# google/dynibar

Hardware: AMD Instinct MI355X
Metric: rays/sec (64 samples x 8 src views) (higher is better)
Workload: dtype f32 in / f32 accumulate; products from two half-float parts per operand (22-bit operands, 3 of the 4 partial products on the f16 matrix pipe, ~2^-20 relative per product); the exact 6-term bf16 build is tested beside it

## Files before the change

dynibar_amd/csrc/dyn_mlp.h:

```cpp
#pragma once
#include <utility>

#include "dyn_device.h"

#ifndef DYN_EXCLUSIVE_CU
#define DYN_EXCLUSIVE_CU 1
#endif
#if DYN_EXCLUSIVE_CU && defined(__AMDGCN__)
#define DYN_CLAIM_REGISTER_FILE() asm volatile("; the whole register file" ::: "v255", "a255")
#else
#define DYN_CLAIM_REGISTER_FILE()
#endif
#define DYN_NET_THREADS 256
#define DYN_VIEW_THREADS 512

__host__ __device__ constexpr int dyn_fi(int r, int h) { return (r & 3) + 8 * (r >> 2) + 4 * h; }

__device__ __forceinline__ f32x16 mfma32(float a, float b, f32x16 c) { return __builtin_amdgcn_mfma_f32_32x32x2f32(a, b, c, 0, 0, 0); }

template <int NT>
__device__ __forceinline__ void acc_zero(f32x16 (&acc)[NT]) {
#pragma unroll
  for (int t = 0; t < NT; ++t)
#pragma unroll
// ... 50 lines not shown
  return __builtin_bit_cast(float, __builtin_amdgcn_mov_dpp(__builtin_bit_cast(int, v), CTRL, 0xF, 0xF, true));
}
template <int VSEG, class Op>
__device__ __forceinline__ float seg_reduce(float v, Op op) {
  static_assert(VSEG == 4 || VSEG == 8 || VSEG == 16 || VSEG == 32, "segments are 4, 8, 16 or 32 lanes");
  v = op(v, dpp_get<DYN_DPP_XOR1>(v));
  v = op(v, dpp_get<DYN_DPP_XOR2>(v));
  if (VSEG >= 8) v = op(v, dpp_get<DYN_DPP_HALF_MIRROR>(v));
  if (VSEG >= 16) v = op(v, dpp_get<DYN_DPP_ROW_MIRROR>(v));
  if (VSEG >= 32) v = op(v, __shfl_xor(v, 16));
  return v;
}
__device__ __forceinline__ float add_half_mirror(float v) {
#if defined(__AMDGCN__)
  float r;
  asm("s_nop 1\n\tv_add_f32_dpp %0, %1, %1 row_half_mirror row_mask:0xf bank_mask:0xf bound_ctrl:1" : "=v"(r) : "v"(v));
  return r;
#else
  return v + dpp_get<DYN_DPP_HALF_MIRROR>(v);
#endif
}
template <int VSEG>
__device__ __forceinline__ float seg_sum(float v, int, int) {
  if (VSEG == 8) {
    v = seg_reduce<4>(v, [](float a, float b) {
#pragma clang fp contract(off)
      return a + b;
    });
    return add_half_mirror(v);
  }
  return seg_reduce<VSEG>(v, [](float a, float b) {
#pragma clang fp contract(off)
    return a + b;
  });
}
template <int VSEG>
__device__ __forceinline__ void seg_sum4(float& a, float& b, float& c, float& d) {
#if defined(__AMDGCN__)
  if (VSEG == 8) {
    auto quad = [](float v) {
      return seg_reduce<4>(v, [](float x, float y) {
#pragma clang fp contract(off)
        return x + y;
      });
    };
    a = quad(a); b = quad(b); c = quad(c); d = quad(d);
    asm("s_nop 1\n\t"
        "v_add_f32_dpp %0, %0, %0 row_half_mirror row_mask:0xf bank_mask:0xf bound_ctrl:1\n\t"
        "v_add_f32_dpp %1, %1, %1 row_half_mirror row_mask:0xf bank_mask:0xf bound_ctrl:1\n\t"
        "v_add_f32_dpp %2, %2, %2 row_half_mirror row_mask:0xf bank_mask:0xf bound_ctrl:1\n\t"
        "v_add_f32_dpp %3, %3, %3 row_half_mirror row_mask:0xf bank_mask:0xf bound_ctrl:1"
        : "+v"(a), "+v"(b), "+v"(c), "+v"(d));
    return;
  }
#endif
  a = seg_sum<VSEG>(a, 0, 0); b = seg_sum<VSEG>(b, 0, 0); c = seg_sum<VSEG>(c, 0, 0); d = seg_sum<VSEG>(d, 0, 0);
}
template <int VSEG>
__device__ __forceinline__ float seg_min(float v, int, int) {
  return seg_reduce<VSEG>(v, [](float a, float b) { return fminf(a, b); });
}
template <int VSEG>
__device__ __forceinline__ float seg_max(float v, int, int) {
  return seg_reduce<VSEG>(v, [](float a, float b) { return fmaxf(a, b); });
}

template <int NTI>
__device__ __forceinline__ float row_dot(const f32x16 (&act)[NTI], const float* tab) {
  const int h = (threadIdx.x & 63) >> 5;
  const float4* t4 = reinterpret_cast<const float4*>(tab + h * 16 * NTI);
  float s = 0.f;
#pragma unroll
  for (int t = 0; t < NTI; ++t)
#pragma unroll
    for (int q = 0; q < 4; ++q) {
      const float4 w = t4[t * 4 + q];
      s = fmaf(act[t][q * 4 + 0], w.x, s);
      s = fmaf(act[t][q * 4 + 1], w.y, s);
      s = fmaf(act[t][q * 4 + 2], w.z, s);
      s = fmaf(act[t][q * 4 + 3], w.w, s);
    }
  return s + __shfl_xor(s, 32);
}

#ifndef DYN_SPLIT_TERMS
#define DYN_SPLIT_TERMS 3
#endif
#ifndef DYN_SPLIT_F16
#define DYN_SPLIT_F16 1
#endif
#if DYN_SPLIT_F16 && DYN_SPLIT_TERMS == 6
#error "the half-float engine has one or two parts per operand (DYN_SPLIT_TERMS == 1 or 3)"
#endif
#if !DYN_SPLIT_F16 && DYN_SPLIT_TERMS == 1
#error "the one-product engine multiplies IEEE halves (DYN_SPLIT_F16 == 1)"
#endif
#if DYN_SPLIT_TERMS == 1
#define DYN_SPLIT_PARTS 1
#define B6_CHUNK_PAIRS 48
#elif DYN_SPLIT_TERMS == 3
#define DYN_SPLIT_PARTS 2
#define B6_CHUNK_PAIRS 24
#elif DYN_SPLIT_TERMS == 6
#define DYN_SPLIT_PARTS 3
#define B6_CHUNK_PAIRS 16
#else
#error "DYN_SPLIT_TERMS must be 1, 3 or 6"
#endif
#define DYN_BIAS_ONE(h) ((DYN_SPLIT_TERMS == 1 || (h) == 0) ? 1.0f : 0.0f)
typedef __bf16 bf16x8 __attribute__((ext_vector_type(8)));
typedef __bf16 bf16x2v __attribute__((ext_vector_type(2)));
typedef _Float16 f16x8 __attribute__((ext_vector_type(8)));
typedef _Float16 f16x2v __attribute__((ext_vector_type(2)));
typedef float f32x2v __attribute__((ext_vector_type(2)));
typedef unsigned u32x4v __attribute__((ext_vector_type(4)));

#define B6_PAIR_FLOATS (DYN_SPLIT_PARTS * 256)
#define B6_CHUNK (B6_CHUNK_PAIRS * B6_PAIR_FLOATS)

#ifdef DYN_PHASE_TIMING
__device__ unsigned long long g_phase[3][2][160];
#define DYN_PHASE_ON (threadIdx.x == 0 && (blockIdx.x == 0 || blockIdx.x == gridDim.x / 2))
#define DYN_PHASE(i)                                                                                  \
  do {                                                                                                \
    if (DYN_PHASE_ON) g_phase[PHASE_KID][blockIdx.x != 0][i] = __builtin_readcyclecounter();          \
  } while (0)
extern "C" int dyn_debug_phases(unsigned long long* out) {
  return hipMemcpyFromSymbol(out, HIP_SYMBOL(g_phase), sizeof(g_phase)) == hipSuccess ? 0 : 1;
}
#define DYN_PHASE_T0 const unsigned long long phase_t0 = __builtin_readcyclecounter();
#ifdef DYN_PHASE_SKEW
__device__ unsigned long long g_skew[8][4];
extern "C" int dyn_debug_skew(unsigned long long* out) { return hipMemcpyFromSymbol(out, HIP_SYMBOL(g_skew), sizeof(g_skew)) == hipSuccess ? 0 : 1; }
extern "C" int dyn_debug_skew_reset(void) { unsigned long long z[32] = {0}; return hipMemcpyToSymbol(HIP_SYMBOL(g_skew), z, sizeof(z)) == hipSuccess ? 0 : 1; }
#endif
#define DYN_PHASE_WAIT(R, c)                                                                          \
  do {                                                                                                \
    if (DYN_PHASE_ON && (c) < 64) {                                                                   \
      g_phase[(R).kid][blockIdx.x != 0][32 + (c)] = __builtin_readcyclecounter() - phase_t0;          \
      g_phase[(R).kid][blockIdx.x != 0][96 + (c)] = phase_t0;                                         \
    }                                                                                                 \
  } while (0)
#define DYN_PHASE_RING_KID(R, k) (R).kid = (k)
#else
#define DYN_PHASE(i)
#define DYN_PHASE_T0
#define DYN_PHASE_WAIT(R, c)
#define DYN_PHASE_RING_KID(R, k)
#endif

struct WeightRing6 {
  const float* gbase;
  float* buf;
  int next, total;
  int skip_at, skip_n;
  int round;
  int half;
  unsigned lds_wave;
  unsigned lane_off;
  int fill, issued;
  int nbuf;
#ifdef DYN_PHASE_TIMING
  int kid;
#endif
};


#ifndef B6_DMA_POLICY
#define B6_DMA_POLICY ""
#endif
#ifndef B6_DMA_WINDOW_NUM
#define B6_DMA_WINDOW_NUM 2
#define B6_DMA_WINDOW_DEN 3
#endif
template <int OFF>
__device__ __forceinline__ void b6_dma_piece(const float* g_uniform, unsigned lane_off, unsigned l, float* l_emu) {
#if defined(__AMDGCN__)
#pragma clang diagnostic push
#pragma clang diagnostic ignored "-Winline-asm"
  asm volatile("s_mov_b32 m0, %2\n\ts_nop 0\n\tglobal_load_lds_dwordx4 %0, %1 offset:%3" B6_DMA_POLICY ::"v"(lane_off), "s"(g_uniform), "s"(l), "n"(OFF) : "m0", "memory");
#pragma clang diagnostic pop
#else
  __builtin_amdgcn_global_load_lds((const __attribute__((address_space(1))) void*)((const char*)g_uniform + lane_off),
                                   (__attribute__((address_space(3))) void*)l_emu, 16, OFF, 0);
#endif
}
__device__ __forceinline__ int ring6_pieces(const WeightRing6& R) { return B6_CHUNK / R.round; }
__device__ __forceinline__ void ring6_piece(const WeightRing6& R, int k) {
  const int waves = R.round / 256, per_wave = B6_CHUNK / waves;
  const int grp = k / 6, i = k % 6;
  const int chunk = R.fill;
  const float* gu = R.gbase + (long)(chunk + (chunk >= R.skip_at ? R.skip_n : 0)) * B6_CHUNK + grp * 1536;
  const int slot = R.nbuf == 2 ? (chunk & 1) : 0;
  const unsigned l = R.lds_wave + (unsigned)((slot * B6_CHUNK + grp * 1536) * sizeof(float));
  float* le = R.buf + slot * B6_CHUNK + (threadIdx.x >> 6) * per_wave + 512 + grp * 1536;
  if (i == 0) b6_dma_piece<-2048>(gu, R.lane_off, l, le);
  if (i == 1) b6_dma_piece<-1024>(gu, R.lane_off, l, le);
  if (i == 2) b6_dma_piece<0>(gu, R.lane_off, l, le);
  if (i == 3) b6_dma_piece<1024>(gu, R.lane_off, l, le);
  if (i == 4) b6_dma_piece<2048>(gu, R.lane_off, l, le);
  if (i == 5) b6_dma_piece<3072>(gu, R.lane_off, l, le);
}
#ifndef B6_FEED_STATELESS
#define B6_FEED_STATELESS (DYN_SPLIT_TERMS == 1 ? 1 : 0)
#endif
__device__ __forceinline__ void ring6_feed(WeightRing6& R, int pr, int npc) {
  if (R.fill < 0) return;
  const int n = ring6_pieces(R);
  const int den = (B6_DMA_WINDOW_NUM * npc + B6_DMA_WINDOW_DEN - 1) / B6_DMA_WINDOW_DEN > 0 ? (B6_DMA_WINDOW_NUM * npc + B6_DMA_WINDOW_DEN - 1) / B6_DMA_WINDOW_DEN : 1;
  int want = (n * (pr + 1) + den - 1) / den;
  if (want > n) want = n;
#if B6_FEED_STATELESS
  int prev = (n * pr + den - 1) / den;
  if (prev > n) prev = n;
#pragma unroll
  for (int k = 0; k < 12; ++k)
    if (k >= prev && k < want) ring6_piece(R, k);
  for (int k = prev > 12 ? prev : 12; k < want; ++k) ring6_piece(R, k);
  R.issued = want;
#else
  for (; R.issued < want; ++R.issued) ring6_piece(R, R.issued);
#endif
}

__device__ __forceinline__ void ring6_issue(const WeightRing6& R, int chunk) {
  const int waves = R.round / 256, wave = threadIdx.x >> 6, lane = threadIdx.x & 63;
  const int per_wave = B6_CHUNK / waves;
  const float* g = R.gbase + (long)(chunk + (chunk >= R.skip_at ? R.skip_n : 0)) * B6_CHUNK + wave * per_wave + 512 + lane * 4;
  float* l = R.buf + (R.nbuf == 2 ? (chunk & 1) : 0) * B6_CHUNK + wave * per_wave + 512;
#pragma unroll
  for (int grp = 0; grp < 2; ++grp)
    if (grp * 1536 < per_wave) {
      const auto* gg = (const __attribute__((address_space(1))) void*)(g + grp * 1536);
      auto* ll = (__attribute__((address_space(3))) void*)(l + grp * 1536);
      __builtin_amdgcn_global_load_lds(gg, ll, 16, -2048, 0);
      __builtin_amdgcn_global_load_lds(gg, ll, 16, -1024, 0);
      __builtin_amdgcn_global_load_lds(gg, ll, 16, 0, 0);
      __builtin_amdgcn_global_load_lds(gg, ll, 16, 1024, 0);
      __builtin_amdgcn_global_load_lds(gg, ll, 16, 2048, 0);
      __builtin_amdgcn_global_load_lds(gg, ll, 16, 3072, 0);
    }
}
__device__ __forceinline__ void ring6_init(WeightRing6& R, const float* stream, int total, float* lds, int skip_at = 1 << 30, int skip_n = 0,
                                           int threads = 0, int nbuf = 2) {
  R.gbase = stream;
  R.buf = lds;
  R.next = 0;
  R.total = total - skip_n;
  R.skip_at = skip_at;
  R.skip_n = skip_n;
  R.round = (threads > 0 ? threads : (int)blockDim.x) * 4;
  R.nbuf = nbuf;
#if defined(__AMDGCN__)
  R.half = __builtin_amdgcn_readfirstlane((int)threadIdx.x >> 8);
#else
  R.half = (int)threadIdx.x >> 8;
#endif
  {
    const int waves = R.round / 256, per_wave = B6_CHUNK / waves;
#if defined(__AMDGCN__)
    const int wave = __builtin_amdgcn_readfirstlane((int)threadIdx.x >> 6);
    R.lds_wave = (unsigned)(size_t)(__attribute__((address_space(3))) void*)(lds + wave * per_wave + 512);
#else
    const int wave = (int)threadIdx.x >> 6;
    R.lds_wave = 0;
#endif
    R.lane_off = (unsigned)((wave * per_wave + 512 + (threadIdx.x & 63) * 4) * sizeof(float));
  }
  R.fill = -1;
  R.issued = 0;
  DYN_PHASE_RING_KID(R, 0);
  ring6_issue(R, 0);
}
__device__ __forceinline__ const float* ring6_acquire(WeightRing6& R) {
  DYN_PHASE_T0
  if (R.nbuf == 1) {
    const int c = R.next++;
    if (c > 0) {
      __syncthreads();
      ring6_issue(R, c);
    }
    __builtin_amdgcn_s_waitcnt(0x0F70);
    __syncthreads();
    DYN_PHASE_WAIT(R, c);
    return R.buf;
  }
  if (R.fill >= 0) {
    const int n = ring6_pieces(R);
    for (; R.issued < n; ++R.issued) ring6_piece(R, R.issued);
    R.fill = -1;
  }
  __builtin_amdgcn_s_waitcnt(0x0F70);
#ifdef DYN_PHASE_SKEW
  const unsigned long long skew_t1 = __builtin_readcyclecounter();
#endif
  __syncthreads();
  const int c = R.next++;
#ifdef DYN_PHASE_SKEW
  if ((threadIdx.x & 63) == 0 && blockIdx.x == gridDim.x / 2 && R.kid == 0) {
    g_skew[threadIdx.x >> 6][0] += skew_t1 - phase_t0;
    g_skew[threadIdx.x >> 6][1] += __builtin_readcyclecounter() - skew_t1;
    g_skew[threadIdx.x >> 6][2] += 1;
  }
#endif
  DYN_PHASE_WAIT(R, c);
  R.fill = c + 1 < R.total ? c + 1 : -1;
  R.issued = 0;
  return R.buf + (c & 1) * B6_CHUNK;
}

#ifndef B6_PRIO_FLIP
#define B6_PRIO_FLIP 2
#endif
#ifndef B6_PRIO_MODE
#define B6_PRIO_MODE 5
#endif
__device__ __forceinline__ void ring6_prio_flip(const WeightRing6& R, int phase) {
#if defined(__AMDGCN__)
  if (R.round != 8 * 256) return;
#if B6_PRIO_MODE == 1
  if (phase & 1) __builtin_amdgcn_s_setprio(1);
  else __builtin_amdgcn_s_setprio(0);
#elif B6_PRIO_MODE == 5
  if ((((int)threadIdx.x >> 8) ^ phase) & 1) __builtin_amdgcn_s_setprio(1);
  else __builtin_amdgcn_s_setprio(0);
#endif
#endif
}
__device__ __forceinline__ void split3_pair(float a, float b, unsigned& hi, unsigned& mid, unsigned& lo) {
#if DYN_SPLIT_TERMS == 1
  const f32x2v v = {__builtin_amdgcn_fmed3f(a, -65504.0f, 65504.0f), __builtin_amdgcn_fmed3f(b, -65504.0f, 65504.0f)};
  hi = __builtin_bit_cast(unsigned, __builtin_convertvector(v, f16x2v));
  mid = 0u;
  lo = 0u;
#elif DYN_SPLIT_F16
  const auto h = __builtin_amdgcn_cvt_pkrtz(a, b);
  hi = __builtin_bit_cast(unsigned, h);
#if defined(__AMDGCN__)
  unsigned m;
  asm("v_fma_mixlo_f16 %0, %1, -1.0, %2 op_sel_hi:[1,0,0]" : "=v"(m) : "v"(hi), "v"(a));
  asm("v_fma_mixhi_f16 %0, %1, -1.0, %2 op_sel:[1,0,0] op_sel_hi:[1,0,0]" : "+v"(m) : "v"(hi), "v"(b));
  mid = m;
#else
  const float ra = a - (float)h[0], rb = b - (float)h[1];
  mid = __builtin_bit_cast(unsigned, __builtin_amdgcn_cvt_pkrtz(ra, rb));
#endif
  lo = 0u;
#else
  f32x2v v = {a, b};
  hi = __builtin_bit_cast(unsigned, __builtin_convertvector(v, bf16x2v));
  f32x2v hf = {__uint_as_float(hi << 16), __uint_as_float(hi & 0xffff0000u)};
  f32x2v r1 = v - hf;
  mid = __builtin_bit_cast(unsigned, __builtin_convertvector(r1, bf16x2v));
#if DYN_SPLIT_PARTS == 3
  f32x2v mf = {__uint_as_float(mid << 16), __uint_as_float(mid & 0xffff0000u)};
  f32x2v r2 = r1 - mf;
  lo = __builtin_bit_cast(unsigned, __builtin_convertvector(r2, bf16x2v));
#else
  lo = 0u;
#endif
#endif
}

__device__ __forceinline__ f32x16 mfma_bf16(u32x4v a, u32x4v b, f32x16 c) {
#if DYN_SPLIT_F16
  return __builtin_amdgcn_mfma_f32_32x32x16_f16(__builtin_bit_cast(f16x8, a), __builtin_bit_cast(f16x8, b), c, 0, 0, 0);
#else
  return __builtin_amdgcn_mfma_f32_32x32x16_bf16(__builtin_bit_cast(bf16x8, a), __builtin_bit_cast(bf16x8, b), c, 0, 0, 0);
#endif
}

__host__ __device__ constexpr int b6_layer_chunks(int NT, int NSLOTS, int CP = B6_CHUNK_PAIRS) {
  return (((NSLOTS + 7) / 8) + (CP / NT) - 1) / (CP / NT);
}

struct B6A {
  u32x4v hi, mid, lo;
};
__device__ __forceinline__ B6A b6_load_a(const float* pair, int lane) {
  const u32x4v* w = reinterpret_cast<const u32x4v*>(pair) + lane;
  B6A a;
  a.hi = w[0];
#if DYN_SPLIT_PARTS >= 2
  a.mid = w[64];
#endif
#if DYN_SPLIT_PARTS == 3
  a.lo = w[128];
#endif
  return a;
}

template <int NSLOTS, int P0, int P1, class Feed>
__device__ __forceinline__ void b6_split_pairs(Feed& feed, int g, u32x4v& bh, u32x4v& bm, u32x4v& bl) {
#pragma unroll
  for (int p2 = P0; p2 < P1; ++p2) {
    const float v0 = (g * 8 + 2 * p2 < NSLOTS) ? feed(g * 8 + 2 * p2) : 0.f;
    const float v1 = (g * 8 + 2 * p2 + 1 < NSLOTS) ? feed(g * 8 + 2 * p2 + 1) : 0.f;
    unsigned h_, m_, l_;
    split3_pair(v0, v1, h_, m_, l_);
    bh[p2] = h_; bm[p2] = m_; bl[p2] = l_;
  }
}

#ifndef B6_AHEAD
#define B6_AHEAD 1
#endif
template <int NT, int NSLOTS, int AHEAD = B6_AHEAD, class Feed>
__device__ __forceinline__ void mlp_layer_b6(WeightRing6& R, f32x16 (&acc)[NT], Feed&& feed) {
  constexpr int NG = (NSLOTS + 7) / 8;
  constexpr int GPC = B6_CHUNK_PAIRS / NT;
  constexpr int NCH = (NG + GPC - 1) / GPC;
  static_assert(B6_CHUNK_PAIRS % NT == 0, "tiles per layer must divide the pairs of a chunk");
  static_assert(NT == 1 || NT == 2 || NT == 4 || NT == 8, "output tiles per layer");
  const int lane = threadIdx.x & 63;
  u32x4v bh, bm, bl, nh, nm, nl;
  b6_split_pairs<NSLOTS, 0, 4>(feed, 0, bh, bm, bl);
  nh = bh; nm = bm; nl = bl;
  __builtin_amdgcn_sched_barrier(0);
#pragma unroll
  for (int c = 0; c < NCH; ++c) {
    const float* buf = ring6_acquire(R);
    constexpr int NPC_MAX = B6_CHUNK_PAIRS;
    const int npc = (NG - c * GPC < GPC ? NG - c * GPC : GPC) * NT;
    B6A q[AHEAD + 1];
#pragma unroll
    for (int i = 0; i < AHEAD; ++i)
      if (i < npc) q[i] = b6_load_a(buf + i * B6_PAIR_FLOATS, lane);
    __builtin_amdgcn_sched_barrier(0);
#pragma unroll
    for (int pr = 0; pr < NPC_MAX; ++pr) {
      if (pr < npc) {
        const int gi = pr / NT, t = pr % NT;
        const int g = c * GPC + gi;
        ring6_feed(R, pr, npc);
#if B6_PRIO_FLIP && (B6_PRIO_MODE == 1 || B6_PRIO_MODE == 5)
        if (pr % B6_PRIO_FLIP == 0) ring6_prio_flip(R, (pr / B6_PRIO_FLIP) & 1);
#endif
        if (pr + AHEAD < npc) q[(pr + AHEAD) % (AHEAD + 1)] = b6_load_a(buf + (pr + AHEAD) * B6_PAIR_FLOATS, lane);
        if (g + 1 < NG) {
          if (NT == 1) b6_split_pairs<NSLOTS, 0, 4>(feed, g + 1, nh, nm, nl);
          if (NT == 2 && t == 0) b6_split_pairs<NSLOTS, 0, 2>(feed, g + 1, nh, nm, nl);
          if (NT == 2 && t == 1) b6_split_pairs<NSLOTS, 2, 4>(feed, g + 1, nh, nm, nl);
          if (NT == 4 && t == 0) b6_split_pairs<NSLOTS, 0, 1>(feed, g + 1, nh, nm, nl);
          if (NT == 4 && t == 1) b6_split_pairs<NSLOTS, 1, 2>(feed, g + 1, nh, nm, nl);
          if (NT == 4 && t == 2) b6_split_pairs<NSLOTS, 2, 3>(feed, g + 1, nh, nm, nl);
          if (NT == 4 && t == 3) b6_split_pairs<NSLOTS, 3, 4>(feed, g + 1, nh, nm, nl);
          if (NT == 8 && t == 0) b6_split_pairs<NSLOTS, 0, 1>(feed, g + 1, nh, nm, nl);
          if (NT == 8 && t == 2) b6_split_pairs<NSLOTS, 1, 2>(feed, g + 1, nh, nm, nl);
          if (NT == 8 && t == 4) b6_split_pairs<NSLOTS, 2, 3>(feed, g + 1, nh, nm, nl);
          if (NT == 8 && t == 6) b6_split_pairs<NSLOTS, 3, 4>(feed, g + 1, nh, nm, nl);
        }
        const B6A& cur = q[pr % (AHEAD + 1)];
#if DYN_SPLIT_TERMS == 6
        acc[t] = mfma_bf16(cur.lo, bh, acc[t]);
        acc[t] = mfma_bf16(cur.hi, bl, acc[t]);
        acc[t] = mfma_bf16(cur.mid, bm, acc[t]);
#endif
#if DYN_SPLIT_TERMS != 1
        acc[t] = mfma_bf16(cur.mid, bh, acc[t]);
        acc[t] = mfma_bf16(cur.hi, bm, acc[t]);
#endif
        acc[t] = mfma_bf16(cur.hi, bh, acc[t]);
        if (t == NT - 1) { bh = nh; bm = nm; bl = nl; }
        __builtin_amdgcn_sched_barrier(0);
      }
    }
  }
}

#ifndef B6D_AHEAD
#define B6D_AHEAD 4
#endif
#define B6D_SLOTS 3
struct WeightRing3 {
  const float* gbase;
  const float* glane;
  float* buf;
  unsigned lds_wave;
  unsigned lane_off;
  int next, total;
  int waves;
  int cf;
  int fill, issued;
  float* slot[B6D_SLOTS];
  unsigned lds_slot[B6D_SLOTS];
#ifdef DYN_PHASE_TIMING
  int kid;
#endif
};
template <int OFF>
__device__ __forceinline__ void ring3_dma(const float* g, float* l_emu, unsigned l, const float* g_uniform, unsigned lane_off) {
#if defined(__AMDGCN__)
#pragma clang diagnostic push
#pragma clang diagnostic ignored "-Winline-asm"
  asm volatile("s_mov_b32 m0, %2\n\ts_nop 0\n\tglobal_load_lds_dwordx4 %0, %1 offset:%3" ::"v"(lane_off), "s"(g_uniform), "s"(l), "n"(OFF) : "m0", "memory");
#pragma clang diagnostic pop
#else
  __builtin_amdgcn_global_load_lds((const __attribute__((address_space(1))) void*)g, (__attribute__((address_space(3))) void*)l_emu, 16, OFF, 0);
#endif
}
__device__ __forceinline__ int ring3_pieces(const WeightRing3& R) { return R.cf / (R.waves * 256); }
__device__ __forceinline__ void ring3_piece(const WeightRing3& R, int chunk, int k) {
  const int per_wave = R.cf / R.waves;
  const int grp = k / 6, i = k % 6;
  const float* g = R.glane + (long)chunk * R.cf + grp * 1536;
  const float* gu = R.gbase + (long)chunk * R.cf + grp * 1536;
  const unsigned l = R.lds_slot[chunk % B6D_SLOTS] + (unsigned)(grp * 1536 * sizeof(float));
  float* le = R.slot[chunk % B6D_SLOTS] + (threadIdx.x >> 6) * per_wave + 512 + grp * 1536;
  if (i == 0) ring3_dma<-2048>(g, le, l, gu, R.lane_off);
  if (i == 1) ring3_dma<-1024>(g, le, l, gu, R.lane_off);
  if (i == 2) ring3_dma<0>(g, le, l, gu, R.lane_off);
  if (i == 3) ring3_dma<1024>(g, le, l, gu, R.lane_off);
  if (i == 4) ring3_dma<2048>(g, le, l, gu, R.lane_off);
  if (i == 5) ring3_dma<3072>(g, le, l, gu, R.lane_off);
}
template <int ALLOW = 0>
__device__ __forceinline__ void ring3_barrier() {
#if defined(__AMDGCN__)
  static_assert(ALLOW >= 0 && ALLOW < 16, "vmcnt immediate");
  __builtin_amdgcn_s_waitcnt(0x0F70 | ALLOW);
  __builtin_amdgcn_s_barrier();
#else
  __syncthreads();
#endif
}
__device__ __forceinline__ void ring3_init(WeightRing3& R, const float* stream, int total, float* lds, int threads, int chunk_pairs = B6_CHUNK_PAIRS) {
  R.gbase = stream;
  R.buf = lds;
  R.next = 0;
  R.total = total;
  R.waves = threads / 64;
  R.cf = chunk_pairs * B6_PAIR_FLOATS;
  {
    const int per_wave = R.cf / R.waves;
#if defined(__AMDGCN__)
    const int wave = __builtin_amdgcn_readfirstlane((int)threadIdx.x >> 6);
    R.lds_wave = (unsigned)(size_t)(__attribute__((address_space(3))) void*)(lds + wave * per_wave + 512);
#else
    const int wave = threadIdx.x >> 6;
    R.lds_wave = 0;
#endif
    R.glane = stream + wave * per_wave + 512 + (threadIdx.x & 63) * 4;
    R.lane_off = (unsigned)((wave * per_wave + 512 + (threadIdx.x & 63) * 4) * sizeof(float));
  }
  R.fill = -1;
  R.issued = 0;
  for (int j = 0; j < B6D_SLOTS; ++j) {
    R.slot[j] = lds + j * R.cf;
    R.lds_slot[j] = R.lds_wave + (unsigned)(j * R.cf * sizeof(float));
  }
  DYN_PHASE_RING_KID(R, 0);
  for (int c = 0; c < 2 && c < total; ++c)
    for (int k = 0; k < ring3_pieces(R); ++k) ring3_piece(R, c, k);
}
__device__ __forceinline__ void ring3_enter(WeightRing3& R) {
  if (R.next != 0) return;
  const int n = R.total > 1 ? ring3_pieces(R) : 0;
  if (n == 12) ring3_barrier<12>();
  else if (n == 8) ring3_barrier<8>();
  else if (n == 6) ring3_barrier<6>();
  else if (n == 4) ring3_barrier<4>();
  else ring3_barrier<0>();
}
__device__ __forceinline__ const float* ring3_slot(const WeightRing3& R, int chunk) { return R.slot[chunk % B6D_SLOTS]; }
#ifndef B6D_DMA_MARGIN
#define B6D_DMA_MARGIN 4
#endif
__device__ __forceinline__ void ring3_feed(WeightRing3& R, int half, int num, int den) {
  if (R.fill < 0) return;
  const int n = ring3_pieces(R), h0 = n / 2;
  int want = half == 0 ? (h0 * num + den - 1) / den : h0 + ((n - h0) * num + den - 1) / den;
// ... 294 lines not shown
```

dynibar_amd/csrc/dyn_nets.hip:

```cpp
#include <math.h>
#include <stdlib.h>
#include <string.h>

#include <functional>
#include <vector>

#include "dyn_host.h"
#include "dyn_mlp.h"
#include "dyn_pack.h"

namespace {

using SlotFn = std::function<float(int t, int i, int s, int h)>;

thread_local bool g_pack_slot_error = false;
thread_local int g_pack_chunk_pairs = B6_CHUNK_PAIRS;
void pack_layer_b6(std::vector<float>& out, int NT, int NSLOTS, const SlotFn& fn, int ones_slot = -1) {
  const int CPAIRS = g_pack_chunk_pairs, CFLOATS = CPAIRS * B6_PAIR_FLOATS;
  const int NG = (NSLOTS + 7) / 8, GPC = CPAIRS / NT, NCH = (NG + GPC - 1) / GPC;
  const size_t base = out.size();
  out.resize(base + (size_t)NCH * CFLOATS, 0.f);
  unsigned short* img = reinterpret_cast<unsigned short*>(out.data() + base);
  for (int c = 0; c < NCH; ++c)
    for (int gi = 0; gi < GPC; ++gi) {
      const int g = c * GPC + gi;
      if (g >= NG) continue;
      for (int t = 0; t < NT; ++t)
        for (int lane = 0; lane < 64; ++lane)
          for (int e = 0; e < 8; ++e) {
            const int s = g * 8 + e;
            if (s >= NSLOTS) continue;
            const bool two_half_bias = DYN_SPLIT_PARTS == 1 && s == ones_slot;
            if (two_half_bias && fn(t, lane & 31, s, 1) != 0.f) g_pack_slot_error = true;
            const float w = fn(t, lane & 31, s, two_half_bias ? 0 : lane >> 5);
            unsigned short hi, mid, lo;
            split_weight(w, hi, mid, lo);
            const size_t pair = (size_t)c * CFLOATS * 2 + (size_t)(gi * NT + t) * B6_PAIR_FLOATS * 2;
            img[pair + 0 * 512 + lane * 8 + e] = two_half_bias && (lane >> 5) == 1 ? mid : hi;
            if (DYN_SPLIT_PARTS >= 2) img[pair + 1 * 512 + lane * 8 + e] = mid;
            if (DYN_SPLIT_PARTS == 3) img[pair + 2 * 512 + lane * 8 + e] = lo;
          }
    }
}

void pack_net_layer(std::vector<float>& out, int NT, int NSLOTS, const SlotFn& fn, int ones_slot = -1) {
  pack_layer_b6(out, NT, NSLOTS, fn, ones_slot);
}

inline int chain_feature(int s, int h) { return 32 * (s / 16) + dyn_fi(s % 16, h); }

SlotFn chained(const float* W, const float* b, int nout, int nin, int ld, int col0 = 0) {
  return [=](int t, int i, int s, int h) -> float {
    const int n = 32 * t + i;
    if (n >= nout) return 0.f;
    const int nsteps_in = nin / 2;
    if (s < nsteps_in) return W[(size_t)n * ld + col0 + chain_feature(s, h)];
    if (s == nsteps_in && h == 0 && b != nullptr) return b[n];
    return 0.f;
  };
}

void pack_rowtab(std::vector<float>& out, const float* w, int n, double scale = 1.0) {
  for (int h = 0; h < 2; ++h)
    for (int k = 0; k < n / 2; ++k) out.push_back((float)((double)w[chain_feature(k, h)] * scale));
}

SlotFn scaled_wb(SlotFn fn, int nsteps_w, double kw, double kb) {
  return [=](int t, int i, int s, int h) -> float { return (float)((double)fn(t, i, s, h) * (s < nsteps_w ? kw : kb)); };
}

SlotFn scaled(SlotFn fn, double scale) {
  if (scale == 1.0) return fn;
  return [=](int t, int i, int s, int h) -> float { return (float)((double)fn(t, i, s, h) * scale); };
}

void pack_qkv_by_head(std::vector<float>& out, const float* Wq, const float* Wk, const float* Wv) {
  for (int hd = 0; hd < 4; ++hd) {
    pack_net_layer(out, 2, 64, [=](int t, int i, int s, int h) -> float { return (t == 0 ? Wq : Wk)[(size_t)(32 * hd + i) * 128 + chain_feature(s, h)]; });
    if (hd % 2 == 0)
      pack_net_layer(out, 2, 64, [=](int t, int i, int s, int h) -> float { return Wv[(size_t)(32 * (hd + t) + i) * 128 + chain_feature(s, h)]; });
  }
}

}

enum {
  ST_RAYDIR0_W, ST_RAYDIR0_B, ST_RAYDIR2_W, ST_RAYDIR2_B, ST_REFFEAT_W, ST_REFFEAT_B, ST_BASE0_W, ST_BASE0_B, ST_BASE2_W, ST_BASE2_B,
  ST_VIS0_W, ST_VIS0_B, ST_VIS2_W, ST_VIS2_B, ST_VISB0_W, ST_VISB0_B, ST_VISB2_W, ST_VISB2_B, ST_GEO0_W, ST_GEO0_B, ST_GEO2_W,
  ST_GEO2_B, ST_WQ, ST_WK, ST_WV, ST_FC, ST_LN_G, ST_LN_B, ST_OG0_W, ST_OG0_B, ST_OG2_W, ST_OG2_B, ST_RGB0_W, ST_RGB0_B,
  ST_RGB2_W, ST_RGB2_B, ST_RGB4_W, ST_RGB4_B, ST_S, ST_NUM_TENSORS
};

#define SA_L1P_STEPS 17
#define SA_L1V_STEPS 36
#define SA_L2_STEPS 128
#define SA_NX 37
#define SA_L3_STEPS (3 * SA_NX + 1)
#define SA_L3P_STEPS (2 * SA_NX)
#define SA_L3V_STEPS (SA_NX + 1)
#define SA_L4_STEPS 128
#define SA_L5_STEPS 64
constexpr int SA_CHUNKS = net_layer_chunks(8, SA_L1P_STEPS) + net_layer_chunks(8, SA_L1V_STEPS) + net_layer_chunks(2, SA_L2_STEPS) + net_layer_chunks(8, SA_L3P_STEPS) + net_layer_chunks(8, SA_L3V_STEPS) +
                          net_layer_chunks(4, SA_L4_STEPS) + 3 * net_layer_chunks(4, SA_L5_STEPS);
#ifndef DYN_POINTS_DUO
#define DYN_POINTS_DUO (DYN_SPLIT_TERMS != 6 ? 1 : 0)
#endif
#if DYN_POINTS_DUO
#define PTS_CP 16
#define PTS_CHUNK (PTS_CP * B6_PAIR_FLOATS)
#define PTS_RING_SLOTS B6D_SLOTS
__host__ __device__ constexpr int pts_layer_chunks(int NT, int NSLOTS) { return b6_layer_chunks(NT, NSLOTS, PTS_CP); }
typedef WeightRing3 PtsRing;
#define pts_ring_init(R, stream, total, lds) ring3_init(R, stream, total, lds, DYN_NET_THREADS, PTS_CP)
#define PTS_LAYER(NT, NSLOTS) mlp_layer_b6_duo<NT, NSLOTS, PTS_CP>
#else
#define PTS_CHUNK NET_CHUNK
#define PTS_RING_SLOTS 2
__host__ __device__ constexpr int pts_layer_chunks(int NT, int NSLOTS) { return net_layer_chunks(NT, NSLOTS); }
typedef NetRing PtsRing;
#define pts_ring_init(R, stream, total, lds) net_ring_init_t(R, stream, total, lds, DYN_NET_THREADS)
#define PTS_LAYER(NT, NSLOTS) net_layer<NT, NSLOTS>
#endif
constexpr int SB_CHUNKS = pts_layer_chunks(8, 129) + pts_layer_chunks(4, 129) + 4 * pts_layer_chunks(4, 64) + 2 * pts_layer_chunks(4, 65);
#define SC_L11_STEPS 67
constexpr int SC_CHUNKS = net_layer_chunks(4, SC_L11_STEPS) + net_layer_chunks(2, 64);
#define SA_CT 848
#define SB_CT 400
#define SC_CT 144
constexpr size_t ST_OFF_A = 0;
constexpr size_t ST_OFF_B = ST_OFF_A + (size_t)SA_CHUNKS * NET_CHUNK;
constexpr size_t ST_OFF_C = ST_OFF_B + (size_t)SB_CHUNKS * PTS_CHUNK;
constexpr size_t ST_OFF_CTA = ST_OFF_C + (size_t)SC_CHUNKS * NET_CHUNK;
constexpr size_t ST_OFF_CTB = ST_OFF_CTA + SA_CT;
constexpr size_t ST_OFF_CTC = ST_OFF_CTB + SB_CT;
constexpr size_t ST_OFF_REF = ST_OFF_CTC + SC_CT;
constexpr size_t ST_OFF_B8 = (ST_OFF_REF + 35 * 66 + 36 + 63) / 64 * 64;
constexpr size_t ST_BLOB_FLOATS = ST_OFF_B8 + (DYN_POINTS_DUO ? (size_t)SB_CHUNKS * PTS_CHUNK : 0);

enum {
  DT_RAYDIR0_W, DT_RAYDIR0_B, DT_RAYDIR2_W, DT_RAYDIR2_B, DT_BASE0_W, DT_BASE0_B, DT_BASE2_W, DT_BASE2_B, DT_VIS0_W, DT_VIS0_B, DT_VIS2_W,
  DT_VIS2_B, DT_VISB0_W, DT_VISB0_B, DT_VISB2_W, DT_VISB2_B, DT_GEO0_W, DT_GEO0_B, DT_GEO2_W, DT_GEO2_B, DT_WQ, DT_WK, DT_WV, DT_FC, DT_LN_G,
  DT_LN_B, DT_REFPTS0_W, DT_REFPTS0_B, DT_REFPTS2_W, DT_REFPTS2_B, DT_OG0_W, DT_OG0_B, DT_OG2_W, DT_OG2_B, DT_RGB0_W, DT_RGB0_B, DT_RGB2_W,
  DT_RGB2_B, DT_RGB4_W, DT_RGB4_B, DT_NUM_TENSORS
};
#define DA_NX 18
#define DA_L3_STEPS (3 * DA_NX + 1)
#define DA_L3P_STEPS (2 * DA_NX)
#define DA_L3V_STEPS (DA_NX + 1)
constexpr int DA_CHUNKS = net_layer_chunks(8, DA_L3P_STEPS) + net_layer_chunks(8, DA_L3V_STEPS) + net_layer_chunks(4, SA_L4_STEPS) + 3 * net_layer_chunks(4, SA_L5_STEPS);
constexpr int DB_CHUNKS = pts_layer_chunks(8, 129) + pts_layer_chunks(4, 129) + 4 * pts_layer_chunks(4, 64) + pts_layer_chunks(8, 81) +
                          pts_layer_chunks(4, 129) + pts_layer_chunks(4, 65) + pts_layer_chunks(4, 78) + pts_layer_chunks(2, 65);
#define DB_CT 592
constexpr size_t DY_OFF_A = 0;
constexpr size_t DY_OFF_B = DY_OFF_A + (size_t)DA_CHUNKS * NET_CHUNK;
constexpr size_t DY_OFF_CTA = DY_OFF_B + (size_t)DB_CHUNKS * PTS_CHUNK;
constexpr size_t DY_OFF_CTB = DY_OFF_CTA + SA_CT;
constexpr size_t DY_OFF_POSENC = DY_OFF_CTB + DB_CT;
constexpr size_t DY_OFF_TIME = DY_OFF_POSENC + 256 * 128;
constexpr size_t DY_OFF_B8 = (DY_OFF_TIME + 256 * 21 + 256 + 35 * 256 + 36 + 63) / 64 * 64;
constexpr size_t DY_BLOB_FLOATS = DY_OFF_B8 + (DYN_POINTS_DUO ? (size_t)DB_CHUNKS * PTS_CHUNK : 0);
__host__ __device__ constexpr int da_c35(int q, int h) { return h == 0 ? q : (q < 17 ? 18 + q : -1); }

__host__ __device__ constexpr int sa_c70(int q, int h) {
  if (q < 18) return h == 0 ? q : (q < 17 ? 18 + q : -1);
  if (q < 34) return 35 + dyn_fi(q - 18, h);
  return h == 0 ? 35 + 32 + (q - 34) : -1;
}

static int sa_l1p_col(int s, int h) {
  if (s < 15) {
    const int c = s / 5, fi = s % 5;
    return 3 + (h * 5 + fi) * 3 + c;
  }
  const int k = (s - 15) * 2 + h;
  return k < 3 ? k : -1;
}
static int sa_l1v_col(int s, int h) {
  if (s < 30) {
    const int c = s / 5, fi = s % 5;
    return 33 + 6 + (h * 5 + fi) * 6 + c;
  }
  const int k = (s - 30) * 2 + h;
  if (k < 6) return 33 + k;
  if (k < 10) return 99 + (k - 6);
  return k == 10 ? -2 : -1;
}

extern "C" size_t dyn_static_net_blob_floats(void) { return ST_BLOB_FLOATS; }

extern "C" int dyn_static_net_pack(const float* const* T, int F, float* blob, size_t blob_floats) {
  DYN_REQUIRE(T && blob, "dyn_static_net_pack: null pointer");
  DYN_REQUIRE(F == 32, "dyn_static_net_pack: the kernels are specialised for 32 feature channels (coarse_feat_dim = fine_feat_dim = 32)");
  DYN_REQUIRE(blob_floats >= ST_BLOB_FLOATS, "dyn_static_net_pack: blob too small");
  for (int i = 0; i < ST_NUM_TENSORS; ++i) DYN_REQUIRE(T[i] != nullptr, "dyn_static_net_pack: tensor %d is NULL", i);
  std::vector<float> o;
  g_pack_range_error = false;
  g_pack_slot_error = false;
  o.reserve(ST_BLOB_FLOATS);
  {
    const float *W = T[ST_RAYDIR0_W], *b = T[ST_RAYDIR0_B];
    pack_net_layer(o, 8, SA_L1P_STEPS, scaled([=](int t, int i, int s, int h) -> float {
      const int n = 32 * t + i, c = sa_l1p_col(s, h);
      return c >= 0 ? W[n * 103 + c] : 0.f;
    }, DYN_ELU_PRE));
    pack_net_layer(o, 8, SA_L1V_STEPS, scaled([=](int t, int i, int s, int h) -> float {
      const int n = 32 * t + i, c = sa_l1v_col(s, h);
      return c >= 0 ? W[n * 103 + c] : (c == -2 ? b[n] : 0.f);
    }, DYN_ELU_PRE), 35);
  }
  pack_net_layer(o, 2, SA_L2_STEPS, scaled(chained(T[ST_RAYDIR2_W], nullptr, 35, 256, 256), DYN_ELU_POST));
  {
    const float *W = T[ST_BASE0_W], *b = T[ST_BASE0_B];
    pack_net_layer(o, 8, SA_L3P_STEPS, scaled([=](int t, int i, int s, int h) -> float {
      const int c = sa_c70(s % SA_NX, h);
      return c < 0 ? 0.f : W[(32 * t + i) * 210 + (s / SA_NX) * 70 + c];
    }, DYN_ELU_PRE));
    pack_net_layer(o, 8, SA_L3V_STEPS, scaled([=](int t, int i, int s, int h) -> float {
      const int n = 32 * t + i;
      if (s == SA_NX) return h == 0 ? b[n] : 0.f;
      const int c = sa_c70(s, h);
      return c < 0 ? 0.f : W[n * 210 + 140 + c];
    }, DYN_ELU_PRE), SA_NX);
  }
  pack_net_layer(o, 4, SA_L4_STEPS, scaled(chained(T[ST_BASE2_W], nullptr, 128, 256, 256), DYN_ELU_POST));
  pack_net_layer(o, 4, SA_L5_STEPS, scaled(chained(T[ST_VIS0_W], nullptr, 128, 128, 128), DYN_ELU_PRE));
  pack_net_layer(o, 4, SA_L5_STEPS, scaled(chained(T[ST_VIS2_W], nullptr, 128, 128, 128), DYN_ELU_POST));
  pack_net_layer(o, 4, SA_L5_STEPS, scaled(chained(T[ST_VISB0_W], nullptr, 128, 128, 128), DYN_ELU_PRE));
  DYN_REQUIRE(o.size() == ST_OFF_B, "static pack: A stream size mismatch");
  const auto pack_b = [&](bool by_head) {
#if DYN_POINTS_DUO
  g_pack_chunk_pairs = PTS_CP;
#endif
  {
    const float *W = T[ST_GEO0_W], *b = T[ST_GEO0_B];
    pack_net_layer(o, 8, 129, scaled([=](int t, int i, int s, int h) -> float {
      const int n = 32 * t + i;
      if (s < 128) return W[n * 257 + (s < 64 ? 0 : 128) + chain_feature(s % 64, h)];
      return h == 0 ? W[n * 257 + 256] : b[n];
    }, DYN_ELU_PRE));
  }
  pack_net_layer(o, 4, 129, scaled_wb(chained(T[ST_GEO2_W], T[ST_GEO2_B], 128, 256, 256), 128, DYN_ELU_POST, 1.0), 128);
  if (by_head) {
    pack_qkv_by_head(o, T[ST_WQ], T[ST_WK], T[ST_WV]);
  } else {
    pack_net_layer(o, 4, 64, chained(T[ST_WQ], nullptr, 128, 128, 128));
    pack_net_layer(o, 4, 64, chained(T[ST_WK], nullptr, 128, 128, 128));
    pack_net_layer(o, 4, 64, chained(T[ST_WV], nullptr, 128, 128, 128));
  }
  pack_net_layer(o, 4, 64, chained(T[ST_FC], nullptr, 128, 128, 128));
  pack_net_layer(o, 4, 65, scaled(chained(T[ST_OG0_W], T[ST_OG0_B], 128, 128, 128), DYN_ELU_PRE), 64);
  pack_net_layer(o, 4, 65, scaled(chained(T[ST_RGB0_W], T[ST_RGB0_B], 128, 128, 261), DYN_ELU_PRE), 64);
  g_pack_chunk_pairs = B6_CHUNK_PAIRS;
  };
  pack_b(false);
  DYN_REQUIRE(o.size() == ST_OFF_C, "static pack: B stream size mismatch");
  {
    const float* W = T[ST_RGB0_W];
    pack_net_layer(o, 4, SC_L11_STEPS, scaled([=](int t, int i, int s, int h) -> float {
      const int n = 32 * t + i;
      if (s < 64) return W[n * 261 + 128 + chain_feature(s, h)];
      const int k = (s - 64) * 2 + h;
      return k < 5 ? W[n * 261 + 256 + k] : 0.f;
    }, DYN_ELU_PRE));
  }
  pack_net_layer(o, 2, 64, scaled(chained(T[ST_RGB2_W], nullptr, 64, 128, 128), DYN_ELU_POST * DYN_ELU_PRE));
  DYN_REQUIRE(o.size() == ST_OFF_CTA, "static pack: C stream size mismatch");
  pack_rowtab(o, T[ST_VIS2_W] + 128 * 128, 128, DYN_ELU_POST);
  pack_rowtab(o, T[ST_VISB2_W], 128, DYN_ELU_POST);
  o.push_back(T[ST_VIS2_B][128]);
  o.push_back(T[ST_VISB2_B][0]);
  o.push_back(fabsf(T[ST_S][0]));
  o.resize(ST_OFF_CTA + 272, 0.f);
  pack_rowtab(o, T[ST_BASE2_B], 128);
  pack_rowtab(o, T[ST_VIS0_B], 128, DYN_ELU_PRE);
  pack_rowtab(o, T[ST_VIS2_B], 128);
  pack_rowtab(o, T[ST_VISB0_B], 128, DYN_ELU_PRE);
  {
    float b64[64] = {0.f};
    for (int i = 0; i < 35; ++i) b64[i] = T[ST_RAYDIR2_B][i];
    pack_rowtab(o, b64, 64);
  }
  o.resize(ST_OFF_CTB, 0.f);
  pack_rowtab(o, T[ST_LN_G], 128);
  pack_rowtab(o, T[ST_LN_B], 128);
  pack_rowtab(o, T[ST_OG2_W], 128, DYN_ELU_POST);
  o.push_back(T[ST_OG2_B][0]);
  o.resize(ST_OFF_CTC, 0.f);
  pack_rowtab(o, T[ST_RGB4_W], 64, DYN_ELU_POST);
  o.push_back(T[ST_RGB4_B][0]);
  o.resize(ST_OFF_CTC + 80, 0.f);
  pack_rowtab(o, T[ST_RGB2_B], 64, DYN_ELU_PRE);
  o.resize(ST_OFF_REF, 0.f);
  for (int i = 0; i < 35 * 66; ++i) o.push_back(T[ST_REFFEAT_W][i]);
  for (int i = 0; i < 35; ++i) o.push_back(T[ST_REFFEAT_B][i]);
  o.resize(ST_OFF_B8, 0.f);
#if DYN_POINTS_DUO
  pack_b(true);
#endif
  DYN_REQUIRE(o.size() == ST_BLOB_FLOATS, "static pack: B8 stream size mismatch");
  DYN_REQUIRE(!g_pack_slot_error, "dyn_static_net_pack: a layer's bias slot carries a weight in its second half (the one-product build stores the bias residual there)");
  DYN_REQUIRE(!g_pack_range_error, "dyn_static_net_pack: a weight is outside the half-float range of the split engine (|w| >= 65504 or not finite)");
  for (size_t i = 0; i < ST_BLOB_FLOATS; ++i) blob[i] = o[i];
  return 0;
}

static bool dense_views(int V) {
  static const int mode = getenv("DYN_DENSE_VIEWS") ? atoi(getenv("DYN_DENSE_VIEWS")) : -1;
  if (mode == 0) return false;
  if (mode == 1) return V >= 9;
  return (V >= 9 && V <= 12) || (V >= 17 && V <= 26);
}
struct StaticWs {
  bool dense, ragged;
  long n_pts, n_tiles_a, n_tiles_b;
  int PT, TPR;
  size_t off_x, off_vis, off_gin, off_nvalid, off_hg, off_ref, total;
  size_t off_qkvg;
  long n_seg, n_wg_max;
  size_t off_bits, off_emin, off_segcnt, off_segstart, off_wgstart;
  size_t off_rowtab, off_ptab;
};
#define RAG_SEG 1024
#define RAG_SEG_WGS 160
#define RAG_MAX_PTS 32
#define RAG_PTAB 36

#define DYN_MAX_SAMPLES 256
#define SB_GIN_RECS 33
#define SB_HG_RECS 16

#ifndef DYN_BLEND_WS
#define DYN_BLEND_WS (DYN_SPLIT_TERMS != 6 ? 1 : 0)
#endif
static bool ragged_rows_enabled() {
  static const int off = getenv("DYN_RAGGED") ? (atoi(getenv("DYN_RAGGED")) == 0) : 0;
  static const int blend_stream = getenv("DYN_BLEND_STREAM") != nullptr;
  return DYN_BLEND_WS && !off && !blend_stream;
}
static StaticWs static_ws(int R, int S, int V, bool dynamic = false) {
  StaticWs w;
  w.n_pts = (long)R * S;
  w.dense = dense_views(V);
  w.ragged = w.dense && ragged_rows_enabled();
  w.PT = w.dense ? 256 / V : 32 / (V <= 4 ? 4 : (V <= 8 ? 8 : (V <= 16 ? 16 : 32)));
  w.n_tiles_a = w.dense ? ((w.n_pts + w.PT - 1) / w.PT) * 8 : (w.n_pts + w.PT - 1) / w.PT;
  w.n_seg = (w.n_pts + RAG_SEG - 1) / RAG_SEG;
  w.n_wg_max = w.ragged ? (w.n_pts + w.PT - 1) / w.PT + w.n_seg : 0;
  if (w.ragged) w.n_tiles_a = w.n_wg_max * 8;
  int tpr = (S + 31) / 32;
  w.TPR = tpr <= 1 ? 1 : (tpr <= 2 ? 2 : ((tpr + 3) / 4) * 4);
  w.n_tiles_b = (long)R * w.TPR;
  size_t o = 0;
  w.off_x = o; o += dynamic ? 0 : (size_t)w.n_tiles_a * 64 * 64;
  w.off_vis = o; o += dynamic ? 0 : (size_t)w.n_tiles_a * 128;
  w.off_gin = o; o += (size_t)w.n_tiles_b * SB_GIN_RECS * 256;
  w.off_nvalid = o; o += (size_t)((w.n_pts + 3) & ~3L);
  w.off_hg = o; o += dynamic ? 0 : (size_t)w.n_tiles_b * SB_HG_RECS * 256;
  w.off_ref = o; o += dynamic ? 64 : (size_t)R * 36;
  o = (o + 3) & ~(size_t)3;
  w.off_qkvg = o; o += w.TPR > 4 ? (size_t)w.n_tiles_b * 4 * 4096 : 0;
  w.off_bits = o; o += w.ragged ? (size_t)((w.n_pts + 3) & ~3L) : 0;
  w.off_emin = o; o += w.ragged ? (size_t)((w.n_pts + 3) & ~3L) : 0;
  w.off_segcnt = o; o += w.ragged ? (size_t)((w.n_seg + 3) & ~3L) : 0;
  w.off_segstart = o; o += w.ragged ? (size_t)w.n_seg * RAG_SEG_WGS : 0;
  w.off_wgstart = o; o += w.ragged ? (size_t)((w.n_wg_max + 2 + 3) & ~3L) : 0;
  w.off_rowtab = o; o += w.ragged ? (size_t)w.n_wg_max * 128 : 0;
  w.off_ptab = o; o += w.ragged ? (size_t)w.n_wg_max * RAG_PTAB : 0;
  w.total = o;
  return w;
}

extern "C" size_t dyn_static_net_workspace_bytes(int R, int S, int V) {
  if (R <= 0 || S <= 0 || V <= 0 || V > 32) return 0;
  return static_ws(R, S, V).total * sizeof(float);
}

__device__ __forceinline__ void unit3(float x, float y, float z, float& ox, float& oy, float& oz) {
  const float d = fmaxf(sqrtf(x * x + y * y + z * z), 1e-12f);
  ox = x / d; oy = y / d; oz = z / d;
}

__device__ __forceinline__ void sincos_small(float x, float& s, float& c) {
  const float y = rintf(x * 0.63661977236758134f);
  const int q = (int)y;
  float r = fmaf(y, -1.57079637050628662109375f, x);
  r = fmaf(y, 4.37113900018624283e-8f, r);
  const float z = r * r;
  const float ps = fmaf(fmaf(fmaf(-1.9515295891e-4f, z, 8.3321608736e-3f), z, -1.6666654611e-1f) * z, r, r);
  const float pc = fmaf(fmaf(fmaf(2.443315711809948e-5f, z, -1.388731625493765e-3f), z, 4.166664568298827e-2f), z * z, fmaf(z, -0.5f, 1.0f));
  const bool swap = q & 1;
  const float sv = swap ? pc : ps, cv = swap ? ps : pc;
  s = __uint_as_float(__float_as_uint(sv) ^ ((unsigned)(q & 2) << 30));
  c = __uint_as_float(__float_as_uint(cv) ^ ((unsigned)((q + 1) & 2) << 30));
}

template <int NF>
__device__ __forceinline__ void octave_embed(float x, int h, float* out) {
  float sn, cs;
  sincos_small(x, sn, cs);
#pragma unroll
  for (int f = 0; f < NF; ++f) {
    out[f] = h == 0 ? cs : sn;
    const float s2 = 2.0f * sn * cs;
    cs = cs * cs - sn * sn;
    sn = s2;
  }
}

#define REF_RAYS 8
__global__ void __launch_bounds__(256, 1) k_static_ref_feat(const float* __restrict__ ray_o, const float* __restrict__ ray_d, const float* __restrict__ Wref, int R,
                                  float* __restrict__ ref_feat) {
  DYN_CLAIM_REGISTER_FILE();
  float* pe = reinterpret_cast<float*>(dyn_smem);
  const int r0 = blockIdx.x * REF_RAYS;
  for (int t = threadIdx.x; t < REF_RAYS * 66; t += 256) {
    const int rl = t / 66, jj = t - rl * 66;
    const int r = r0 + rl < R ? r0 + rl : R - 1;
    float d[3], c[6];
    unit3(ray_d[r * 3], ray_d[r * 3 + 1], ray_d[r * 3 + 2], d[0], d[1], d[2]);
    const float ox = ray_o[r * 3], oy = ray_o[r * 3 + 1], oz = ray_o[r * 3 + 2];
    c[0] = d[0]; c[1] = d[1]; c[2] = d[2];
    c[3] = oy * d[2] - oz * d[1];
    c[4] = oz * d[0] - ox * d[2];
    c[5] = ox * d[1] - oy * d[0];
    if (dyn_ref_cross_axis(R) != DYN_CROSS_XYZ) {
      float m[3];
      dyn_ref_moment_over_rays(ray_o, ray_d, r, m);
      c[3] = m[0]; c[4] = m[1]; c[5] = m[2];
    }
    const int e = jj < 6 ? jj : (jj - 6) % 6;
    float ck = c[0];
    ck = e == 1 ? c[1] : ck; ck = e == 2 ? c[2] : ck; ck = e == 3 ? c[3] : ck; ck = e == 4 ? c[4] : ck; ck = e == 5 ? c[5] : ck;
    float v = ck;
    if (jj >= 6) {
      const int f = ((jj - 6) / 6) % 5, fn = (jj - 6) / 30;
      const float a = (float)(1 << f) * ck;
      v = fn == 0 ? cosf(a) : sinf(a);
    }
    pe[t] = v;
  }
  __syncthreads();
  for (int t = threadIdx.x; t < REF_RAYS * 36; t += 256) {
    const int rl = t / 36, ch = t - rl * 36;
    if (r0 + rl >= R) continue;
    float acc = 0.f;
    if (ch < 35) {
      const float* w = Wref + ch * 66;
      const float* x = pe + rl * 66;
      acc = Wref[35 * 66 + ch];
      for (int j = 0; j < 66; ++j) acc = fmaf(w[j], x[j], acc);
    }
    ref_feat[(long)(r0 + rl) * 36 + ch] = acc;
// ... 99 lines not shown
  d.point0 = hd.point0;
  d.PTW = hd.np;
  const bool live = d.rw < d.n_rows;
  d.p_local = live ? (ri & 0xff) : RAG_MAX_PTS + 1;
  d.view = live ? (ri >> 8) : 0;
  const int pc = live ? d.p_local : d.PTW - 1;
  d.base = pt[pc];
  d.cnt = pt[pc + 1] - d.base;
  return d;
}

__device__ __forceinline__ float aa_exp(float s_abs, float dot) { return expm1f(s_abs * (dot - 1.0f)); }

__global__ void __launch_bounds__(256) k_ragged_points(long n_pts, int V, const float* __restrict__ mask, const float4* __restrict__ ray_diff, const float* __restrict__ s_abs,
                                                       unsigned* __restrict__ bits, float* __restrict__ emin) {
  float* dw = reinterpret_cast<float*>(dyn_smem);
  unsigned char* mk = reinterpret_cast<unsigned char*>(dw + 256 * V);
  const long p0 = (long)blockIdx.x * 256;
  const int np = (int)(n_pts - p0 < 256 ? n_pts - p0 : 256), n = np * V;
  const bool aa = s_abs != nullptr;
  for (int i = threadIdx.x; i < n; i += 256) {
    mk[i] = mask[p0 * V + i] != 0.f ? 1 : 0;
    if (aa) dw[i] = ray_diff[p0 * V + i].w;
  }
  __syncthreads();
  const int t = threadIdx.x;
  if (t >= np) return;
  unsigned b = 0u;
  float m = 3.0e38f;
  const float sa = aa ? s_abs[0] : 0.f;
  for (int v = 0; v < V; ++v) {
    if (mk[t * V + v]) b |= 1u << v;
    if (aa) m = fminf(m, aa_exp(sa, dw[t * V + v]));
  }
  bits[p0 + t] = b;
  if (aa) emin[p0 + t] = m;
}

__global__ void __launch_bounds__(256) k_ragged_segments(long n_pts, long n_seg, const unsigned* __restrict__ bits, int* __restrict__ seg_cnt, int* __restrict__ seg_start) {
  int* pre = reinterpret_cast<int*>(dyn_smem);
  int* part = pre + RAG_SEG + 4;
  unsigned short* nxt = reinterpret_cast<unsigned short*>(part + 256);
  const int tid = threadIdx.x;
  const long seg = blockIdx.x;
  const long p0 = seg * RAG_SEG;
  const int n = (int)((p0 + RAG_SEG < n_pts ? p0 + RAG_SEG : n_pts) - p0);
  int r4[4], sum = 0;
#pragma unroll
  for (int j = 0; j < 4; ++j) {
    const int i = 4 * tid + j;
    const unsigned b = i < n ? bits[p0 + i] : 0u;
    r4[j] = i < n ? (b != 0u ? __popc(b) : 1) : 0;
    sum += r4[j];
  }
  part[tid] = sum;
  __syncthreads();
  for (int off = 1; off < 256; off <<= 1) {
    const int t = tid >= off ? part[tid - off] : 0;
    __syncthreads();
    part[tid] += t;
    __syncthreads();
  }
  int run = part[tid] - sum;
#pragma unroll
  for (int j = 0; j < 4; ++j) {
    pre[4 * tid + j] = run;
    run += r4[j];
  }
  if (tid == 255) pre[RAG_SEG] = run;
  __syncthreads();
#pragma unroll
  for (int j = 0; j < 4; ++j) {
    const int i = 4 * tid + j;
    if (i < n) {
      int lo = i + 1, hi = i + RAG_MAX_PTS < n ? i + RAG_MAX_PTS : n;
      const int base = pre[i];
      while (lo < hi) {
        const int mid = (lo + hi + 1) >> 1;
        if (pre[mid] - base <= 256) lo = mid; else hi = mid - 1;
      }
      nxt[i] = (unsigned short)lo;
    }
  }
  __syncthreads();
  if (tid != 0) return;
  int* out = seg_start + seg * RAG_SEG_WGS;
  int n_wg = 0;
  for (int i = 0; i < n; i = nxt[i]) out[n_wg++] = i;
  seg_cnt[seg] = n_wg;
}

__global__ void __launch_bounds__(1024) k_ragged_scatter(long n_pts, long n_seg, const int* __restrict__ seg_cnt, const int* __restrict__ seg_start, int* __restrict__ wg) {
  int* part = reinterpret_cast<int*>(dyn_smem);
  int& carry = part[1024];
  const int tid = threadIdx.x;
  if (tid == 0) carry = 0;
  __syncthreads();
  for (long s0 = 0; s0 < n_seg; s0 += 1024) {
    const long seg = s0 + tid;
    const int n = seg < n_seg ? seg_cnt[seg] : 0;
    part[tid] = n;
    __syncthreads();
    for (int off = 1; off < 1024; off <<= 1) {
      const int t = tid >= off ? part[tid - off] : 0;
      __syncthreads();
      part[tid] += t;
      __syncthreads();
    }
    const int base = carry + part[tid] - n;
    if (seg < n_seg)
      for (int i = 0; i < n; ++i) wg[1 + base + i] = (int)(seg * RAG_SEG) + seg_start[seg * RAG_SEG_WGS + i];
    __syncthreads();
    if (tid == 1023) carry += part[1023];
    __syncthreads();
  }
  if (tid == 0) {
    wg[0] = carry;
    wg[1 + carry] = (int)n_pts;
  }
}

__global__ void __launch_bounds__(64) k_ragged_tables(const unsigned* __restrict__ bits_g, const int* __restrict__ wg, unsigned short* __restrict__ rowtab, int* __restrict__ ptab) {
  const long wgi = blockIdx.x;
  if (wgi >= wg[0]) return;
  const int tid = threadIdx.x, i = tid & 31;
  const int p0 = wg[1 + wgi], np = wg[2 + wgi] - p0;
  const bool own = tid < 32 && i < np;
  const unsigned bits = own ? bits_g[p0 + i] : 0u;
  const int n = own ? (bits != 0u ? __popc(bits) : 1) : 0;
  int incl = n;
#pragma unroll
  for (int off = 1; off < 32; off <<= 1) {
    const int t = __shfl_up(incl, off, 32);
    if (i >= off) incl += t;
  }
  unsigned short* rt = rowtab + wgi * 256;
  int* pt = ptab + wgi * RAG_PTAB;
  const int total = __shfl(incl, 31);
  for (int r = total + tid; r < 256; r += 64) rt[r] = 0;
  if (tid < 32) {
    pt[i] = incl - n;
    if (i == 31) { pt[32] = incl; pt[33] = p0; pt[34] = np; pt[35] = 0; }
    int r = incl - n;
    if (own) {
      if (bits == 0u) {
        rt[r] = (unsigned short)i;
      } else {
        for (unsigned b = bits; b != 0u; b &= b - 1u) rt[r++] = (unsigned short)(i | ((__ffs(b) - 1) << 8));
      }
    }
  }
}

template <class Op>
__device__ __forceinline__ float dense_all(const DenseRows& d, float v, float ident, Op op) {
  if ((threadIdx.x & 32) == 0) d.scal[d.rw] = v;
  __syncthreads();
  const float* src = d.scal + d.base;
  float a0 = ident, a1 = ident, a2 = ident, a3 = ident;
  int k = 0;
  for (; k + 4 <= d.cnt; k += 4) { a0 = op(a0, src[k]); a1 = op(a1, src[k + 1]); a2 = op(a2, src[k + 2]); a3 = op(a3, src[k + 3]); }
  for (; k < d.cnt; ++k) a0 = op(a0, src[k]);
  __syncthreads();
  return op(op(a0, a1), op(a2, a3));
}
__device__ __forceinline__ void dense_all2(const DenseRows& d, float v0, float v1, float& s0, float& s1) {
  if ((threadIdx.x & 32) == 0) { d.scal[d.rw] = v0; d.scal[256 + d.rw] = v1; }
  __syncthreads();
  const float* src = d.scal + d.base;
  float a0 = 0.f, a1 = 0.f, b0 = 0.f, b1 = 0.f;
  int k = 0;
  for (; k + 2 <= d.cnt; k += 2) { a0 += src[k]; a1 += src[k + 1]; b0 += src[256 + k]; b1 += src[256 + k + 1]; }
  for (; k < d.cnt; ++k) { a0 += src[k]; b0 += src[256 + k]; }
  __syncthreads();
  s0 = a0 + a1; s1 = b0 + b1;
}
template <int VSEG>
__device__ __forceinline__ float views_sum(const DenseRows& d, float v) {
  if constexpr (VSEG == 0) return dense_all(d, v, 0.f, [](float a, float b) { return a + b; });
  else return seg_sum<VSEG>(v, 0, 0);
}
template <int VSEG>
__device__ __forceinline__ float views_min(const DenseRows& d, float v) {
  if constexpr (VSEG == 0) return dense_all(d, v, 3.0e38f, [](float a, float b) { return fminf(a, b); });
  else return seg_min<VSEG>(v, 0, 0);
}
template <int VSEG>
__device__ __forceinline__ float views_max(const DenseRows& d, float v) {
  if constexpr (VSEG == 0) return dense_all(d, v, -3.0e38f, [](float a, float b) { return fmaxf(a, b); });
  else return seg_max<VSEG>(v, 0, 0);
}

__device__ __forceinline__ float4 dense_quad(const float* src, int k, int stride, int) { return *reinterpret_cast<const float4*>(src + k * stride); }
__device__ __forceinline__ float dense_w(const float* w, int k, int) { return w[k]; }

template <int NX>
__device__ __forceinline__ void dense_pool_stats(const DenseRows& d, const float (&xin)[NX], float wgt, float* pool, float* tab) {
  constexpr int QPH = 4, RS = 2 * 4 * QPH + 4;
  constexpr int NQ = (NX + 3) / 4, ROUNDS = (NQ + QPH - 1) / QPH;
  const int tid = threadIdx.x, h = (tid >> 5) & 1;
  float* wrow = d.scal;
  if (h == 0) wrow[d.rw] = wgt;
  auto X = [&](int i) { return i < NX ? xin[i < NX ? i : 0] : 0.f; };
#pragma unroll
  for (int round = 0; round < ROUNDS; ++round) {
    const int nq = (NQ - round * QPH < QPH) ? NQ - round * QPH : QPH;
    float4* mine = reinterpret_cast<float4*>(tab + d.rw * RS + h * (4 * QPH));
#pragma unroll
    for (int qq = 0; qq < QPH; ++qq) {
      const int q = round * QPH + qq;
      if (q < NQ) mine[qq] = make_float4(X(4 * q), X(4 * q + 1), X(4 * q + 2), X(4 * q + 3));
    }
    __syncthreads();
    const int total = d.PTW * 2 * nq;
    for (int task = tid; task < total; task += DYN_VIEW_THREADS) {
      const int pnt = task / (2 * nq), rem = task - pnt * (2 * nq), hh = rem / nq, qq = rem - hh * nq;
      const int pb = dense_pt_base(d, pnt), pn = dense_pt_cnt(d, pnt);
      const float* src = tab + pb * RS + hh * (4 * QPH) + qq * 4;
      const float* w = wrow + pb;
      float4 m0 = make_float4(0.f, 0.f, 0.f, 0.f), m1 = m0;
      int k = 0;
      for (; k + 2 <= pn; k += 2) {
        const float4 x0 = dense_quad(src, k, RS, pn), x1 = dense_quad(src, k + 1, RS, pn);
        const float w0 = dense_w(w, k, pn), w1 = dense_w(w, k + 1, pn);
        m0.x = fmaf(w0, x0.x, m0.x); m0.y = fmaf(w0, x0.y, m0.y); m0.z = fmaf(w0, x0.z, m0.z); m0.w = fmaf(w0, x0.w, m0.w);
        m1.x = fmaf(w1, x1.x, m1.x); m1.y = fmaf(w1, x1.y, m1.y); m1.z = fmaf(w1, x1.z, m1.z); m1.w = fmaf(w1, x1.w, m1.w);
      }
      if (k < pn) {
        const float4 x0 = dense_quad(src, k, RS, pn);
        const float w0 = dense_w(w, k, pn);
        m0.x = fmaf(w0, x0.x, m0.x); m0.y = fmaf(w0, x0.y, m0.y); m0.z = fmaf(w0, x0.z, m0.z); m0.w = fmaf(w0, x0.w, m0.w);
      }
      const float mean[4] = {m0.x + m1.x, m0.y + m1.y, m0.z + m1.z, m0.w + m1.w};
      float v0[4] = {0.f, 0.f, 0.f, 0.f}, v1[4] = {0.f, 0.f, 0.f, 0.f};
      for (k = 0; k + 2 <= pn; k += 2) {
        const float4 x0 = dense_quad(src, k, RS, pn), x1 = dense_quad(src, k + 1, RS, pn);
        const float w0 = dense_w(w, k, pn), w1 = dense_w(w, k + 1, pn);
        const float a0[4] = {x0.x, x0.y, x0.z, x0.w}, a1[4] = {x1.x, x1.y, x1.z, x1.w};
#pragma unroll
        for (int e = 0; e < 4; ++e) {
          const float d0 = a0[e] - mean[e], d1 = a1[e] - mean[e];
          v0[e] = fmaf(w0, d0 * d0, v0[e]);
          v1[e] = fmaf(w1, d1 * d1, v1[e]);
        }
      }
      if (k < pn) {
        const float4 x0 = dense_quad(src, k, RS, pn);
        const float w0 = dense_w(w, k, pn);
        const float a0[4] = {x0.x, x0.y, x0.z, x0.w};
#pragma unroll
        for (int e = 0; e < 4; ++e) {
          const float d0 = a0[e] - mean[e];
          v0[e] = fmaf(w0, d0 * d0, v0[e]);
        }
      }
#pragma unroll
      for (int e = 0; e < 4; ++e) {
        const int q = 4 * (round * QPH + qq) + e;
        if (q < NX) {
          pool[(q * 2 + hh) * 32 + pnt] = mean[e];
          pool[((NX + q) * 2 + hh) * 32 + pnt] = v0[e] + v1[e];
        }
      }
    }
    __syncthreads();
  }
}

template <int VSEG, int NX>
__device__ __forceinline__ void base_fc0(NetRing& ring, const float* pooled_w, const float (&xin)[NX], float wgt, int V, int view, int p_local,
                                         float* pool, f32x16 (&a1)[8], const DenseRows* dr = nullptr, float wsum = 0.f) {
  constexpr int PHASE_KID = 0;
  (void)PHASE_KID;
  const int lane = threadIdx.x & 63, j = lane & 31, h = lane >> 5, wave = threadIdx.x >> 6;
  const float one_h0 = DYN_BIAS_ONE(h);
  if constexpr (VSEG == 0) {
    float* res = pool + POOL_FLOATS(NX);
    B6TileW<2 * NX> pw;
    b6_tile_prefetch<8, 2 * NX>(pooled_w, wave, pw);
    dense_pool_stats<NX>(*dr, xin, wgt, pool, res);
    if (threadIdx.x < 2 * 2 * NX)
      for (int c = dr->PTW; c < 32; ++c) pool[threadIdx.x * 32 + c] = 0.f;
    __syncthreads();
    f32x16 accp[1];
    acc_zero(accp);
    b6_tile_apply<2 * NX>(pw, accp[0], [&](int s) { return pool[(s * 2 + h) * 32 + j]; });
    res_put(res, wave, j, h, accp[0]);
    __syncthreads();
    const int col = dr->p_local < dr->PTW ? dr->p_local : dr->PTW - 1;
    res_get(res, col, h, a1);
  } else if (VSEG >= 8) {
    static_assert(DYN_VIEW_THREADS / 64 == 8, "one output tile of base_fc.0 per wave");
    constexpr int PT = 32 / VSEG;
    float* res = pool + POOL_FLOATS(NX);
    const int col = wave * PT + p_local;
    B6TileW<2 * NX> pw;
    b6_tile_prefetch<8, 2 * NX>(pooled_w, wave, pw);
    float pm[NX], pvr[NX];
#pragma unroll
    for (int q0 = 0; q0 + 4 <= NX; q0 += 4) {
      float m4[4], v4[4];
#pragma unroll
      for (int e = 0; e < 4; ++e) m4[e] = xin[q0 + e] * wgt;
      seg_sum4<VSEG>(m4[0], m4[1], m4[2], m4[3]);
#pragma unroll
      for (int e = 0; e < 4; ++e) {
        const float d = xin[q0 + e] - m4[e];
        v4[e] = wgt * (d * d);
      }
      seg_sum4<VSEG>(v4[0], v4[1], v4[2], v4[3]);
#pragma unroll
      for (int e = 0; e < 4; ++e) { pm[q0 + e] = m4[e]; pvr[q0 + e] = v4[e]; }
    }
#pragma unroll
    for (int q = NX & ~3; q < NX; ++q) {
      pm[q] = seg_sum<VSEG>(xin[q] * wgt, V, 0);
      const float d = xin[q] - pm[q];
      pvr[q] = seg_sum<VSEG>(wgt * (d * d), V, 0);
    }
    if (view == 0) {
#pragma unroll
      for (int q = 0; q < NX; ++q) {
        pool[(q * 2 + h) * 32 + col] = pm[q];
        pool[((NX + q) * 2 + h) * 32 + col] = pvr[q];
      }
    }
    if (8 * PT < 32 && threadIdx.x < 2 * 2 * NX)
      for (int c = 8 * PT; c < 32; ++c) pool[threadIdx.x * 32 + c] = 0.f;
    DYN_PHASE(6);
    __syncthreads();
    f32x16 accp[1];
    acc_zero(accp);
    b6_tile_apply<2 * NX>(pw, accp[0], [&](int s) { return pool[(s * 2 + h) * 32 + j]; });
    DYN_PHASE(7);
    res_put(res, wave, j, h, accp[0]);
    __syncthreads();
    res_get(res, col, h, a1);
    DYN_PHASE(8);
  } else {
    acc_zero(a1);
    net_layer<8, 2 * NX>(ring, a1, [&](int s) {
      const int q = s < NX ? s : s - NX;
      const float m = seg_sum<VSEG>(xin[q] * wgt, V, 0);
      if (s < NX) return m;
      const float d = xin[q] - m;
      return seg_sum<VSEG>(wgt * (d * d), V, 0);
    });
  }
  net_layer<8, NX + 1>(ring, a1, [&](int s) { return s < NX ? xin[s] : one_h0; });
  DYN_PHASE(9);
}

template <int VSEG, bool STORE_X>
__device__ __forceinline__ void views_tail(NetRing& ring, f32x16 (&a1)[8], const StaticArgs& p, const float* ctab, float wgt, float msk,
                                           long tile, long point, bool valid, int view, int seg_base, const DenseRows* dr = nullptr,
                                           float* lds_base = nullptr, int v_const = 0) {
  constexpr int PHASE_KID = 0;
  (void)PHASE_KID;
  const int lane = threadIdx.x & 63, h = lane >> 5;
  const int V = v_const > 0 ? v_const : p.V;
  f32x16 x[4];
  {
    acc_init_bias<4>(x, ctab + 272);
    net_layer<4, SA_L4_STEPS>(ring, x, [&](int s) { return elu_s(a1[s / 16][s % 16]); });
    DYN_PHASE(11);
  }
  float vis;
  {
    f32x16 a5[4], a6[4];
    acc_init_bias<4>(a5, ctab + 400);
    DYN_PHASE(12);
    net_layer<4, SA_L5_STEPS>(ring, a5, [&](int s) {
      const float r = elu1(x[s / 16][s % 16]);
      x[s / 16][s % 16] = r;
      return r * wgt;
    });
    DYN_PHASE(13);
    acc_init_bias<4>(a6, ctab + 528);
    net_layer<4, SA_L5_STEPS>(ring, a6, [&](int s) {
      const float r = elu_s(a5[s / 16][s % 16]);
      a5[s / 16][s % 16] = r;
      return r;
    });
    DYN_PHASE(14);
    vis = sigmoid1(elu1(row_dot<4>(a5, ctab) + ctab[256])) * msk;
#pragma unroll
    for (int t = 0; t < 4; ++t)
#pragma unroll
      for (int r = 0; r < 16; ++r) x[t][r] += elu1(a6[t][r]);
  }
  float vis2;
  {
    f32x16 a7[4];
    acc_init_bias<4>(a7, ctab + 656);
    DYN_PHASE(15);
    net_layer<4, SA_L5_STEPS>(ring, a7, [&](int s) { return x[s / 16][s % 16] * vis; });
    DYN_PHASE(16);
    acc_elu_s(a7);
    vis2 = sigmoid1(row_dot<4>(a7, ctab + 128) + ctab[257]) * msk;
  }
  DYN_PHASE(17);
  const bool tile_ok = tile < p.n_tiles_a;
  if (STORE_X && tile_ok) {
    float4* xw = reinterpret_cast<float4*>(p.ws + p.o.off_x) + tile * 16 * 64 + lane;
#pragma unroll
    for (int t = 0; t < 4; ++t)
#pragma unroll
      for (int q = 0; q < 4; ++q) nt_store4<4>(xw + (t * 4 + q) * 64, make_float4(x[t][q * 4], x[t][q * 4 + 1], x[t][q * 4 + 2], x[t][q * 4 + 3]));
    if (h == 0) nt_store1<4>(p.ws + p.o.off_vis + (tile * 32 + (lane & 31)) * 4, vis2);
  }
  DYN_PHASE(18);
  if constexpr (VSEG == 0) {
    const DenseRows& d = *dr;
    const int tid = threadIdx.x;
    float vsum, nvalid;
    dense_all2(d, vis2, msk, vsum, nvalid);
    const float w2 = vis2 / (vsum + 1e-8f);
    const float wmean = (vsum / (vsum + 1e-8f)) / (float)V;
    constexpr int XS = 132;
    float* tab = lds_base;
    float* wrow = lds_base + 256 * XS;
    const long point0 = d.point0;
    {
      float4* mine = reinterpret_cast<float4*>(tab + d.rw * XS) + h;
#pragma unroll
      for (int t = 0; t < 4; ++t)
#pragma unroll
        for (int q = 0; q < 4; ++q) mine[8 * t + 2 * q] = make_float4(x[t][q * 4], x[t][q * 4 + 1], x[t][q * 4 + 2], x[t][q * 4 + 3]);
      if (h == 0) wrow[d.rw] = w2;
    }
    __syncthreads();
    for (int task = tid; task < d.PTW * 32; task += DYN_VIEW_THREADS) {
      const int pnt = task >> 5, qd = task & 31;
      const int pb = dense_pt_base(d, pnt), pn = dense_pt_cnt(d, pnt);
      const float* src = tab + pb * XS + qd * 4;
      const float* w = wrow + pb;
      float4 m0 = make_float4(0.f, 0.f, 0.f, 0.f), m1 = m0;
      int k = 0;
      for (; k + 2 <= pn; k += 2) {
        const float4 x0 = dense_quad(src, k, XS, pn), x1 = dense_quad(src, k + 1, XS, pn);
        const float w0 = dense_w(w, k, pn), w1 = dense_w(w, k + 1, pn);
        m0.x = fmaf(w0, x0.x, m0.x); m0.y = fmaf(w0, x0.y, m0.y); m0.z = fmaf(w0, x0.z, m0.z); m0.w = fmaf(w0, x0.w, m0.w);
        m1.x = fmaf(w1, x1.x, m1.x); m1.y = fmaf(w1, x1.y, m1.y); m1.z = fmaf(w1, x1.z, m1.z); m1.w = fmaf(w1, x1.w, m1.w);
      }
      if (k < pn) {
        const float4 x0 = dense_quad(src, k, XS, pn);
        const float w0 = dense_w(w, k, pn);
        m0.x = fmaf(w0, x0.x, m0.x); m0.y = fmaf(w0, x0.y, m0.y); m0.z = fmaf(w0, x0.z, m0.z); m0.w = fmaf(w0, x0.w, m0.w);
      }
      const float mean[4] = {m0.x + m1.x, m0.y + m1.y, m0.z + m1.z, m0.w + m1.w};
      float v0[4] = {0.f, 0.f, 0.f, 0.f}, v1[4] = {0.f, 0.f, 0.f, 0.f};
      for (k = 0; k + 2 <= pn; k += 2) {
        const float4 x0 = dense_quad(src, k, XS, pn), x1 = dense_quad(src, k + 1, XS, pn);
        const float w0 = dense_w(w, k, pn), w1 = dense_w(w, k + 1, pn);
        const float a0[4] = {x0.x, x0.y, x0.z, x0.w}, b0[4] = {x1.x, x1.y, x1.z, x1.w};
#pragma unroll
        for (int e = 0; e < 4; ++e) {
          const float d0 = a0[e] - mean[e], d1 = b0[e] - mean[e];
          v0[e] = fmaf(w0, d0 * d0, v0[e]);
          v1[e] = fmaf(w1, d1 * d1, v1[e]);
        }
      }
      if (k < pn) {
        const float4 x0 = dense_quad(src, k, XS, pn);
        const float w0 = dense_w(w, k, pn);
        const float a0[4] = {x0.x, x0.y, x0.z, x0.w};
#pragma unroll
        for (int e = 0; e < 4; ++e) {
          const float d0 = a0[e] - mean[e];
          v0[e] = fmaf(w0, d0 * d0, v0[e]);
        }
      }
      const long pt = point0 + pnt;
      if (pt < p.n_pts) {
        const int g = 4 * (qd >> 3) + ((qd >> 1) & 3);
        float4* gin = reinterpret_cast<float4*>(p.ws + p.o.off_gin) + point_rec(p, pt, qd & 1, SB_GIN_RECS);
        nt_store4<4>(gin + g * 64, make_float4(mean[0], mean[1], mean[2], mean[3]));
        nt_store4<4>(gin + (16 + g) * 64, make_float4(v0[0] + v1[0], v0[1] + v1[1], v0[2] + v1[2], v0[3] + v1[3]));
      }
    }
    if (valid && d.rw == d.base) {
      float4* gin = reinterpret_cast<float4*>(p.ws + p.o.off_gin) + point_rec(p, point, h, SB_GIN_RECS);
      gin[32 * 64] = make_float4(h == 0 ? wmean : 1.0f, 0.f, 0.f, 0.f);
      if (h == 0) p.ws[p.o.off_nvalid + point] = nvalid;
    }
  } else {
  const float w2 = vis2 / (seg_sum<VSEG>(vis2, V, seg_base) + 1e-8f);
  const float wmean = seg_sum<VSEG>(w2, V, seg_base) / (float)V;
  const float nvalid = seg_sum<VSEG>(msk, V, seg_base);
  float4* gin = reinterpret_cast<float4*>(p.ws + p.o.off_gin) + (valid ? point_rec(p, point, h, SB_GIN_RECS) : 0);
#pragma unroll
  for (int t = 0; t < 4; ++t)
#pragma unroll
    for (int q = 0; q < 4; ++q) {
      float m[4], vv[4];
#pragma unroll
      for (int e = 0; e < 4; ++e) m[e] = x[t][q * 4 + e] * w2;
      seg_sum4<VSEG>(m[0], m[1], m[2], m[3]);
#pragma unroll
      for (int e = 0; e < 4; ++e) {
        const float d = x[t][q * 4 + e] - m[e];
        vv[e] = w2 * (d * d);
      }
      seg_sum4<VSEG>(vv[0], vv[1], vv[2], vv[3]);
      const int g = t * 4 + q;
      const int sel = g & (VSEG - 1);
      const bool mine = valid && (view == (sel < V ? sel : 0));
      if (mine) {
        nt_store4<4>(gin + g * 64, make_float4(m[0], m[1], m[2], m[3]));
        nt_store4<4>(gin + (16 + g) * 64, make_float4(vv[0], vv[1], vv[2], vv[3]));
      }
    }
  if (valid && view == 0) {
    gin[32 * 64] = make_float4(h == 0 ? wmean : 1.0f, 0.f, 0.f, 0.f);
    if (h == 0) p.ws[p.o.off_nvalid + point] = nvalid;
  }
  }
}

template <int VSEG, int VC = 0, bool RAG = false>
__global__ void __launch_bounds__(DYN_VIEW_THREADS, 2) k_static_views(StaticArgs p) {
  static_assert(VC == 0 || VSEG == 0, "a compile-time view count is a dense-rows specialisation");
  static_assert(!RAG || VSEG == 0, "ragged rows are a dense-rows flavour");
  if (RAG && (int)blockIdx.x >= p.rg_wg[0]) return;
  constexpr int PHASE_KID = 0;
  (void)PHASE_KID;
  float* lds = reinterpret_cast<float*>(dyn_smem);
  float* ctab = lds + 2 * NET_CHUNK;
  const int tid = threadIdx.x, lane = tid & 63, j = lane & 31, h = lane >> 5, wave = tid >> 6;
  for (int i = tid; i < SA_CT; i += DYN_VIEW_THREADS) ctab[i] = p.blob[ST_OFF_CTA + i];
  NetRing ring;
  DYN_PHASE(0);
  constexpr bool POOLED = VSEG >= 8 || VSEG == 0;
  constexpr int SA_L1P_CHUNKS = net_layer_chunks(8, SA_L1P_STEPS);
  constexpr int SA_POOLED_AT = SA_L1P_CHUNKS + net_layer_chunks(8, SA_L1V_STEPS) + net_layer_chunks(2, SA_L2_STEPS);
  constexpr int LDS_FLOATS = 2 * NET_CHUNK + SA_CT + POOL_FLOATS(SA_NX) + RES_FLOATS + (VSEG == 0 ? DENSE_EXTRA : 0);

  const int V = VC > 0 ? VC : p.V;
  const long tile = (long)blockIdx.x * (DYN_VIEW_THREADS / 64) + wave;
  const DenseRows dr = RAG ? ragged_rows(V, p.rg_rowtab, p.rg_ptab, blockIdx.x, lds + LDS_FLOATS - DENSE_SCALARS, reinterpret_cast<int*>(lds + LDS_FLOATS))
                           : dense_rows(V, VC > 0 ? 256 / VC : p.PT, lds + LDS_FLOATS - DENSE_SCALARS);
  const int PT = RAG ? dr.PTW : (VC > 0 ? 256 / VC : p.PT);
  const int p_local = VSEG == 0 ? dr.p_local : j / (VSEG == 0 ? 1 : VSEG);
  const int view = VSEG == 0 ? dr.view : (j & (VSEG - 1));
  const long point = VSEG == 0 ? dr.point0 + p_local : tile * PT + p_local;
  const bool valid = (VSEG == 0 ? p_local < PT : view < V) && (point < p.n_pts);
  const int seg_base = 0;
  const long pv = valid ? point * V + view : 0;
  net_ring_init(ring, p.blob + ST_OFF_A + (POOLED ? (size_t)SA_L1P_CHUNKS * NET_CHUNK : 0), SA_CHUNKS - (POOLED ? SA_L1P_CHUNKS : 0), lds,
                SA_POOLED_AT - (POOLED ? SA_L1P_CHUNKS : 0), POOLED ? net_layer_chunks(8, SA_L3P_STEPS) : 0, DYN_VIEW_THREADS);

  float msk = valid ? p.mask[pv] : 0.f;
  float4 rd = valid ? reinterpret_cast<const float4*>(p.ray_diff)[pv] : make_float4(0.f, 0.f, 0.f, 0.f);
  float px = 0.f, py = 0.f, pz = 0.f, cx = 0.f, cy = 0.f, cz = 0.f;
  if (valid) {
    px = p.pts[point * 3]; py = p.pts[point * 3 + 1]; pz = p.pts[point * 3 + 2];
    cx = p.centers[view * 16 + 12]; cy = p.centers[view * 16 + 13]; cz = p.centers[view * 16 + 14];
  }
  const int cross_axis = dyn_src_cross_axis(V, p.R, p.S);
  float mq[3] = {0.f, 0.f, 0.f};
  if (cross_axis != DYN_CROSS_XYZ && valid) {
    const int ray = (int)(point / p.S), smp = (int)(point - (long)ray * p.S);
    dyn_src_moment_over_axis(cross_axis, view, ray, smp,
        [&](int, int rr, int ss, float (&q)[3]) { const float* s3 = p.pts + ((long)rr * p.S + ss) * 3; q[0] = s3[0]; q[1] = s3[1]; q[2] = s3[2]; },
        [&](int vv, float (&c3)[3]) { c3[0] = p.centers[vv * 16 + 12]; c3[1] = p.centers[vv * 16 + 13]; c3[2] = p.centers[vv * 16 + 14]; }, mq);
  }
  float xin[SA_NX];
  f32x16 a1[8];
  const bool h0 = h == 0;
  if constexpr (POOLED) {
    B6TileW<SA_L1P_STEPS> pw1;
    b6_tile_prefetch<8, SA_L1P_STEPS>(p.blob + ST_OFF_A, wave, pw1);
    const int npw = VSEG == 0 ? PT : (DYN_VIEW_THREADS / 64) * PT;
    const long qp = VSEG == 0 ? dr.point0 + j : (long)blockIdx.x * npw + j;
    const bool qok = j < npw && qp < p.n_pts;
    const float qx = qok ? p.pts[qp * 3] : 0.f, qy = qok ? p.pts[qp * 3 + 1] : 0.f, qz = qok ? p.pts[qp * 3 + 2] : 0.f;
    float in1p[SA_L1P_STEPS];
    octave_embed<5>(qx, h, in1p);
    octave_embed<5>(qy, h, in1p + 5);
    octave_embed<5>(qz, h, in1p + 10);
    in1p[15] = h0 ? qx : qy;
    in1p[16] = h0 ? qz : 0.f;
    f32x16 accp[1];
    acc_zero(accp);
    b6_tile_apply<SA_L1P_STEPS>(pw1, accp[0], [&](int s) { return in1p[s]; });
    float* res = ctab + SA_CT + POOL_FLOATS(SA_NX);
    res_put(res, wave, j, h, accp[0]);
    __syncthreads();
    res_get(res, VSEG == 0 ? (dr.p_local < dr.PTW ? dr.p_local : dr.PTW - 1) : wave * PT + p_local, h, a1);
  } else {
    float in1p[SA_L1P_STEPS];
    octave_embed<5>(px, h, in1p);
    octave_embed<5>(py, h, in1p + 5);
    octave_embed<5>(pz, h, in1p + 10);
    in1p[15] = h0 ? px : py;
    in1p[16] = h0 ? pz : 0.f;
    acc_zero(a1);
    net_layer<8, SA_L1P_STEPS>(ring, a1, [&](int s) { return in1p[s]; });
  }
  {
    float c6[6];
    unit3(px - cx, py - cy, pz - cz, c6[0], c6[1], c6[2]);
    c6[3] = cy * c6[2] - cz * c6[1];
    c6[4] = cz * c6[0] - cx * c6[2];
    c6[5] = cx * c6[1] - cy * c6[0];
    if (cross_axis != DYN_CROSS_XYZ) { c6[3] = mq[0]; c6[4] = mq[1]; c6[5] = mq[2]; }
    float in1[SA_L1V_STEPS];
#pragma unroll
    for (int c = 0; c < 6; ++c) octave_embed<5>(c6[c], h, in1 + c * 5);
    in1[30] = h0 ? c6[0] : c6[1];
    in1[31] = h0 ? c6[2] : c6[3];
    in1[32] = h0 ? c6[4] : c6[5];
    in1[33] = h0 ? rd.x : rd.y;
    in1[34] = h0 ? rd.z : rd.w;
    in1[35] = DYN_BIAS_ONE(h0 ? 0 : 1);
    DYN_PHASE(1);
    net_layer<8, SA_L1V_STEPS>(ring, a1, [&](int s) { return in1[s]; });
    DYN_PHASE(2);
  }
  {
    f32x16 a2[2];
    acc_init_bias<2>(a2, ctab + 784);
    net_layer<2, SA_L2_STEPS>(ring, a2, [&](int s) {
      if (s == 64) {
#pragma unroll
        for (int q = 0; q < 18; ++q) {
          const int ch = h == 0 ? q : 18 + q;
          xin[q] = (valid && ch < 35) ? nt_load1<2>(p.rgb_feat + pv * 35 + ch) : 0.f;
        }
      }
      return elu_s(a1[s / 16][s % 16]);
    });
    const float* rf = p.ws + p.o.off_ref + (valid ? (point / p.S) * 36 : 0);
#pragma unroll
    for (int r = 0; r < 16; ++r) xin[18 + r] = a2[0][r] * rf[dyn_fi(r, h)];
#pragma unroll
    for (int r = 0; r < 3; ++r) xin[34 + r] = h == 0 ? a2[1][r] * rf[32 + r] : 0.f;
    if (h == 0 && tile < p.n_tiles_a) {
      float* rec = p.ws + p.o.off_vis + (tile * 32 + j) * 4;
      nt_store1<4>(rec + 1, xin[0]); nt_store1<4>(rec + 2, xin[1]); nt_store1<4>(rec + 3, xin[2]);
    }
  }
  DYN_PHASE(4);
  if (p.mask_rgb) {
    const float s3 = (xin[0] + xin[1]) + xin[2];
    msk *= (__shfl(s3, j) > 1e-3f) ? 1.0f : 0.0f;
  }
  float wgt;
  if (p.anti_alias) {
    const float e = ((VSEG == 0 ? p_local < PT : view < V)) ? aa_exp(ctab[258], rd.w) : 3.0e38f;
    const float emin = RAG ? (valid ? p.rg_emin[point] : e) : views_min<VSEG>(dr, e);
    wgt = (e - emin) * msk;
  } else {
    wgt = msk;
  }
  const float wraw = views_sum<VSEG>(dr, wgt);
  wgt = wgt / (wraw + 1e-8f);

  DYN_PHASE(5);
  base_fc0<VSEG, SA_NX>(ring, p.blob + ST_OFF_A + (size_t)SA_POOLED_AT * NET_CHUNK, xin, wgt, V, view, p_local, ctab + SA_CT, a1, &dr, wraw / (wraw + 1e-8f));
  DYN_PHASE(10);
  views_tail<VSEG, true>(ring, a1, p, ctab, wgt, msk, tile, point, valid, view, seg_base, &dr, lds, VC);
  DYN_PHASE(20);
}

#define SB_KL_FLOATS 4096
#define SB_VL_LD 132
#define SB_VL_FLOATS (32 * SB_VL_LD)

__device__ __forceinline__ void lds_barrier() {
#if defined(__AMDGCN__) && DYN_POINTS_DUO
  __builtin_amdgcn_s_waitcnt(0xC07F);
  __builtin_amdgcn_s_barrier();
#else
  __syncthreads();
#endif
}

constexpr int SB_CHUNKS_QKV = pts_layer_chunks(8, 129) + pts_layer_chunks(4, 129) + 3 * pts_layer_chunks(4, 64);
static int dyn_cu_count() {
  static int n_cu[DYN_MAX_DEVICES] = {0};
  int dev = 0;
  (void)hipGetDevice(&dev);
  const int slot = (dev >= 0 && dev < DYN_MAX_DEVICES) ? dev : 0;
  if (n_cu[slot] == 0) {
    hipDeviceProp_t prop;
    n_cu[slot] = (hipGetDeviceProperties(&prop, dev) == hipSuccess && prop.multiProcessorCount > 0) ? prop.multiProcessorCount : 256;
  }
  return n_cu[slot];
}

template <bool DYN, int PHASE>
__global__ void __launch_bounds__(DYN_NET_THREADS, 1) k_net_points(StaticArgs p) {
  constexpr int PHASE_KID = 1;
  (void)PHASE_KID;
  DYN_PHASE(0);
  DYN_CLAIM_REGISTER_FILE();
  float* lds = reinterpret_cast<float*>(dyn_smem);
  float* ctab = lds + PTS_RING_SLOTS * PTS_CHUNK;
  float* Kl = ctab + (DYN ? DB_CT : SB_CT);
  float* Vl = Kl + SB_KL_FLOATS;
  const int tid = threadIdx.x, lane = tid & 63, j = lane & 31, h = lane >> 5, wave = tid >> 6;
  constexpr int CT = DYN ? DB_CT : SB_CT;
  for (int i = tid; i < CT; i += DYN_NET_THREADS) ctab[i] = p.blob[(DYN ? DY_OFF_CTB : ST_OFF_CTB) + i];
  PtsRing ring;
  if (PHASE == 2)
    pts_ring_init(ring, p.blob + (DYN ? DY_OFF_B : ST_OFF_B) + (size_t)SB_CHUNKS_QKV * PTS_CHUNK, (DYN ? DB_CHUNKS : SB_CHUNKS) - SB_CHUNKS_QKV, lds);
  else
    pts_ring_init(ring, p.blob + (DYN ? DY_OFF_B : ST_OFF_B), PHASE == 1 ? SB_CHUNKS_QKV : (DYN ? DB_CHUNKS : SB_CHUNKS), lds);
  DYN_PHASE_RING_KID(ring, 1);
  lds_barrier();

  const int TPR = p.TPR;
  const float one_h0 = DYN_BIAS_ONE(h);
  const long tile = (long)blockIdx.x * 4 + wave;
  const long ray = tile / TPR;
  const int kt_self = (int)(tile - ray * TPR);
  const int smp = kt_self * 32 + j;
  const bool valid = (ray < p.R) && (smp < p.S);
  const long point = valid ? ray * p.S + smp : 0;
  const float nvalid = valid ? p.ws[p.o.off_nvalid + point] : 0.f;

  float4* hand = reinterpret_cast<float4*>(p.ws + p.o.off_qkvg) + (PHASE == 0 ? 0 : tile * 4096) + lane;
  f32x16 g[4];
  if (PHASE == 2) {
    if (ray < p.R) {
#pragma unroll
      for (int t = 0; t < 4; ++t)
#pragma unroll
        for (int q = 0; q < 4; ++q) {
          const float4 v = hand[(t * 4 + q) * 64];
          g[t][q * 4] = v.x; g[t][q * 4 + 1] = v.y; g[t][q * 4 + 2] = v.z; g[t][q * 4 + 3] = v.w;
        }
    } else {
      acc_zero(g);
    }
  } else {
    f32x16 a9[8];
    {
      float gin[129];
      const bool gv = valid;
      const float4* src = reinterpret_cast<const float4*>(p.ws + p.o.off_gin) + (tile < p.n_tiles_b ? tile : 0) * SB_GIN_RECS * 64 + lane;
#pragma unroll
      for (int i = 0; i < 32; ++i) {
        const float4 v = gv ? nt_load4<4>(src + i * 64) : make_float4(0.f, 0.f, 0.f, 0.f);
        gin[i * 4] = v.x; gin[i * 4 + 1] = v.y; gin[i * 4 + 2] = v.z; gin[i * 4 + 3] = v.w;
      }
      gin[128] = gv ? src[32 * 64].x : (h == 1 ? 1.0f : 0.f);
      acc_zero(a9);
      PTS_LAYER(8, 129)(ring, a9, [&](int s) { return gin[s]; });
    }
    acc_zero(g);
    PTS_LAYER(4, 129)(ring, g, [&](int s) { return s < 128 ? elu_s(a9[s / 16][s % 16]) : one_h0; });
    acc_elu(g);
  }
  if (DYN && PHASE != 2) {
    const float4* pe = reinterpret_cast<const float4*>(p.blob + DY_OFF_POSENC + ((valid ? smp : 0) * 2 + h) * 64);
#pragma unroll
    for (int t = 0; t < 4; ++t)
#pragma unroll
      for (int q = 0; q < 4; ++q) {
        const float4 v = pe[t * 4 + q];
        g[t][q * 4] += v.x; g[t][q * 4 + 1] += v.y; g[t][q * 4 + 2] += v.z; g[t][q * 4 + 3] += v.w;
      }
  }
  DYN_PHASE(1);
  f32x16 att[4];
  const float inv_temp = 1.0f / 5.656854249492381f;
  const bool q_ok = nvalid > 1.0f;
  if (PHASE == 2) {
    f32x16 qh[4];
#pragma unroll
    for (int t = 0; t < 4; ++t)
#pragma unroll
      for (int q = 0; q < 4; ++q) {
        const float4 v = hand[(16 + t * 4 + q) * 64];
        qh[t][q * 4] = v.x * inv_temp; qh[t][q * 4 + 1] = v.y * inv_temp; qh[t][q * 4 + 2] = v.z * inv_temp; qh[t][q * 4 + 3] = v.w * inv_temp;
      }
    const float4* ray_hand = reinterpret_cast<const float4*>(p.ws + p.o.off_qkvg) + ray * TPR * 4096;
    const int n_blocks = TPR / 4;
#pragma unroll
    for (int hd = 0; hd < 4; ++hd) {
      float run_max = -3.0e38f, run_sum = 0.f;
      f32x16 oh;
#pragma unroll
      for (int r = 0; r < 16; ++r) oh[r] = 0.f;
      for (int kb = 0; kb < n_blocks; ++kb) {
        __syncthreads();
        {
          const float4* kv = ray_hand + (long)(kb * 4 + wave) * 4096 + lane;
#pragma unroll
          for (int q = 0; q < 4; ++q) {
            reinterpret_cast<float4*>(Kl)[(wave * 4 + q) * 64 + lane] = kv[(32 + hd * 4 + q) * 64];
            const float4 v = kv[(48 + hd * 4 + q) * 64];
            Vl[dyn_fi(q * 4 + 0, h) * SB_VL_LD + wave * 32 + j] = v.x;
            Vl[dyn_fi(q * 4 + 1, h) * SB_VL_LD + wave * 32 + j] = v.y;
            Vl[dyn_fi(q * 4 + 2, h) * SB_VL_LD + wave * 32 + j] = v.z;
            Vl[dyn_fi(q * 4 + 3, h) * SB_VL_LD + wave * 32 + j] = v.w;
          }
        }
        __syncthreads();
        f32x16 sc[4];
        acc_zero(sc);
#pragma unroll
        for (int kt = 0; kt < 4; ++kt)
#pragma unroll
          for (int q = 0; q < 4; ++q) {
            const float4 a = reinterpret_cast<const float4*>(Kl)[(kt * 4 + q) * 64 + lane];
            sc[kt] = mfma32(a.x, qh[hd][q * 4 + 0], sc[kt]);
            sc[kt] = mfma32(a.y, qh[hd][q * 4 + 1], sc[kt]);
            sc[kt] = mfma32(a.z, qh[hd][q * 4 + 2], sc[kt]);
            sc[kt] = mfma32(a.w, qh[hd][q * 4 + 3], sc[kt]);
          }
        float mx = run_max;
#pragma unroll
// ... 739 lines not shown
      }
      const float extra[3] = {h == 0 ? vis2 : rd.x, h == 0 ? rd.y : rd.z, h == 0 ? rd.w : 0.f};
      mlp_layer_b6_lds<4, SC_L11_STEPS>(w11, a, [&](int s) { return s < 64 ? x[s / 16][s % 16] : extra[s - 64]; });
    }
    f32x16 b2[2];
    acc_init_bias<2>(b2, ctab + 80);
    mlp_layer_b6_lds<2, 64>(w12, b2, [&](int s) {
      const float r = elu_s(a[s / 16][s % 16]);
      if (DYN_BLEND_PREFETCH && (s & 15) == 15) load_x(u + step, s / 16);
      return r;
    });
    acc_elu_s(b2);
    float logit = row_dot<2>(b2, ctab) + ctab[64];
    if (msk == 0.f) logit = -1e9f;
    if (VSEG == 0 ? p_local >= PT : view >= V) logit = -3.0e38f;
    const float mx = views_max<VSEG>(dr, logit);
    const float e = (VSEG == 0 && p_local >= PT) ? 0.f : __expf(logit - mx);
    const float bw = e / views_sum<VSEG>(dr, e);
    const bool writer = valid && (VSEG == 0 ? dr.rw == dr.base : view == 0) && h == 0;
    const bool all_masked = RAG && writer && p.ws[p.o.off_nvalid + point] == 0.f;
#pragma unroll
    for (int c = 0; c < 3; ++c) {
      float v = views_sum<VSEG>(dr, rgb_in[c] * bw);
      if (all_masked) {
        const float wv = 1.0f / (float)V;
        v = 0.f;
        for (int k = 0; k < V; ++k) v += p.rgb_feat[(point * V + k) * 35 + c] * wv;
      }
      if (writer) p.raw[point * 4 + c] = v;
    }
  }
}
template <int VSEG>
__global__ void __launch_bounds__(DYN_BLEND_WS_THREADS, 1) k_static_blend_ws(StaticArgs p) { static_blend_ws_body<VSEG, DYN_BLEND_WS_THREADS>(p); }
template <bool RAG>
__global__ void __launch_bounds__(DYN_VIEW_THREADS, 1) k_static_blend_dense_ws(StaticArgs p) { static_blend_ws_body<0, DYN_VIEW_THREADS, RAG>(p); }
#endif

template <int VSEG>
__global__ void __launch_bounds__(DYN_BLEND_THREADS, 3) k_static_blend(StaticArgs p) { static_blend_body<VSEG, DYN_BLEND_THREADS>(p); }
__global__ void __launch_bounds__(DYN_VIEW_THREADS, 1) k_static_blend_dense(StaticArgs p) { static_blend_body<0, DYN_VIEW_THREADS>(p); }


static int ragged_plan(StaticArgs& a, const float* s_abs, hipStream_t stream) {
  unsigned* bits = reinterpret_cast<unsigned*>(a.ws + a.o.off_bits);
  float* emin = a.ws + a.o.off_emin;
  int* seg_cnt = reinterpret_cast<int*>(a.ws + a.o.off_segcnt);
  int* seg_start = reinterpret_cast<int*>(a.ws + a.o.off_segstart);
  int* wg = reinterpret_cast<int*>(a.ws + a.o.off_wgstart);
  unsigned short* rowtab = reinterpret_cast<unsigned short*>(a.ws + a.o.off_rowtab);
  int* ptab = reinterpret_cast<int*>(a.ws + a.o.off_ptab);
  a.rg_bits = bits; a.rg_emin = emin; a.rg_wg = wg; a.rg_rowtab = rowtab; a.rg_ptab = ptab;
  DYN_REQUIRE(a.n_pts < (1L << 31), "ragged plan: R * S must stay below 2^31 points");
  DYN_LAUNCH(DYN_K_STATIC_PLAN, "k_ragged_points", k_ragged_points, dim3(dyn_cdiv(a.n_pts, 256)), dim3(256), (size_t)256 * a.V * 5, stream, a.n_pts, a.V, a.mask,
             reinterpret_cast<const float4*>(a.ray_diff), s_abs, bits, emin);
  DYN_LAUNCH(DYN_K_STATIC_PLAN, "k_ragged_segments", k_ragged_segments, dim3((unsigned)a.o.n_seg), dim3(256), (RAG_SEG + 4 + 256) * sizeof(int) + RAG_SEG * sizeof(unsigned short), stream, a.n_pts, a.o.n_seg, bits, seg_cnt, seg_start);
  DYN_LAUNCH(DYN_K_STATIC_PLAN, "k_ragged_scatter", k_ragged_scatter, dim3(1), dim3(1024), 1028 * sizeof(int), stream, a.n_pts, a.o.n_seg, seg_cnt, seg_start, wg);
  DYN_LAUNCH(DYN_K_STATIC_PLAN, "k_ragged_tables", k_ragged_tables, dim3((unsigned)a.o.n_wg_max), dim3(64), 0, stream, bits, wg, rowtab, ptab);
  return 0;
}

extern "C" int dyn_static_net(const DynStaticNetParams* q, void* stream_) {
  DYN_REQUIRE(q, "dyn_static_net: null params");
  DYN_REQUIRE(q->R > 0 && q->S > 0 && q->V > 0, "dyn_static_net: empty problem");
  DYN_REQUIRE(q->V <= 32, "dyn_static_net: at most 32 source views");
  DYN_REQUIRE(q->S <= DYN_MAX_SAMPLES, "dyn_static_net: at most %d samples per ray", DYN_MAX_SAMPLES);
  DYN_REQUIRE(q->blob && q->ray_o && q->ray_d && q->pts && q->rgb_feat && q->ray_diff && q->mask && q->centers && q->raw && q->workspace,
              "dyn_static_net: null pointer");
  hipStream_t stream = (hipStream_t)stream_;
  StaticArgs a;
  a.R = q->R; a.S = q->S; a.V = q->V;
  a.o = static_ws(q->R, q->S, q->V);
  DYN_REQUIRE(q->workspace_bytes >= a.o.total * sizeof(float), "dyn_static_net: workspace too small (%zu < %zu bytes)", q->workspace_bytes,
              a.o.total * sizeof(float));
  a.PT = a.o.PT; a.TPR = a.o.TPR;
  a.anti_alias = q->anti_alias_pooling; a.mask_rgb = q->mask_rgb;
  a.n_pts = a.o.n_pts; a.n_tiles_a = a.o.n_tiles_a; a.n_tiles_b = a.o.n_tiles_b;
  a.blob = q->blob; a.pts = q->pts; a.rgb_feat = q->rgb_feat; a.ray_diff = q->ray_diff; a.mask = q->mask; a.centers = q->centers;
  a.raw = q->raw; a.ws = (float*)q->workspace;
  a.rg_bits = nullptr; a.rg_emin = nullptr; a.rg_wg = nullptr; a.rg_rowtab = nullptr; a.rg_ptab = nullptr;

  DYN_LAUNCH(DYN_K_STATIC_REF, "k_static_ref_feat", k_static_ref_feat, dim3(dyn_cdiv(q->R, REF_RAYS)), dim3(256), REF_RAYS * 66 * sizeof(float), stream, q->ray_o,
             q->ray_d, q->blob + ST_OFF_REF, q->R, a.ws + a.o.off_ref);
  const dim3 grid_a(dyn_cdiv(a.n_tiles_a, DYN_VIEW_THREADS / 64)), grid_b(dyn_cdiv(a.n_tiles_b, 4)), blk(DYN_NET_THREADS), blk_v(DYN_VIEW_THREADS);
  const size_t lds_a = (2 * NET_CHUNK + SA_CT + POOL_FLOATS(SA_NX) + RES_FLOATS) * sizeof(float);
  const size_t lds_b = (PTS_RING_SLOTS * PTS_CHUNK + SB_CT + SB_KL_FLOATS + SB_VL_FLOATS) * sizeof(float);
  const size_t lds_c = (NET_CHUNK + SC_CT) * sizeof(float);
  const dim3 grid_c(dyn_cdiv(a.n_tiles_a, DYN_BLEND_THREADS / 64)), blk_c(DYN_BLEND_THREADS);
  const size_t lds_rag = (DENSE_EXTRA + RAG_PTAB) * sizeof(float);
  if (a.o.ragged) {
    const int rc = ragged_plan(a, a.anti_alias ? a.blob + ST_OFF_CTA + 258 : nullptr, stream);
    if (rc != 0) return rc;
  }
  if (a.o.ragged && a.V == 11) DYN_LAUNCH(DYN_K_STATIC_VIEWS, "k_static_views", (k_static_views<0, 11, true>), grid_a, blk_v, lds_a + lds_rag, stream, a);
  else if (a.o.ragged) DYN_LAUNCH(DYN_K_STATIC_VIEWS, "k_static_views", (k_static_views<0, 0, true>), grid_a, blk_v, lds_a + lds_rag, stream, a);
  else if (a.o.dense && a.V == 11) DYN_LAUNCH(DYN_K_STATIC_VIEWS, "k_static_views", (k_static_views<0, 11>), grid_a, blk_v, lds_a + DENSE_EXTRA * sizeof(float), stream, a);
  else if (a.o.dense) DYN_LAUNCH(DYN_K_STATIC_VIEWS, "k_static_views", k_static_views<0>, grid_a, blk_v, lds_a + DENSE_EXTRA * sizeof(float), stream, a);
  else if (q->V <= 4) DYN_LAUNCH(DYN_K_STATIC_VIEWS, "k_static_views", k_static_views<4>, grid_a, blk_v, lds_a, stream, a);
  else if (q->V <= 8) DYN_LAUNCH(DYN_K_STATIC_VIEWS, "k_static_views", k_static_views<8>, grid_a, blk_v, lds_a, stream, a);
  else if (q->V <= 16) DYN_LAUNCH(DYN_K_STATIC_VIEWS, "k_static_views", k_static_views<16>, grid_a, blk_v, lds_a, stream, a);
  else DYN_LAUNCH(DYN_K_STATIC_VIEWS, "k_static_views", k_static_views<32>, grid_a, blk_v, lds_a, stream, a);
  if (a.TPR <= 4) {
#if DYN_POINTS_DUO
    const dim3 grid_b8(dyn_cdiv(a.n_tiles_b, DYN_VIEW_THREADS / 64));
    const size_t lds_b8 = (PTS_RING_SLOTS * PTS_CHUNK + SB_CT + SB8_KV_FLOATS) * sizeof(float);
    if (a.TPR <= 2) DYN_LAUNCH(DYN_K_STATIC_POINTS, "k_static_points", (k_net_points_w8<false, 2>), grid_b8, blk_v, lds_b8, stream, a);
    else DYN_LAUNCH(DYN_K_STATIC_POINTS, "k_static_points", (k_net_points_w8<false, 4>), grid_b8, blk_v, lds_b8, stream, a);
#else
    DYN_LAUNCH(DYN_K_STATIC_POINTS, "k_static_points", (k_net_points<false, 0>), grid_b, blk, lds_b, stream, a);
#endif
  } else {
    DYN_LAUNCH(DYN_K_STATIC_POINTS_QKV, "k_static_points_qkv", (k_net_points<false, 1>), grid_b, blk, lds_b, stream, a);
    DYN_LAUNCH(DYN_K_STATIC_POINTS, "k_static_points", (k_net_points<false, 2>), grid_b, blk, lds_b, stream, a);
  }
#if DYN_BLEND_WS
  static const int blend_stream = getenv("DYN_BLEND_STREAM") != nullptr;
  if (!blend_stream) {
    const size_t lds_w = (SC_WS_FLOATS + SC_CT + DENSE_SCALARS + RAG_PTAB) * sizeof(float);
    const unsigned n_cu = (unsigned)dyn_cu_count();
    if (a.o.dense) {
      const unsigned nb = (unsigned)dyn_cdiv(a.n_tiles_a, DYN_VIEW_THREADS / 64);
      if (a.o.ragged) DYN_LAUNCH(DYN_K_STATIC_BLEND, "k_static_blend", k_static_blend_dense_ws<true>, dim3(nb < n_cu ? nb : n_cu), blk_v, lds_w, stream, a);
      else DYN_LAUNCH(DYN_K_STATIC_BLEND, "k_static_blend", k_static_blend_dense_ws<false>, dim3(nb < n_cu ? nb : n_cu), blk_v, lds_w, stream, a);
    } else {
      const unsigned nb = (unsigned)dyn_cdiv(a.n_tiles_a, DYN_BLEND_WS_THREADS / 64);
      const dim3 gw(nb < n_cu ? nb : n_cu), bw_(DYN_BLEND_WS_THREADS);
      if (q->V <= 4) DYN_LAUNCH(DYN_K_STATIC_BLEND, "k_static_blend", k_static_blend_ws<4>, gw, bw_, lds_w, stream, a);
      else if (q->V <= 8) DYN_LAUNCH(DYN_K_STATIC_BLEND, "k_static_blend", k_static_blend_ws<8>, gw, bw_, lds_w, stream, a);
      else if (q->V <= 16) DYN_LAUNCH(DYN_K_STATIC_BLEND, "k_static_blend", k_static_blend_ws<16>, gw, bw_, lds_w, stream, a);
      else DYN_LAUNCH(DYN_K_STATIC_BLEND, "k_static_blend", k_static_blend_ws<32>, gw, bw_, lds_w, stream, a);
    }
    return 0;
  }
#endif
  if (a.o.dense) DYN_LAUNCH(DYN_K_STATIC_BLEND, "k_static_blend", k_static_blend_dense, grid_a, blk_v, lds_c + DENSE_SCALARS * sizeof(float), stream, a);
  else if (q->V <= 4) DYN_LAUNCH(DYN_K_STATIC_BLEND, "k_static_blend", k_static_blend<4>, grid_c, blk_c, lds_c, stream, a);
  else if (q->V <= 8) DYN_LAUNCH(DYN_K_STATIC_BLEND, "k_static_blend", k_static_blend<8>, grid_c, blk_c, lds_c, stream, a);
  else if (q->V <= 16) DYN_LAUNCH(DYN_K_STATIC_BLEND, "k_static_blend", k_static_blend<16>, grid_c, blk_c, lds_c, stream, a);
  else DYN_LAUNCH(DYN_K_STATIC_BLEND, "k_static_blend", k_static_blend<32>, grid_c, blk_c, lds_c, stream, a);
  return 0;
}

extern "C" size_t dyn_dynamic_net_blob_floats(void) { return DY_BLOB_FLOATS; }

extern "C" int dyn_dynamic_net_pack(const float* const* T, int F, float* blob, size_t blob_floats) {
  DYN_REQUIRE(T && blob, "dyn_dynamic_net_pack: null pointer");
  DYN_REQUIRE(F == 32, "dyn_dynamic_net_pack: the kernels are specialised for 32 feature channels");
  DYN_REQUIRE(blob_floats >= DY_BLOB_FLOATS, "dyn_dynamic_net_pack: blob too small");
  for (int i = 0; i < DT_NUM_TENSORS; ++i) DYN_REQUIRE(T[i] != nullptr, "dyn_dynamic_net_pack: tensor %d is NULL", i);
  std::vector<float> o;
  g_pack_range_error = false;
  g_pack_slot_error = false;
  o.reserve(DY_BLOB_FLOATS);
  {
    const float *W = T[DT_BASE0_W], *b = T[DT_BASE0_B];
    pack_net_layer(o, 8, DA_L3P_STEPS, scaled([=](int t, int i, int s, int h) -> float {
      const int c = da_c35(s % DA_NX, h);
      return c < 0 ? 0.f : W[(32 * t + i) * 105 + (s / DA_NX) * 35 + c];
    }, DYN_ELU_PRE));
    pack_net_layer(o, 8, DA_L3V_STEPS, scaled([=](int t, int i, int s, int h) -> float {
      const int n = 32 * t + i;
      if (s == DA_NX) return h == 0 ? b[n] : 0.f;
      const int c = da_c35(s, h);
      return c < 0 ? 0.f : W[n * 105 + 70 + c];
    }, DYN_ELU_PRE), DA_NX);
  }
  pack_net_layer(o, 4, SA_L4_STEPS, scaled(chained(T[DT_BASE2_W], nullptr, 128, 256, 256), DYN_ELU_POST));
  pack_net_layer(o, 4, SA_L5_STEPS, scaled(chained(T[DT_VIS0_W], nullptr, 128, 128, 128), DYN_ELU_PRE));
  pack_net_layer(o, 4, SA_L5_STEPS, scaled(chained(T[DT_VIS2_W], nullptr, 128, 128, 128), DYN_ELU_POST));
  pack_net_layer(o, 4, SA_L5_STEPS, scaled(chained(T[DT_VISB0_W], nullptr, 128, 128, 128), DYN_ELU_PRE));
  DYN_REQUIRE(o.size() == DY_OFF_B, "dynamic pack: A stream size mismatch");
  const auto pack_b = [&](bool by_head) {
#if DYN_POINTS_DUO
  g_pack_chunk_pairs = PTS_CP;
#endif
  {
    const float *W = T[DT_GEO0_W], *b = T[DT_GEO0_B];
    pack_net_layer(o, 8, 129, scaled([=](int t, int i, int s, int h) -> float {
      const int n = 32 * t + i;
      if (s < 128) return W[n * 257 + (s < 64 ? 0 : 128) + chain_feature(s % 64, h)];
      return h == 0 ? W[n * 257 + 256] : b[n];
    }, DYN_ELU_PRE));
  }
  pack_net_layer(o, 4, 129, scaled_wb(chained(T[DT_GEO2_W], T[DT_GEO2_B], 128, 256, 256), 128, DYN_ELU_POST, 1.0), 128);
  if (by_head) {
    pack_qkv_by_head(o, T[DT_WQ], T[DT_WK], T[DT_WV]);
  } else {
    pack_net_layer(o, 4, 64, chained(T[DT_WQ], nullptr, 128, 128, 128));
    pack_net_layer(o, 4, 64, chained(T[DT_WK], nullptr, 128, 128, 128));
    pack_net_layer(o, 4, 64, chained(T[DT_WV], nullptr, 128, 128, 128));
  }
  pack_net_layer(o, 4, 64, chained(T[DT_FC], nullptr, 128, 128, 128));
  {
    const float *W = T[DT_REFPTS0_W], *b = T[DT_REFPTS0_B];
    pack_net_layer(o, 8, 81, scaled([=](int t, int i, int s, int h) -> float {
      const int n = 32 * t + i;
      if (s < 64) return W[n * 161 + chain_feature(s, h)];
      if (s < 79) { const int c = (s - 64) / 5, f = (s - 64) % 5; return W[n * 161 + 128 + 3 + (h * 5 + f) * 3 + c]; }
      if (s == 79) return W[n * 161 + 128 + h];
      return h == 0 ? W[n * 161 + 128 + 2] : b[n];
    }, DYN_ELU_PRE));
  }
  pack_net_layer(o, 4, 129, scaled_wb(chained(T[DT_REFPTS2_W], T[DT_REFPTS2_B], 128, 256, 256), 128, DYN_ELU_POST, 1.0), 128);
  pack_net_layer(o, 4, 65, scaled(chained(T[DT_OG0_W], T[DT_OG0_B], 128, 128, 128), DYN_ELU_PRE), 64);
  {
    const float *W = T[DT_RGB0_W], *b = T[DT_RGB0_B];
    pack_net_layer(o, 4, 78, scaled([=](int t, int i, int s, int h) -> float {
      const int n = 32 * t + i;
      if (s < 64) return W[n * 155 + chain_feature(s, h)];
      if (s < 76) { const int c = (s - 64) / 4, f = (s - 64) % 4; return W[n * 155 + 128 + 3 + (h * 4 + f) * 3 + c]; }
      if (s == 76) return W[n * 155 + 128 + h];
      return h == 0 ? W[n * 155 + 128 + 2] : b[n];
    }, DYN_ELU_PRE));
  }
  pack_net_layer(o, 2, 65, scaled_wb(chained(T[DT_RGB2_W], T[DT_RGB2_B], 64, 128, 128), 64, DYN_ELU_POST * DYN_ELU_PRE, DYN_ELU_PRE), 64);
  g_pack_chunk_pairs = B6_CHUNK_PAIRS;
  };
  pack_b(false);
  DYN_REQUIRE(o.size() == DY_OFF_CTA, "dynamic pack: B stream size mismatch");
  pack_rowtab(o, T[DT_VIS2_W] + 128 * 128, 128, DYN_ELU_POST);
  pack_rowtab(o, T[DT_VISB2_W], 128, DYN_ELU_POST);
  o.push_back(T[DT_VIS2_B][128]);
  o.push_back(T[DT_VISB2_B][0]);
  o.resize(DY_OFF_CTA + 272, 0.f);
  pack_rowtab(o, T[DT_BASE2_B], 128);
  pack_rowtab(o, T[DT_VIS0_B], 128, DYN_ELU_PRE);
  pack_rowtab(o, T[DT_VIS2_B], 128);
  pack_rowtab(o, T[DT_VISB0_B], 128, DYN_ELU_PRE);
  o.resize(DY_OFF_CTB, 0.f);
  pack_rowtab(o, T[DT_LN_G], 128);
  pack_rowtab(o, T[DT_LN_B], 128);
  pack_rowtab(o, T[DT_OG2_W], 128, DYN_ELU_POST);
  o.push_back(T[DT_OG2_B][0]);
  for (int c = 0; c < 3; ++c) o.push_back(T[DT_RGB4_B][c]);
  o.resize(DY_OFF_CTB + 400, 0.f);
  for (int c = 0; c < 3; ++c) pack_rowtab(o, T[DT_RGB4_W] + c * 64, 64, DYN_ELU_POST);
  o.resize(DY_OFF_POSENC, 0.f);
  for (int pos = 0; pos < DYN_MAX_SAMPLES; ++pos)
    for (int h = 0; h < 2; ++h)
      for (int k = 0; k < 64; ++k) {
        const int f = chain_feature(k, h);
        const double ang = (double)pos / pow(10000.0, 2.0 * (f / 2) / 128.0);
        o.push_back((float)((f % 2 == 0) ? sin(ang) : cos(ang)));
      }
  for (int i = 0; i < 256 * 21; ++i) o.push_back(T[DT_RAYDIR0_W][i]);
  for (int i = 0; i < 256; ++i) o.push_back(T[DT_RAYDIR0_B][i]);
  for (int i = 0; i < 35 * 256; ++i) o.push_back(T[DT_RAYDIR2_W][i]);
  for (int i = 0; i < 35; ++i) o.push_back(T[DT_RAYDIR2_B][i]);
  o.resize(DY_OFF_B8, 0.f);
#if DYN_POINTS_DUO
  pack_b(true);
#endif
  DYN_REQUIRE(o.size() == DY_BLOB_FLOATS, "dynamic pack: B8 stream size mismatch");
  DYN_REQUIRE(!g_pack_slot_error, "dyn_dynamic_net_pack: a layer's bias slot carries a weight in its second half (the one-product build stores the bias residual there)");
  DYN_REQUIRE(!g_pack_range_error, "dyn_dynamic_net_pack: a weight is outside the half-float range of the split engine (|w| >= 65504 or not finite)");
  for (size_t i = 0; i < DY_BLOB_FLOATS; ++i) blob[i] = o[i];
  return 0;
}

extern "C" size_t dyn_dynamic_net_workspace_bytes(int R, int S, int V) {
  if (R <= 0 || S <= 0 || V <= 0 || V > 32) return 0;
  return static_ws(R, S, V, true).total * sizeof(float);
}

__global__ void __launch_bounds__(256) k_dynamic_time_feat(const float* __restrict__ Wt, const float* __restrict__ time, float* __restrict__ out) {
  float* hid = reinterpret_cast<float*>(dyn_smem);
  const int tid = threadIdx.x;
  const float t = time[0];
  float pe[21];
  pe[0] = t;
  for (int f = 0; f < 10; ++f) {
    const float a = (float)(1 << f) * t;
    pe[1 + f] = cosf(a);
    pe[11 + f] = sinf(a);
  }
  {
    const float* w = Wt + tid * 21;
    float acc = Wt[256 * 21 + tid];
    for (int k = 0; k < 21; ++k) acc = fmaf(w[k], pe[k], acc);
    hid[tid] = acc > 0.f ? acc : expm1f(acc);
  }
  __syncthreads();
  if (tid < 35) {
    const float* w = Wt + 256 * 21 + 256 + tid * 256;
    float acc = Wt[256 * 21 + 256 + 35 * 256 + tid];
    for (int k = 0; k < 256; ++k) acc = fmaf(w[k], hid[k], acc);
    out[tid] = acc > 0.f ? acc : expm1f(acc);
  } else if (tid < 36) {
    out[tid] = 0.f;
  }
}

template <int VSEG, bool RAG = false>
__global__ void __launch_bounds__(DYN_VIEW_THREADS, 2) k_dynamic_views(StaticArgs p) {
  static_assert(!RAG || VSEG == 0, "ragged rows are a dense-rows flavour");
  if (RAG && (int)blockIdx.x >= p.rg_wg[0]) return;
  float* lds = reinterpret_cast<float*>(dyn_smem);
  float* ctab = lds + 2 * NET_CHUNK;
  const int tid = threadIdx.x, lane = tid & 63, j = lane & 31, h = lane >> 5, wave = tid >> 6;
  for (int i = tid; i < SA_CT; i += DYN_VIEW_THREADS) ctab[i] = p.blob[DY_OFF_CTA + i];
  NetRing ring;
  constexpr int LDS_FLOATS = 2 * NET_CHUNK + SA_CT + POOL_FLOATS(SA_NX) + RES_FLOATS + (VSEG == 0 ? DENSE_EXTRA : 0);
  net_ring_init(ring, p.blob + DY_OFF_A, DA_CHUNKS, lds, 0, (VSEG >= 8 || VSEG == 0) ? net_layer_chunks(8, DA_L3P_STEPS) : 0, DYN_VIEW_THREADS);

  const int V = p.V;
  const long tile = (long)blockIdx.x * (DYN_VIEW_THREADS / 64) + wave;
  const DenseRows dr = RAG ? ragged_rows(V, p.rg_rowtab, p.rg_ptab, blockIdx.x, lds + LDS_FLOATS - DENSE_SCALARS, reinterpret_cast<int*>(lds + LDS_FLOATS))
                           : dense_rows(V, p.PT, lds + LDS_FLOATS - DENSE_SCALARS);
  const int PT = RAG ? dr.PTW : p.PT;
  const int p_local = VSEG == 0 ? dr.p_local : j / (VSEG == 0 ? 1 : VSEG);
  const int view = VSEG == 0 ? dr.view : (j & (VSEG - 1));
  const long point = VSEG == 0 ? dr.point0 + p_local : tile * PT + p_local;
  const bool valid = (VSEG == 0 ? p_local < PT : view < V) && (point < p.n_pts);
  const int seg_base = 0;
  const long pv = valid ? point * V + view : 0;
  const float msk = valid ? p.mask[pv] : 0.f;
  const float* tf = p.ws + p.o.off_ref;
  float xin[DA_NX];
#pragma unroll
  for (int q = 0; q < DA_NX; ++q) {
    const int ch = h == 0 ? q : 18 + q;
    xin[q] = (valid && ch < 35) ? nt_load1<2>(p.rgb_feat + pv * 35 + ch) + tf[ch] : 0.f;
  }
  const float wraw = views_sum<VSEG>(dr, msk);
  const float wgt = msk / (wraw + 1e-8f);
  f32x16 a1[8];
  base_fc0<VSEG, DA_NX>(ring, p.blob + DY_OFF_A, xin, wgt, V, view, p_local, ctab + SA_CT, a1, &dr, wraw / (wraw + 1e-8f));
  views_tail<VSEG, false>(ring, a1, p, ctab, wgt, msk, tile, point, valid, view, seg_base, &dr, lds);
}

extern "C" int dyn_dynamic_net(const DynDynamicNetParams* q, void* stream_) {
  DYN_REQUIRE(q, "dyn_dynamic_net: null params");
  DYN_REQUIRE(q->R > 0 && q->S > 0 && q->V > 0, "dyn_dynamic_net: empty problem");
  DYN_REQUIRE(q->V <= 32, "dyn_dynamic_net: at most 32 source views");
  DYN_REQUIRE(q->S <= DYN_MAX_SAMPLES, "dyn_dynamic_net: at most %d samples per ray", DYN_MAX_SAMPLES);
  DYN_REQUIRE(q->blob && q->ray_d && q->pts && q->rgb_feat && q->mask && q->time && q->raw && q->workspace, "dyn_dynamic_net: null pointer");
  hipStream_t stream = (hipStream_t)stream_;
  StaticArgs a;
  a.R = q->R; a.S = q->S; a.V = q->V;
  a.o = static_ws(q->R, q->S, q->V, true);
  DYN_REQUIRE(q->workspace_bytes >= a.o.total * sizeof(float), "dyn_dynamic_net: workspace too small (%zu < %zu bytes)", q->workspace_bytes,
              a.o.total * sizeof(float));
  a.PT = a.o.PT; a.TPR = a.o.TPR;
  a.anti_alias = 0; a.mask_rgb = 0;
  a.n_pts = a.o.n_pts; a.n_tiles_a = a.o.n_tiles_a; a.n_tiles_b = a.o.n_tiles_b;
  a.shift = q->shift;
  a.blob = q->blob; a.ray_d = q->ray_d; a.pts = q->pts; a.rgb_feat = q->rgb_feat; a.ray_diff = nullptr; a.mask = q->mask; a.centers = nullptr;
  a.raw = q->raw; a.ws = (float*)q->workspace;
  a.rg_bits = nullptr; a.rg_emin = nullptr; a.rg_wg = nullptr; a.rg_rowtab = nullptr; a.rg_ptab = nullptr;
  DYN_LAUNCH(DYN_K_DYNAMIC_TIME, "k_dynamic_time_feat", k_dynamic_time_feat, dim3(1), dim3(256), 256 * sizeof(float), stream,
             q->blob + DY_OFF_TIME, q->time, a.ws + a.o.off_ref);
  const dim3 grid_a(dyn_cdiv(a.n_tiles_a, DYN_VIEW_THREADS / 64)), grid_b(dyn_cdiv(a.n_tiles_b, 4)), blk(DYN_NET_THREADS), blk_v(DYN_VIEW_THREADS);
  const size_t lds_a = (2 * NET_CHUNK + SA_CT + POOL_FLOATS(SA_NX) + RES_FLOATS) * sizeof(float);
  const size_t lds_b = (PTS_RING_SLOTS * PTS_CHUNK + DB_CT + SB_KL_FLOATS + SB_VL_FLOATS) * sizeof(float);
  if (a.o.ragged) {
    const int rc = ragged_plan(a, nullptr, stream);
    if (rc != 0) return rc;
    DYN_LAUNCH(DYN_K_DYNAMIC_VIEWS, "k_dynamic_views", (k_dynamic_views<0, true>), grid_a, blk_v, lds_a + (DENSE_EXTRA + RAG_PTAB) * sizeof(float), stream, a);
  } else if (a.o.dense) DYN_LAUNCH(DYN_K_DYNAMIC_VIEWS, "k_dynamic_views", k_dynamic_views<0>, grid_a, blk_v, lds_a + DENSE_EXTRA * sizeof(float), stream, a);
  else if (q->V <= 4) DYN_LAUNCH(DYN_K_DYNAMIC_VIEWS, "k_dynamic_views", k_dynamic_views<4>, grid_a, blk_v, lds_a, stream, a);
  else if (q->V <= 8) DYN_LAUNCH(DYN_K_DYNAMIC_VIEWS, "k_dynamic_views", k_dynamic_views<8>, grid_a, blk_v, lds_a, stream, a);
  else if (q->V <= 16) DYN_LAUNCH(DYN_K_DYNAMIC_VIEWS, "k_dynamic_views", k_dynamic_views<16>, grid_a, blk_v, lds_a, stream, a);
  else DYN_LAUNCH(DYN_K_DYNAMIC_VIEWS, "k_dynamic_views", k_dynamic_views<32>, grid_a, blk_v, lds_a, stream, a);
  if (a.TPR <= 4) {
#if DYN_POINTS_DUO
    const dim3 grid_b8(dyn_cdiv(a.n_tiles_b, DYN_VIEW_THREADS / 64));
    const size_t lds_b8 = (PTS_RING_SLOTS * PTS_CHUNK + DB_CT + SB8_KV_FLOATS) * sizeof(float);
    if (a.TPR <= 2) DYN_LAUNCH(DYN_K_DYNAMIC_POINTS, "k_dynamic_points", (k_net_points_w8<true, 2>), grid_b8, blk_v, lds_b8, stream, a);
    else DYN_LAUNCH(DYN_K_DYNAMIC_POINTS, "k_dynamic_points", (k_net_points_w8<true, 4>), grid_b8, blk_v, lds_b8, stream, a);
#else
    DYN_LAUNCH(DYN_K_DYNAMIC_POINTS, "k_dynamic_points", (k_net_points<true, 0>), grid_b, blk, lds_b, stream, a);
#endif
  } else {
    DYN_LAUNCH(DYN_K_DYNAMIC_POINTS_QKV, "k_dynamic_points_qkv", (k_net_points<true, 1>), grid_b, blk, lds_b, stream, a);
    DYN_LAUNCH(DYN_K_DYNAMIC_POINTS, "k_dynamic_points", (k_net_points<true, 2>), grid_b, blk, lds_b, stream, a);
  }
  return 0;
}

enum { MT_L0_W, MT_L0_B, MT_L1_W, MT_L1_B, MT_L2_W, MT_L2_B, MT_L3_W, MT_L3_B, MT_L4_W, MT_L4_B, MT_L5_W, MT_L5_B, MT_L6_W, MT_L6_B, MT_L7_W,
       MT_L7_B, MT_COEFF_W, MT_COEFF_B, MT_NUM_TENSORS };
#define MO_PE_STEPS 66
constexpr int MO_CHUNKS = net_layer_chunks(8, MO_PE_STEPS + 1) + 4 * net_layer_chunks(8, 129) + net_layer_chunks(8, MO_PE_STEPS + 129) +
                          2 * net_layer_chunks(8, 129) + net_layer_chunks(1, 129);
constexpr size_t MO_OFF_FREQ = (size_t)MO_CHUNKS * NET_CHUNK;
constexpr size_t MO_BLOB_FLOATS = MO_OFF_FREQ + 16;

extern "C" size_t dyn_motion_mlp_blob_floats(void) { return MO_BLOB_FLOATS; }

static int mo_pe_col(int s, int h) {
  if (s < 64) { const int c = s / 16, f = s % 16; return 4 + (h * 16 + f) * 4 + c; }
  return (s - 64) * 2 + h;
}

extern "C" int dyn_motion_mlp_pack(const float* const* T, int num_basis, float* blob, size_t blob_floats) {
  DYN_REQUIRE(T && blob, "dyn_motion_mlp_pack: null pointer");
  DYN_REQUIRE(num_basis >= 1 && 3 * num_basis <= 32, "dyn_motion_mlp_pack: 3 * num_basis must be at most 32");
  DYN_REQUIRE(blob_floats >= MO_BLOB_FLOATS, "dyn_motion_mlp_pack: blob too small");
  for (int i = 0; i < MT_NUM_TENSORS; ++i) DYN_REQUIRE(T[i] != nullptr, "dyn_motion_mlp_pack: tensor %d is NULL", i);
  std::vector<float> o;
  g_pack_range_error = false;
  g_pack_slot_error = false;
  o.reserve(MO_BLOB_FLOATS);
  {
    const float *W = T[MT_L0_W], *b = T[MT_L0_B];
    pack_net_layer(o, 8, MO_PE_STEPS + 1, [=](int t, int i, int s, int h) -> float {
      const int n = 32 * t + i;
      if (s < MO_PE_STEPS) return W[n * 132 + mo_pe_col(s, h)];
      return h == 0 ? b[n] : 0.f;
    }, MO_PE_STEPS);
  }
  for (int l = 1; l <= 4; ++l) pack_net_layer(o, 8, 129, chained(T[MT_L0_W + 2 * l], T[MT_L0_B + 2 * l], 256, 256, 256), 128);
  {
    const float *W = T[MT_L5_W], *b = T[MT_L5_B];
    pack_net_layer(o, 8, MO_PE_STEPS + 129, [=](int t, int i, int s, int h) -> float {
      const int n = 32 * t + i;
      if (s < MO_PE_STEPS) return W[n * 388 + mo_pe_col(s, h)];
      const int s2 = s - MO_PE_STEPS;
      if (s2 < 128) return W[n * 388 + 132 + chain_feature(s2, h)];
      return h == 0 ? b[n] : 0.f;
    }, MO_PE_STEPS + 128);
  }
  pack_net_layer(o, 8, 129, chained(T[MT_L6_W], T[MT_L6_B], 256, 256, 256), 128);
  pack_net_layer(o, 8, 129, chained(T[MT_L7_W], T[MT_L7_B], 256, 256, 256), 128);
  pack_net_layer(o, 1, 129, chained(T[MT_COEFF_W], T[MT_COEFF_B], 3 * num_basis, 256, 256), 128);
  DYN_REQUIRE(o.size() == MO_OFF_FREQ, "motion pack: stream size mismatch");
  {
    const float step = (17.0f - 1.0f) / 15.0f;
    for (int i = 0; i < 16; ++i) o.push_back(i < 8 ? 1.0f + (float)i * step : 17.0f - (float)(15 - i) * step);
  }
  DYN_REQUIRE(!g_pack_slot_error, "dyn_motion_mlp_pack: a layer's bias slot carries a weight in its second half (the one-product build stores the bias residual there)");
  DYN_REQUIRE(!g_pack_range_error, "dyn_motion_mlp_pack: a weight is outside the half-float range of the split engine (|w| >= 65504 or not finite)");
  for (size_t i = 0; i < MO_BLOB_FLOATS; ++i) blob[i] = o[i];
  return 0;
}

__device__ __attribute__((noinline)) float sin_or_cos_huge(float x, int want_sin) { return want_sin ? sinf(x) : cosf(x); }

__device__ __forceinline__ void motion_embed(const float (&c4)[4], const float* __restrict__ freq, int h, float (&pe)[MO_PE_STEPS]) {
#pragma unroll
  for (int c = 0; c < 4; ++c)
#pragma unroll
    for (int f = 0; f < 16; ++f) {
      float sn, cs;
      const float arg = freq[f] * c4[c];
      sincos_small(arg, sn, cs);
      float v = h == 0 ? cs : sn;
      if (__builtin_expect(fabsf(arg) > 1.0e6f, 0)) v = sin_or_cos_huge(arg, h);
      pe[c * 16 + f] = v;
    }
  pe[64] = h == 0 ? c4[0] : c4[1];
  pe[65] = h == 0 ? c4[2] : c4[3];
}

#ifndef DYN_MOTION_DUO
#define DYN_MOTION_DUO 1
#endif
#if DYN_MOTION_DUO
typedef WeightRing3 MotionRing;
#define MOTION_RING_SLOTS B6D_SLOTS
#define motion_ring_init(R, stream, total, lds) ring3_init(R, stream, total, lds, DYN_NET_THREADS)
#define motion_layer mlp_layer_b6_duo
#else
typedef NetRing MotionRing;
#define MOTION_RING_SLOTS 2
#define motion_ring_init(R, stream, total, lds) net_ring_init_t(R, stream, total, lds, DYN_NET_THREADS)
#define motion_layer net_layer
#endif

__global__ void __launch_bounds__(256) k_motion_zero_tail(long R, int S, int n_zero_last, int n_out, float* __restrict__ coeff) {
  const long i = (long)blockIdx.x * blockDim.x + threadIdx.x;
  const long per_ray = (long)n_zero_last * n_out;
  if (i >= R * per_ray) return;
  const long ray = i / per_ray;
  coeff[(ray * S + (S - n_zero_last)) * n_out + (i - ray * per_ray)] = 0.f;
}

__global__ void __launch_bounds__(DYN_NET_THREADS, 1)
k_motion_mlp(const float* __restrict__ blob, const float* __restrict__ pts, const float* __restrict__ time, long n_kept, int S, int n_zero_last,
             int n_out, float inv_div, float* __restrict__ coeff) {
  DYN_CLAIM_REGISTER_FILE();
  float* lds = reinterpret_cast<float*>(dyn_smem);
  const int tid = threadIdx.x, lane = tid & 63, j = lane & 31, h = lane >> 5, wave = tid >> 6;
  MotionRing ring;
  motion_ring_init(ring, blob, MO_CHUNKS, lds);
  const long row = ((long)blockIdx.x * 4 + wave) * 32 + j;
  const bool valid = row < n_kept;
  const int Sk = S - n_zero_last;
  const long ray = (valid ? row : 0) / Sk;
  const long point = ray * S + ((valid ? row : 0) - ray * Sk);
  float c4[4] = {0.f, 0.f, 0.f, time[0]};
  if (valid) { c4[0] = pts[point * 3]; c4[1] = pts[point * 3 + 1]; c4[2] = pts[point * 3 + 2]; }
  const float* freq = blob + MO_OFF_FREQ;
  const float one_h0 = DYN_BIAS_ONE(h);
  f32x16 a[8], b[8];
  float pe[MO_PE_STEPS];
  motion_embed(c4, freq, h, pe);
  acc_zero(a);
  motion_layer<8, MO_PE_STEPS + 1>(ring, a, [&](int s) { return s < MO_PE_STEPS ? pe[s] : one_h0; });
  acc_zero(b);
  motion_layer<8, 129>(ring, b, [&](int s) { return s < 128 ? relu1(a[s / 16][s % 16]) : one_h0; });
  acc_zero(a);
  motion_layer<8, 129>(ring, a, [&](int s) { return s < 128 ? relu1(b[s / 16][s % 16]) : one_h0; });
  acc_zero(b);
  motion_layer<8, 129>(ring, b, [&](int s) { return s < 128 ? relu1(a[s / 16][s % 16]) : one_h0; });
  acc_zero(a);
  motion_layer<8, 129>(ring, a, [&](int s) { return s < 128 ? relu1(b[s / 16][s % 16]) : one_h0; });
  acc_zero(b);
  motion_layer<8, MO_PE_STEPS + 129>(ring, b, [&](int s) {
    if (s < MO_PE_STEPS) return pe[s];
    return s - MO_PE_STEPS < 128 ? relu1(a[(s - MO_PE_STEPS) / 16][(s - MO_PE_STEPS) % 16]) : one_h0;
  });
  acc_zero(a);
  motion_layer<8, 129>(ring, a, [&](int s) { return s < 128 ? relu1(b[s / 16][s % 16]) : one_h0; });
  acc_zero(b);
  motion_layer<8, 129>(ring, b, [&](int s) { return s < 128 ? relu1(a[s / 16][s % 16]) : one_h0; });
  f32x16 c1[1];
  acc_zero(c1);
  motion_layer<1, 129>(ring, c1, [&](int s) { return s < 128 ? relu1(b[s / 16][s % 16]) : one_h0; });
  if (valid) {
#pragma unroll
    for (int r = 0; r < 16; ++r) {
      const int f = dyn_fi(r, h);
      if (f < n_out) coeff[point * n_out + f] = c1[0][r] * inv_div;
    }
  }
}

extern "C" int dyn_motion_mlp(const float* blob, const float* pts, const float* time, int R, int S, int num_basis, int n_zero_last,
                              float sf_mag_div, float* coeff, void* stream) {
  DYN_REQUIRE(blob && pts && time && coeff, "dyn_motion_mlp: null pointer");
  DYN_REQUIRE(R > 0 && S > 0 && num_basis >= 1 && 3 * num_basis <= 32 && n_zero_last >= 0 && sf_mag_div != 0.f, "dyn_motion_mlp: bad argument");
  const int nz = n_zero_last < S ? n_zero_last : S;
  const long n_kept = (long)R * (S - nz);
  if (n_kept > 0)
    DYN_LAUNCH(DYN_K_MOTION_MLP, "k_motion_mlp", k_motion_mlp, dim3(dyn_cdiv(n_kept, 128)), dim3(DYN_NET_THREADS), MOTION_RING_SLOTS * NET_CHUNK * sizeof(float),
               (hipStream_t)stream, blob, pts, time, n_kept, S, nz, 3 * num_basis, 1.0f / sf_mag_div, coeff);
  if (nz > 0)
    DYN_LAUNCH(DYN_K_MOTION_TAIL, "k_motion_zero_tail", k_motion_zero_tail, dim3(dyn_cdiv((long)R * nz * 3 * num_basis, 256)), dim3(256), 0, (hipStream_t)stream, (long)R, S, nz,
               3 * num_basis, coeff);
  return 0;
}

extern "C" int dyn_mlp_split_terms(void) {
  return DYN_SPLIT_TERMS;
}
extern "C" int dyn_mlp_split_kind(void) {
#if DYN_SPLIT_F16
  return 2;
#else
  return 1;
#endif
}

__global__ void __launch_bounds__(DYN_NET_THREADS, 2) k_selftest(const float* __restrict__ stream, const float* __restrict__ x, float* __restrict__ y,
                                                                  int rows) {
  float* lds = reinterpret_cast<float*>(dyn_smem);
  const int lane = threadIdx.x & 63, j = lane & 31, h = lane >> 5, wave = threadIdx.x >> 6;
  NetRing ring;
  net_ring_init_t(ring, stream, 2 * net_layer_chunks(2, 33), lds, DYN_NET_THREADS);
  const int row = (blockIdx.x * 4 + wave) * 32 + j;
  f32x16 in[2];
#pragma unroll
  for (int s = 0; s < 32; ++s) in[s / 16][s % 16] = row < rows ? x[row * 64 + 32 * (s / 16) + dyn_fi(s % 16, h)] : 0.f;
  const float one_h0 = DYN_BIAS_ONE(h);
#pragma unroll
  for (int rep = 0; rep < 2; ++rep) {
    f32x16 acc[2];
    acc_zero(acc);
    net_layer<2, 33>(ring, acc, [&](int s) { return s < 32 ? in[s / 16][s % 16] : one_h0; });
    acc_elu(acc);
    in[0] = acc[0];
    in[1] = acc[1];
  }
  if (row < rows)
#pragma unroll
    for (int s = 0; s < 32; ++s) y[row * 64 + 32 * (s / 16) + dyn_fi(s % 16, h)] = in[s / 16][s % 16];
}

extern "C" int dyn_mlp_selftest(const float* W, const float* b, const float* x, float* y, int rows, float* stream_buf, void* stream) {
  DYN_REQUIRE(W && b && x && y && stream_buf && rows > 0, "dyn_mlp_selftest: bad argument");
  std::vector<float> o;
  pack_net_layer(o, 2, 33, chained(W, b, 64, 64, 64), 32);
  pack_net_layer(o, 2, 33, chained(W, b, 64, 64, 64), 32);
  if (hipMemcpy(stream_buf, o.data(), o.size() * sizeof(float), hipMemcpyHostToDevice) != hipSuccess) {
    dyn_set_error("dyn_mlp_selftest: hipMemcpy failed");
    return DYN_E_LAUNCH;
  }
  DYN_LAUNCH(DYN_K_SELFTEST, "k_selftest", k_selftest, dim3(dyn_cdiv(rows, 128)), dim3(DYN_NET_THREADS), 2 * NET_CHUNK * sizeof(float),
             (hipStream_t)stream, stream_buf, x, y, rows);
  return 0;
}
```

include/dynibar_hip.h:

```cpp
#ifndef DYNIBAR_HIP_H_
#define DYNIBAR_HIP_H_
#include <stddef.h>
#include <stdint.h>

#ifdef __cplusplus
extern "C" {
#endif

#define DYN_ABI_VERSION 1
#define DYN_E_INVALID (-1)
#define DYN_E_LAUNCH (-2)

int dyn_abi_version(void);
const char* dyn_last_error(void);

int dyn_prepare_cameras(const float* cams, int V, const float* query_cam, float* proj, float* query_center, void* stream);

int dyn_nchw_to_nhwc(const float* src, float* dst, int V, int F, int Hf, int Wf, void* stream);

typedef struct {
  int R, S;
  int inv_uniform;
  const float* ray_o;
  const float* ray_d;
// ... 11 lines not shown
typedef struct {
  int R, S, V;
  int H, W;
  int Hf, Wf, F;
  float img_h, img_w;
  const float* ray_o;
  const float* ray_d;
  const float* z_vals;
  const float* pts_st;
  const float* xyz;
  const float* proj;
  const float* query_center;
  const float* src_rgb;
  const float* feat_cl;
  float* rgb_feat;
  float* ray_diff;
  float* mask;
  float* pix_mask;
  float pix_mask_thresh;
  const float* traj_coeff;
  const float* traj_basis;
  const int* traj_rows;
  int traj_B, traj_ref;
} DynProjectGatherParams;
int dyn_project_gather(const DynProjectGatherParams* p, void* stream);

typedef struct {
  int R, S;
  const float* raw_dy;
  const float* raw_static;
  const float* z_vals;
  const float* pix_mask_dy;
  const float* pix_mask_st;
  float* rgb;
  float* rgb_static;
  float* rgb_dy;
  float* depth;
  float* ray_mask;
  float* weights;
  float* alpha;
  float* alpha_dy;
  float* weights_dy;
  float* weights_st;
} DynCompositeParams;
int dyn_composite(const DynCompositeParams* p, void* stream);

int dyn_sample_mask(const float* mask, int RS, int V, float thresh, float* pix_mask, void* stream);

typedef struct {
  int R, S, N;
  int inv_uniform;
  const float* z_vals;
  const float* weights;
  const float* u;
  float* z_out;
  float* z_samples;
  int32_t* inds;
} DynFineSampleParams;
int dyn_fine_samples(const DynFineSampleParams* p, void* stream);

#define DYN_STATIC_NUM_TENSORS 39
size_t dyn_static_net_blob_floats(void);
int dyn_static_net_pack(const float* const* tensors, int F, float* blob, size_t blob_floats);
size_t dyn_static_net_workspace_bytes(int R, int S, int V);
typedef struct {
  int R, S, V;
  int anti_alias_pooling;
  int mask_rgb;
  const float* blob;
  const float* ray_o;
  const float* ray_d;
  const float* pts;
  const float* rgb_feat;
  const float* ray_diff;
  const float* mask;
  const float* centers;
  float* raw;
  void* workspace;
  size_t workspace_bytes;
} DynStaticNetParams;
int dyn_static_net(const DynStaticNetParams* p, void* stream);

#define DYN_DYNAMIC_NUM_TENSORS 40
size_t dyn_dynamic_net_blob_floats(void);
int dyn_dynamic_net_pack(const float* const* tensors, int F, float* blob, size_t blob_floats);
size_t dyn_dynamic_net_workspace_bytes(int R, int S, int V);
typedef struct {
  int R, S, V;
  float shift;
  const float* blob;
  const float* ray_d;
  const float* pts;
  const float* rgb_feat;
  const float* mask;
  const float* time;
  float* raw;
  void* workspace;
  size_t workspace_bytes;
} DynDynamicNetParams;
int dyn_dynamic_net(const DynDynamicNetParams* p, void* stream);

#define DYN_MOTION_NUM_TENSORS 18
size_t dyn_motion_mlp_blob_floats(void);
int dyn_motion_mlp_pack(const float* const* tensors, int num_basis, float* blob, size_t blob_floats);
int dyn_motion_mlp(const float* blob, const float* pts, const float* time, int R, int S, int num_basis, int n_zero_last, float sf_mag_div,
                   float* coeff, void* stream);

int dyn_trajectory_points(const float* coeff, const float* basis, const float* pts, long n_pts, int B, const int* rows, int n_rows, int row_ref,
                          float* pts_seq, void* stream);

int dyn_render_flows(const float* weights, const float* pts_seq, const float* proj, const float* uv, int R, int S, int V, float* flows,
                     void* stream);
int dyn_render_flows_traj(const float* weights, const float* pts, const float* coeff, const float* basis, int B, const int* rows_dev, int row_ref,
                          const float* proj, const float* uv, int R, int S, int V, float* flows, void* stream);
int dyn_expected_scene_flow(const float* weights, const float* coeff, const float* basis, int R, int S, int B, int row_p, int row_m, int row_ref,
                            float* exp_sf, void* stream);
int dyn_image_rays(const float* camera, int H, int W, int render_stride, float* rays_o, float* rays_d, void* stream);

int dyn_sample_pdf(const float* bins, float* weights, const float* u, int R, int M, int N, float* samples, void* stream);
int dyn_plucker_ref(const float* ray_o, const float* ray_d, int R, float* out, void* stream);
int dyn_plucker_src(const float* pts, int per_view_pts, const float* cams, int R, int S, int V, float* out, void* stream);
int dyn_project_points(const float* xyz, const float* xyz_st, const float* proj, const float* query_center, int V, long n_pts, float* pix,
                       float* in_front, float* ray_diff, void* stream);

size_t dyn_encoder_blob_floats(void);
int dyn_encoder_pack(const float* const* tensors, float* blob, size_t blob_floats);
size_t dyn_encoder_workspace_bytes(int N, int H, int W);
int dyn_encoder_out_size(int H, int W, int* Hf, int* Wf);
typedef struct {
  int N, H, W;
  const float* blob;
  const float* images;
  float* coarse;
  float* fine;
  void* workspace;
  size_t workspace_bytes;
} DynEncoderParams;
int dyn_encoder_forward(const DynEncoderParams* p, void* stream);

int dyn_enc_im2col(const float* in, int N, int Hin, int Win, int C, int KH, int KW, int stride, int pad, int Hout, int Wout, float* col, long ldc,
                   void* stream);
int dyn_enc_col2im(const float* dcol, long ldc, int N, int Hin, int Win, int C, int KH, int KW, int stride, int pad, int Hout, int Wout, float* din,
                   void* stream);
int dyn_enc_in_stats(const float* x, int N, long HW, double* stats, void* stream);
int dyn_enc_in_apply(const float* x, const double* stats, const float* gamma, const float* beta, const float* res, int relu, int N, long HW, float* y,
                     void* stream);
int dyn_enc_in_bwd(const float* dy, const float* y, int relu, const float* x, const double* stats, const float* gamma, int N, long HW, double* sums2,
                   float* dx, float* dres, float* dgamma, float* dbeta, void* stream);

int dyn_mlp_split_terms(void);
int dyn_mlp_split_kind(void);

int dyn_mlp_selftest(const float* W, const float* b, const float* x, float* y, int rows, float* stream_buf, void* stream);

int dyn_profile_enable(int on);
int dyn_profile_count(void);
const char* dyn_profile_name(int slot);
int dyn_profile_read(float* total_ms, int* launches);


typedef struct {
  const float* A;
  long a_rs, a_ks;
  const float* B;
  long b_rs, b_ks;
  float* C;
  long ldc;
  int M, N, K;
  const float* bias;
  const float* addend;
  long ld_add;
  int add_div;
  int act;
  int accumulate;
  int k_split;
  const float* a_absmax;
  const float* act_y;
  long ld_y;
  int act_y_kind;
  float* colsum_part;
  long ld_part;
  float* amax_part;
  const float* rowscale;
  const float* kscale;
} DynTrainGemmParams;
int dyn_train_gemm(const DynTrainGemmParams* p, void* stream);
int dyn_train_gemm_mode(int mode);
int dyn_train_colsum_reduce(const float* colsum_part, long tiles, int N, long ld_part, float* dbias, const float* amax_part, long n_amax,
                            float* absmax, void* stream);

int dyn_train_act_bwd(float* dY, const float* Y, long rows, int cols, long ld_dy, long ld_y, int act, float* dbias, int seg, float* dseg,
                      long ld_seg, float* absmax, void* stream);
int dyn_train_absmax(const float* x, long rows, int cols, long ld, float* absmax, void* stream);

int dyn_train_static_embed(const float* pts, const float* ray_o, const float* ray_d, const float* centers, int center_stride,
                           const float* ray_diff, const float* rgb_feat, const float* mask, int R, int S, int V, int mask_rgb, float* a0,
                           float* ref_pe, float* mask_eff, void* stream);

int dyn_train_build_f(const float* rgb_feat, const float* src_feat, long ld_src, const float* ref_feat, long ld_ref, long N, int rows_per_ray,
                      float* f, void* stream);
int dyn_train_build_f_bwd(const float* df, long ld_df, const float* src_feat, long ld_src, const float* ref_feat, long ld_ref, long R,
                          int rows_per_ray, float* dsrc, long ld_dsrc, float* dref, long ld_dref, void* stream);

int dyn_train_view_weights(int mode, const float* in, long in_stride, const float* mask, const float* s_param, long P, int V, float* w,
                           float* vis_out, long vis_stride, float* wmean, long wmean_stride, float* nvalid, void* stream);
int dyn_train_view_weights_bwd(int mode, const float* in, long in_stride, const float* mask, const float* s_param, long P, int V,
                               const float* w, const float* dw, const float* dvis_direct, long dvis_stride, const float* vis, long vis_stride,
                               const float* dwmean, long dwmean_stride, float* dlogit, long dlogit_stride, float* ds, void* stream);

int dyn_train_meanvar(const float* x, long ldx, const float* w, long P, int V, int C, float* mean, float* var, long ld_out, void* stream);
int dyn_train_meanvar_bwd(const float* x, long ldx, const float* w, long P, int V, int C, const float* mean, const float* dmean,
                          const float* dvar, long ld_stat, float* dx, long ld_dx, int accumulate, float* dw, int dw_accumulate, void* stream);

int dyn_train_rowscale(const float* x, long ldx, const float* s, long s_stride, long N, int C, float* y, long ldy, void* stream);
int dyn_train_rowscale_bwd(const float* dy, long ld_dy, const float* x, long ldx, const float* s, long s_stride, long N, int C, float* dx,
                           long ld_dx, int accumulate, float* ds, long ds_stride, int ds_accumulate, void* stream);

int dyn_train_vis_split(const float* x1, long ld1, const float* xv, long ldv, const float* mask, const float* ray_diff, long N, float* x2,
                        long ld2, float* vis0, void* stream);
int dyn_train_vis_split_bwd(const float* dx2, long ld_dx2, const float* dvis0, const float* xv, long ldv, const float* mask, long N, float* dxv,
                            long ld_dxv, void* stream);
int dyn_train_rowscale_act_bwd(const float* dy, long ld_dy, const float* x, long ldx, const float* s, long s_stride, long N, float* dx,
                               long ld_dx, float* ds, long ds_stride, int ds_accumulate, int act, float* dbias, float* absmax, void* stream);
int dyn_train_vis_split_act_bwd(float* dx2, long ld_dx2, const float* dvis0, const float* xv, long ldv, const float* mask, long N, float* dxv,
                                long ld_dxv, float* dbias, float* absmax, const float* dxs, long ld_dxs, const float* x2, long ldx2,
                                const float* vis0, void* stream);
int dyn_train_rowdot(const float* X, long ldx, const float* w, const float* bias, long N, int C, float* y, long y_stride, void* stream);
int dyn_train_outer_act_bwd(const float* dz, long dz_stride, const float* w, const float* Y, long ld_y, long N, int C, int act, float* dX,
                            long ld_dx, float* dbias, float* absmax, float* dW, void* stream);

int dyn_train_attn(const float* qkv, const float* nvalid, int R, int S, float* out, float* prob, void* stream);
int dyn_train_attn_bwd(const float* qkv, const float* nvalid, int R, int S, const float* prob, const float* dout, float* dscore, float* dqkv,
                       void* stream);

int dyn_train_layernorm(const float* a, const float* b, const float* gamma, const float* beta, long P, float* out, float* xhat, float* rstd,
                        void* stream);
int dyn_train_layernorm_bwd(const float* dout, const float* xhat, const float* rstd, const float* gamma, long P, float* din, float* dgamma,
                            float* dbeta, void* stream);

int dyn_train_blend(const float* logit, long logit_stride, const float* mask, const float* rgb_feat, const float* sigma, long sigma_stride,
                    const float* nvalid, long P, int V, float* blend, float* raw, void* stream);
int dyn_train_blend_bwd(const float* draw, const float* blend, const float* mask, const float* rgb_feat, const float* nvalid, long P, int V,
                        float* dlogit, long dlogit_stride, float* dsigma, long dsigma_stride, void* stream);

int dyn_train_composite_bwd(const float* raw, const float* z_vals, const float* alpha, const float* weights, const float* drgb,
                            const float* ddepth, const float* dweights, int R, int S, float* draw, void* stream);

int dyn_gather_bwd(const float* pts_st, const float* xyz, const float* proj, int R, int S, int V, int Hf, int Wf, int F, float img_h, float img_w,
                   const float* drgb_feat, long ld_d, int col0, float* dfeat_cl, void* stream);


int dyn_train_add_table(const float* x, long ldx, const float* tab, long ld_tab, int period, long rows, int C, float* y, long ldy, void* stream);

int dyn_train_dynamic_embed(const float* pts, const float* ray_d, long P, int R, float* pts_pe, float* dir_pe, void* stream);

int dyn_train_dynamic_head(const float* logit, long ld_logit, const float* sigma, const float* nvalid, float shift, long P, float* raw, void* stream);
int dyn_train_dynamic_head_bwd(const float* draw, const float* raw, const float* nvalid, long P, float* dlogit, long ld_dlogit, float* dsigma,
                               void* stream);

int dyn_train_composite2_bwd(const float* raw_dy, const float* raw_st, const float* z_vals, const float* g_rgb, const float* g_rgb_st,
                             const float* g_rgb_dy, const float* g_depth, const float* g_wd, const float* g_ws, const float* g_w, int R, int S,
                             float* draw_dy, float* draw_st, void* stream);


int dyn_train_embed(const float* x, long ldx, long rows, int D, const float* freqs, int n_freqs, float* out, long ld, void* stream);
int dyn_train_embed_bwd(const float* x, long ldx, long rows, int D, const float* freqs, int n_freqs, const float* dout, long ld, float* dx, long ld_dx,
                        int accumulate, void* stream);

int dyn_train_zero_tail(float* x, long R, int S, int C, int n_last, float scale, void* stream);

int dyn_trajectory_bwd(const float* dseq, const float* coeff, const float* basis, long n_pts, int B, const int* rows, int n_rows, int row_ref,
                       float* dcoeff, float* dbasis, float* dpts, void* stream);

int dyn_render_flows_bwd(const float* dflows, const float* weights, const float* pts_seq, const float* proj, int R, int S, int V, float* dweights,
                         float* dseq, void* stream);

int dyn_gather_bwd_pts(const float* pts_st, const float* xyz, const float* proj, const float* src_rgb, const float* feat_cl, int R, int S, int V,
                       int H, int W, int Hf, int Wf, int F, float img_h, float img_w, const float* drgb_feat, long ld_d, float* dxyz, void* stream);

int dyn_comm_available(void);
int dyn_comm_unique_id(void* id128);
int dyn_comm_init_rank(void** comm, int nranks, const void* id128, int rank);
int dyn_comm_size_rank(void* comm, int* nranks, int* rank);
int dyn_comm_destroy(void* comm);
int dyn_gather_tiles(const float* send, float* recv, long rows_per_rank, int cols, void* comm, void* stream);

size_t dyn_splat_workspace_bytes(int B, int H, int W);
typedef struct {
  int B, C, H, W;
  const float* frame;
  const float* flow;
  const float* multiplier;
  int normalize;
  float eps;
  float* out;
  void* workspace;
  size_t workspace_bytes;
} DynSplatParams;
int dyn_splat(const DynSplatParams* p, void* stream);

typedef struct {
  int B, H, W, C;
  const float* src;
  const float* depth;
  const float* k_src_inv;
  const float* rot;
// ... 128 lines not shown
```

Baseline: 1.535 million.

## Pack view-net weights as a dense chunk stream without per-layer padding

```diff
diff --git a/dynibar_amd/csrc/dyn_mlp.h b/dynibar_amd/csrc/dyn_mlp.h
--- a/dynibar_amd/csrc/dyn_mlp.h
+++ b/dynibar_amd/csrc/dyn_mlp.h
@@ -226,6 +226,7 @@
 struct WeightRing6 {
   const float* gbase;
   float* buf;
+  const float* cur;
   int next, total;
   int skip_at, skip_n;
   int round;
@@ -278,13 +279,14 @@
 #ifndef B6_FEED_STATELESS
 #define B6_FEED_STATELESS (DYN_SPLIT_TERMS == 1 ? 1 : 0)
 #endif
+template <bool STATELESS = (B6_FEED_STATELESS != 0)>
 __device__ __forceinline__ void ring6_feed(WeightRing6& R, int pr, int npc) {
   if (R.fill < 0) return;
   const int n = ring6_pieces(R);
   const int den = (B6_DMA_WINDOW_NUM * npc + B6_DMA_WINDOW_DEN - 1) / B6_DMA_WINDOW_DEN > 0 ? (B6_DMA_WINDOW_NUM * npc + B6_DMA_WINDOW_DEN - 1) / B6_DMA_WINDOW_DEN : 1;
   int want = (n * (pr + 1) + den - 1) / den;
   if (want > n) want = n;
-#if B6_FEED_STATELESS
+  if constexpr (STATELESS) {
   int prev = (n * pr + den - 1) / den;
   if (prev > n) prev = n;
 #pragma unroll
@@ -292,9 +294,9 @@
     if (k >= prev && k < want) ring6_piece(R, k);
   for (int k = prev > 12 ? prev : 12; k < want; ++k) ring6_piece(R, k);
   R.issued = want;
-#else
+  } else {
   for (; R.issued < want; ++R.issued) ring6_piece(R, R.issued);
-#endif
+  }
 }
 
 __device__ __forceinline__ void ring6_issue(const WeightRing6& R, int chunk) {
@@ -319,6 +321,7 @@
                                            int threads = 0, int nbuf = 2) {
   R.gbase = stream;
   R.buf = lds;
+  R.cur = lds;
   R.next = 0;
   R.total = total - skip_n;
   R.skip_at = skip_at;
@@ -357,6 +360,7 @@
     __builtin_amdgcn_s_waitcnt(0x0F70);
     __syncthreads();
     DYN_PHASE_WAIT(R, c);
+    R.cur = R.buf;
     return R.buf;
   }
   if (R.fill >= 0) {
@@ -380,7 +384,17 @@
   DYN_PHASE_WAIT(R, c);
   R.fill = c + 1 < R.total ? c + 1 : -1;
   R.issued = 0;
-  return R.buf + (c & 1) * B6_CHUNK;
+  R.cur = R.buf + (c & 1) * B6_CHUNK;
+  return R.cur;
+}
+__device__ __forceinline__ void b6_lds_sync() {
+#if defined(__AMDGCN__)
+  __builtin_amdgcn_fence(__ATOMIC_RELEASE, "workgroup", "local");
+  __builtin_amdgcn_s_barrier();
+  __builtin_amdgcn_fence(__ATOMIC_ACQUIRE, "workgroup", "local");
+#else
+  __syncthreads();
+#endif
 }
 
 #ifndef B6_PRIO_FLIP
@@ -447,6 +461,8 @@
 __host__ __device__ constexpr int b6_layer_chunks(int NT, int NSLOTS, int CP = B6_CHUNK_PAIRS) {
   return (((NSLOTS + 7) / 8) + (CP / NT) - 1) / (CP / NT);
 }
+__host__ __device__ constexpr int b6_layer_pairs(int NT, int NSLOTS) { return ((NSLOTS + 7) / 8) * NT; }
+__host__ __device__ constexpr int b6_dense_chunks(int pairs, int CP = B6_CHUNK_PAIRS) { return (pairs + CP - 1) / CP; }
 
 struct B6A {
   u32x4v hi, mid, lo;
@@ -464,6 +480,42 @@
   return a;
 }
 
+struct B6ChunkBase {
+#if defined(__AMDGCN__)
+  unsigned addr;
+#else
+  const float* p;
+#endif
+};
+__device__ __forceinline__ B6ChunkBase b6_chunk_base(const float* buf, int lane) {
+  B6ChunkBase b;
+#if defined(__AMDGCN__)
+  b.addr = (unsigned)(size_t)(const __attribute__((address_space(3))) void*)(reinterpret_cast<const u32x4v*>(buf) + lane);
+  asm volatile("" : "+v"(b.addr));
+#else
+  b.p = buf;
+  (void)lane;
+#endif
+  return b;
+}
+__device__ __forceinline__ B6A b6_load_a(const B6ChunkBase& b, int i, int lane) {
+#if defined(__AMDGCN__)
+  (void)lane;
+  const __attribute__((address_space(3))) u32x4v* w = (const __attribute__((address_space(3))) u32x4v*)b.addr + i * (B6_PAIR_FLOATS / 4);
+  B6A a;
+  a.hi = w[0];
+#if DYN_SPLIT_PARTS >= 2
+  a.mid = w[64];
+#endif
+#if DYN_SPLIT_PARTS == 3
+  a.lo = w[128];
+#endif
+  return a;
+#else
+  return b6_load_a(b.p + i * B6_PAIR_FLOATS, lane);
+#endif
+}
+
 template <int NSLOTS, int P0, int P1, class Feed>
 __device__ __forceinline__ void b6_split_pairs(Feed& feed, int g, u32x4v& bh, u32x4v& bm, u32x4v& bl) {
 #pragma unroll
@@ -479,18 +531,80 @@
 #ifndef B6_AHEAD
 #define B6_AHEAD 1
 #endif
-template <int NT, int NSLOTS, int AHEAD = B6_AHEAD, class Feed>
+template <int NT, int NSLOTS, class Feed>
+__device__ __forceinline__ void b6_split_share(Feed& feed, int g, int t, u32x4v& nh, u32x4v& nm, u32x4v& nl) {
+  if (NT == 1) b6_split_pairs<NSLOTS, 0, 4>(feed, g, nh, nm, nl);
+  if (NT == 2 && t == 0) b6_split_pairs<NSLOTS, 0, 2>(feed, g, nh, nm, nl);
+  if (NT == 2 && t == 1) b6_split_pairs<NSLOTS, 2, 4>(feed, g, nh, nm, nl);
+  if (NT == 4 && t == 0) b6_split_pairs<NSLOTS, 0, 1>(feed, g, nh, nm, nl);
+  if (NT == 4 && t == 1) b6_split_pairs<NSLOTS, 1, 2>(feed, g, nh, nm, nl);
+  if (NT == 4 && t == 2) b6_split_pairs<NSLOTS, 2, 3>(feed, g, nh, nm, nl);
+  if (NT == 4 && t == 3) b6_split_pairs<NSLOTS, 3, 4>(feed, g, nh, nm, nl);
+  if (NT == 8 && t == 0) b6_split_pairs<NSLOTS, 0, 1>(feed, g, nh, nm, nl);
+  if (NT == 8 && t == 2) b6_split_pairs<NSLOTS, 1, 2>(feed, g, nh, nm, nl);
+  if (NT == 8 && t == 4) b6_split_pairs<NSLOTS, 2, 3>(feed, g, nh, nm, nl);
+  if (NT == 8 && t == 6) b6_split_pairs<NSLOTS, 3, 4>(feed, g, nh, nm, nl);
+}
+template <int NT, int NSLOTS, int AHEAD = B6_AHEAD, int START = 0, bool DENSE = (START != 0), class Feed>
 __device__ __forceinline__ void mlp_layer_b6(WeightRing6& R, f32x16 (&acc)[NT], Feed&& feed) {
   constexpr int NG = (NSLOTS + 7) / 8;
   constexpr int GPC = B6_CHUNK_PAIRS / NT;
   constexpr int NCH = (NG + GPC - 1) / GPC;
-  static_assert(B6_CHUNK_PAIRS % NT == 0, "tiles per layer must divide the pairs of a chunk");
+  static_assert(DENSE || B6_CHUNK_PAIRS % NT == 0, "tiles per layer must divide the pairs of a chunk");
+  static_assert(DENSE || START == 0, "a layer of an aligned stream begins a chunk");
   static_assert(NT == 1 || NT == 2 || NT == 4 || NT == 8, "output tiles per layer");
   const int lane = threadIdx.x & 63;
   u32x4v bh, bm, bl, nh, nm, nl;
   b6_split_pairs<NSLOTS, 0, 4>(feed, 0, bh, bm, bl);
   nh = bh; nm = bm; nl = bl;
   __builtin_amdgcn_sched_barrier(0);
+  if constexpr (DENSE) {
+    constexpr int CP = B6_CHUNK_PAIRS, NP = NG * NT, C0 = START % CP;
+    static_assert(START >= 0 && AHEAD >= 1 && AHEAD < CP, "stream position / look-ahead");
+    B6ChunkBase buf = b6_chunk_base(R.cur, lane);
+    B6A q[AHEAD + 1];
+    if (C0 != 0) {
+#pragma unroll
+      for (int i = 0; i < AHEAD; ++i)
+        if (i < NP && C0 + i < CP) q[i] = b6_load_a(buf, C0 + i, lane);
+      __builtin_amdgcn_sched_barrier(0);
+    }
+#pragma unroll
+    for (int g = 0; g < NG; ++g) {
+#pragma unroll
+    for (int t = 0; t < NT; ++t) {
+      const int pr = g * NT + t;
+      const int cr = (START + pr) % CP;
+      if (cr == 0) {
+        buf = b6_chunk_base(ring6_acquire(R), lane);
+#pragma unroll
+        for (int i = 0; i < AHEAD; ++i)
+          if (pr + i < NP) q[(pr + i) % (AHEAD + 1)] = b6_load_a(buf, i, lane);
+        __builtin_amdgcn_sched_barrier(0);
+      }
+      ring6_feed<true>(R, cr, CP);
+#if B6_PRIO_FLIP && (B6_PRIO_MODE == 1 || B6_PRIO_MODE == 5)
+      if (cr % B6_PRIO_FLIP == 0) ring6_prio_flip(R, (cr / B6_PRIO_FLIP) & 1);
+#endif
+      if (pr + AHEAD < NP && cr + AHEAD < CP) q[(pr + AHEAD) % (AHEAD + 1)] = b6_load_a(buf, cr + AHEAD, lane);
+      if (g + 1 < NG) b6_split_share<NT, NSLOTS>(feed, g + 1, t, nh, nm, nl);
+      const B6A& cur = q[pr % (AHEAD + 1)];
+#if DYN_SPLIT_TERMS == 6
+      acc[t] = mfma_bf16(cur.lo, bh, acc[t]);
+      acc[t] = mfma_bf16(cur.hi, bl, acc[t]);
+      acc[t] = mfma_bf16(cur.mid, bm, acc[t]);
+#endif
+#if DYN_SPLIT_TERMS != 1
+      acc[t] = mfma_bf16(cur.mid, bh, acc[t]);
+      acc[t] = mfma_bf16(cur.hi, bm, acc[t]);
+#endif
+      acc[t] = mfma_bf16(cur.hi, bh, acc[t]);
+      if (t == NT - 1) { bh = nh; bm = nm; bl = nl; }
+      __builtin_amdgcn_sched_barrier(0);
+    }
+    }
+    return;
+  }
 #pragma unroll
   for (int c = 0; c < NCH; ++c) {
     const float* buf = ring6_acquire(R);
diff --git a/dynibar_amd/csrc/dyn_nets.hip b/dynibar_amd/csrc/dyn_nets.hip
--- a/dynibar_amd/csrc/dyn_nets.hip
+++ b/dynibar_amd/csrc/dyn_nets.hip
@@ -15,6 +15,21 @@
 
 thread_local bool g_pack_slot_error = false;
 thread_local int g_pack_chunk_pairs = B6_CHUNK_PAIRS;
+void pack_pair_b6(unsigned short* img, int NSLOTS, int g, int t, const SlotFn& fn, int ones_slot) {
+  for (int lane = 0; lane < 64; ++lane)
+    for (int e = 0; e < 8; ++e) {
+      const int s = g * 8 + e;
+      if (s >= NSLOTS) continue;
+      const bool two_half_bias = DYN_SPLIT_PARTS == 1 && s == ones_slot;
+      if (two_half_bias && fn(t, lane & 31, s, 1) != 0.f) g_pack_slot_error = true;
+      const float w = fn(t, lane & 31, s, two_half_bias ? 0 : lane >> 5);
+      unsigned short hi, mid, lo;
+      split_weight(w, hi, mid, lo);
+      img[0 * 512 + lane * 8 + e] = two_half_bias && (lane >> 5) == 1 ? mid : hi;
+      if (DYN_SPLIT_PARTS >= 2) img[1 * 512 + lane * 8 + e] = mid;
+      if (DYN_SPLIT_PARTS == 3) img[2 * 512 + lane * 8 + e] = lo;
+    }
+}
 void pack_layer_b6(std::vector<float>& out, int NT, int NSLOTS, const SlotFn& fn, int ones_slot = -1) {
   const int CPAIRS = g_pack_chunk_pairs, CFLOATS = CPAIRS * B6_PAIR_FLOATS;
   const int NG = (NSLOTS + 7) / 8, GPC = CPAIRS / NT, NCH = (NG + GPC - 1) / GPC;
@@ -26,25 +41,33 @@
       const int g = c * GPC + gi;
       if (g >= NG) continue;
       for (int t = 0; t < NT; ++t)
-        for (int lane = 0; lane < 64; ++lane)
-          for (int e = 0; e < 8; ++e) {
-            const int s = g * 8 + e;
-            if (s >= NSLOTS) continue;
-            const bool two_half_bias = DYN_SPLIT_PARTS == 1 && s == ones_slot;
-            if (two_half_bias && fn(t, lane & 31, s, 1) != 0.f) g_pack_slot_error = true;
-            const float w = fn(t, lane & 31, s, two_half_bias ? 0 : lane >> 5);
-            unsigned short hi, mid, lo;
-            split_weight(w, hi, mid, lo);
-            const size_t pair = (size_t)c * CFLOATS * 2 + (size_t)(gi * NT + t) * B6_PAIR_FLOATS * 2;
-            img[pair + 0 * 512 + lane * 8 + e] = two_half_bias && (lane >> 5) == 1 ? mid : hi;
-            if (DYN_SPLIT_PARTS >= 2) img[pair + 1 * 512 + lane * 8 + e] = mid;
-            if (DYN_SPLIT_PARTS == 3) img[pair + 2 * 512 + lane * 8 + e] = lo;
-          }
-    }
-}
-
+        pack_pair_b6(img + (size_t)c * CFLOATS * 2 + (size_t)(gi * NT + t) * B6_PAIR_FLOATS * 2, NSLOTS, g, t, fn, ones_slot);
+    }
+}
+void pack_layer_b6_dense(std::vector<float>& out, size_t base, int& cursor, int NT, int NSLOTS, const SlotFn& fn, int ones_slot = -1) {
+  const int NG = (NSLOTS + 7) / 8, end = cursor + NG * NT;
+  const size_t need = base + (size_t)b6_dense_chunks(end) * B6_CHUNK;
+  if (out.size() < need) out.resize(need, 0.f);
+  unsigned short* img = reinterpret_cast<unsigned short*>(out.data() + base);
+  for (int g = 0; g < NG; ++g)
+    for (int t = 0; t < NT; ++t) pack_pair_b6(img + (size_t)(cursor + g * NT + t) * B6_PAIR_FLOATS * 2, NSLOTS, g, t, fn, ones_slot);
+  cursor = end;
+}
+
+struct PackedLayer {
+  int NT, NSLOTS;
+  SlotFn fn;
+  int ones_slot;
+};
+thread_local std::vector<PackedLayer>* g_pack_record = nullptr;
 void pack_net_layer(std::vector<float>& out, int NT, int NSLOTS, const SlotFn& fn, int ones_slot = -1) {
+  if (g_pack_record) g_pack_record->push_back({NT, NSLOTS, fn, ones_slot});
   pack_layer_b6(out, NT, NSLOTS, fn, ones_slot);
+}
+void pack_dense_stream(std::vector<float>& out, const std::vector<PackedLayer>& layers, std::initializer_list<int> which) {
+  const size_t base = out.size();
+  int cursor = 0;
+  for (int i : which) pack_layer_b6_dense(out, base, cursor, layers[i].NT, layers[i].NSLOTS, layers[i].fn, layers[i].ones_slot);
 }
 
 inline int chain_feature(int s, int h) { return 32 * (s / 16) + dyn_fi(s % 16, h); }
@@ -100,6 +123,15 @@
 #define SA_L3V_STEPS (SA_NX + 1)
 #define SA_L4_STEPS 128
 #define SA_L5_STEPS 64
+#ifndef DYN_DENSE_STREAM
+#define DYN_DENSE_STREAM 1
+#endif
+constexpr int SA_D_L1V = 0;
+constexpr int SA_D_L2 = SA_D_L1V + b6_layer_pairs(8, SA_L1V_STEPS);
+constexpr int SA_D_L3V = SA_D_L2 + b6_layer_pairs(2, SA_L2_STEPS);
+constexpr int SA_D_L4 = SA_D_L3V + b6_layer_pairs(8, SA_L3V_STEPS);
+constexpr int VT_D_PAIRS = b6_layer_pairs(4, SA_L4_STEPS) + 3 * b6_layer_pairs(4, SA_L5_STEPS);
+constexpr int SA_D_CHUNKS = b6_dense_chunks(SA_D_L4 + VT_D_PAIRS);
 constexpr int SA_CHUNKS = net_layer_chunks(8, SA_L1P_STEPS) + net_layer_chunks(8, SA_L1V_STEPS) + net_layer_chunks(2, SA_L2_STEPS) + net_layer_chunks(8, SA_L3P_STEPS) + net_layer_chunks(8, SA_L3V_STEPS) +
                           net_layer_chunks(4, SA_L4_STEPS) + 3 * net_layer_chunks(4, SA_L5_STEPS);
 #ifndef DYN_POINTS_DUO
@@ -135,7 +167,8 @@
 constexpr size_t ST_OFF_CTC = ST_OFF_CTB + SB_CT;
 constexpr size_t ST_OFF_REF = ST_OFF_CTC + SC_CT;
 constexpr size_t ST_OFF_B8 = (ST_OFF_REF + 35 * 66 + 36 + 63) / 64 * 64;
-constexpr size_t ST_BLOB_FLOATS = ST_OFF_B8 + (DYN_POINTS_DUO ? (size_t)SB_CHUNKS * PTS_CHUNK : 0);
+constexpr size_t ST_OFF_AD = ST_OFF_B8 + (DYN_POINTS_DUO ? (size_t)SB_CHUNKS * PTS_CHUNK : 0);
+constexpr size_t ST_BLOB_FLOATS = ST_OFF_AD + (DYN_DENSE_STREAM ? (size_t)SA_D_CHUNKS * NET_CHUNK : 0);
 
 enum {
   DT_RAYDIR0_W, DT_RAYDIR0_B, DT_RAYDIR2_W, DT_RAYDIR2_B, DT_BASE0_W, DT_BASE0_B, DT_BASE2_W, DT_BASE2_B, DT_VIS0_W, DT_VIS0_B, DT_VIS2_W,
@@ -147,6 +180,9 @@
 #define DA_L3_STEPS (3 * DA_NX + 1)
 #define DA_L3P_STEPS (2 * DA_NX)
 #define DA_L3V_STEPS (DA_NX + 1)
+constexpr int DA_D_L3V = 0;
+constexpr int DA_D_L4 = DA_D_L3V + b6_layer_pairs(8, DA_L3V_STEPS);
+constexpr int DA_D_CHUNKS = b6_dense_chunks(DA_D_L4 + VT_D_PAIRS);
 constexpr int DA_CHUNKS = net_layer_chunks(8, DA_L3P_STEPS) + net_layer_chunks(8, DA_L3V_STEPS) + net_layer_chunks(4, SA_L4_STEPS) + 3 * net_layer_chunks(4, SA_L5_STEPS);
 constexpr int DB_CHUNKS = pts_layer_chunks(8, 129) + pts_layer_chunks(4, 129) + 4 * pts_layer_chunks(4, 64) + pts_layer_chunks(8, 81) +
                           pts_layer_chunks(4, 129) + pts_layer_chunks(4, 65) + pts_layer_chunks(4, 78) + pts_layer_chunks(2, 65);
@@ -158,7 +194,8 @@
 constexpr size_t DY_OFF_POSENC = DY_OFF_CTB + DB_CT;
 constexpr size_t DY_OFF_TIME = DY_OFF_POSENC + 256 * 128;
 constexpr size_t DY_OFF_B8 = (DY_OFF_TIME + 256 * 21 + 256 + 35 * 256 + 36 + 63) / 64 * 64;
-constexpr size_t DY_BLOB_FLOATS = DY_OFF_B8 + (DYN_POINTS_DUO ? (size_t)DB_CHUNKS * PTS_CHUNK : 0);
+constexpr size_t DY_OFF_AD = DY_OFF_B8 + (DYN_POINTS_DUO ? (size_t)DB_CHUNKS * PTS_CHUNK : 0);
+constexpr size_t DY_BLOB_FLOATS = DY_OFF_AD + (DYN_DENSE_STREAM ? (size_t)DA_D_CHUNKS * NET_CHUNK : 0);
 __host__ __device__ constexpr int da_c35(int q, int h) { return h == 0 ? q : (q < 17 ? 18 + q : -1); }
 
 __host__ __device__ constexpr int sa_c70(int q, int h) {
@@ -197,6 +234,8 @@
   g_pack_range_error = false;
   g_pack_slot_error = false;
   o.reserve(ST_BLOB_FLOATS);
+  std::vector<PackedLayer> a_layers;
+  g_pack_record = &a_layers;
   {
     const float *W = T[ST_RAYDIR0_W], *b = T[ST_RAYDIR0_B];
     pack_net_layer(o, 8, SA_L1P_STEPS, scaled([=](int t, int i, int s, int h) -> float {
@@ -226,6 +265,7 @@
   pack_net_layer(o, 4, SA_L5_STEPS, scaled(chained(T[ST_VIS0_W], nullptr, 128, 128, 128), DYN_ELU_PRE));
   pack_net_layer(o, 4, SA_L5_STEPS, scaled(chained(T[ST_VIS2_W], nullptr, 128, 128, 128), DYN_ELU_POST));
   pack_net_layer(o, 4, SA_L5_STEPS, scaled(chained(T[ST_VISB0_W], nullptr, 128, 128, 128), DYN_ELU_PRE));
+  g_pack_record = nullptr;
   DYN_REQUIRE(o.size() == ST_OFF_B, "static pack: A stream size mismatch");
   const auto pack_b = [&](bool by_head) {
 #if DYN_POINTS_DUO
@@ -297,7 +337,11 @@
 #if DYN_POINTS_DUO
   pack_b(true);
 #endif
-  DYN_REQUIRE(o.size() == ST_BLOB_FLOATS, "static pack: B8 stream size mismatch");
+  DYN_REQUIRE(o.size() == ST_OFF_AD, "static pack: B8 stream size mismatch");
+#if DYN_DENSE_STREAM
+  pack_dense_stream(o, a_layers, {1, 2, 4, 5, 6, 7, 8});
+#endif
+  DYN_REQUIRE(o.size() == ST_BLOB_FLOATS, "static pack: dense stream size mismatch");
   DYN_REQUIRE(!g_pack_slot_error, "dyn_static_net_pack: a layer's bias slot carries a weight in its second half (the one-product build stores the bias residual there)");
   DYN_REQUIRE(!g_pack_range_error, "dyn_static_net_pack: a weight is outside the half-float range of the split engine (|w| >= 65504 or not finite)");
   for (size_t i = 0; i < ST_BLOB_FLOATS; ++i) blob[i] = o[i];
@@ -703,16 +747,21 @@
   }
 }
 
-template <class Op>
+template <bool LDS_ONLY>
+__device__ __forceinline__ void view_sync() {
+  if constexpr (LDS_ONLY) b6_lds_sync();
+  else __syncthreads();
+}
+template <bool LDS_ONLY = false, class Op>
 __device__ __forceinline__ float dense_all(const DenseRows& d, float v, float ident, Op op) {
   if ((threadIdx.x & 32) == 0) d.scal[d.rw] = v;
-  __syncthreads();
+  view_sync<LDS_ONLY>();
   const float* src = d.scal + d.base;
   float a0 = ident, a1 = ident, a2 = ident, a3 = ident;
   int k = 0;
   for (; k + 4 <= d.cnt; k += 4) { a0 = op(a0, src[k]); a1 = op(a1, src[k + 1]); a2 = op(a2, src[k + 2]); a3 = op(a3, src[k + 3]); }
   for (; k < d.cnt; ++k) a0 = op(a0, src[k]);
-  __syncthreads();
+  view_sync<LDS_ONLY>();
   return op(op(a0, a1), op(a2, a3));
 }
 __device__ __forceinline__ void dense_all2(const DenseRows& d, float v0, float v1, float& s0, float& s1) {
@@ -726,14 +775,14 @@
   __syncthreads();
   s0 = a0 + a1; s1 = b0 + b1;
 }
-template <int VSEG>
+template <int VSEG, bool LDS_ONLY = false>
 __device__ __forceinline__ float views_sum(const DenseRows& d, float v) {
-  if constexpr (VSEG == 0) return dense_all(d, v, 0.f, [](float a, float b) { return a + b; });
+  if constexpr (VSEG == 0) return dense_all<LDS_ONLY>(d, v, 0.f, [](float a, float b) { return a + b; });
   else return seg_sum<VSEG>(v, 0, 0);
 }
-template <int VSEG>
+template <int VSEG, bool LDS_ONLY = false>
 __device__ __forceinline__ float views_min(const DenseRows& d, float v) {
-  if constexpr (VSEG == 0) return dense_all(d, v, 3.0e38f, [](float a, float b) { return fminf(a, b); });
+  if constexpr (VSEG == 0) return dense_all<LDS_ONLY>(d, v, 3.0e38f, [](float a, float b) { return fminf(a, b); });
   else return seg_min<VSEG>(v, 0, 0);
 }
 template <int VSEG>
@@ -745,7 +794,7 @@
 __device__ __forceinline__ float4 dense_quad(const float* src, int k, int stride, int) { return *reinterpret_cast<const float4*>(src + k * stride); }
 __device__ __forceinline__ float dense_w(const float* w, int k, int) { return w[k]; }
 
-template <int NX>
+template <int NX, bool LDS_ONLY = false>
 __device__ __forceinline__ void dense_pool_stats(const DenseRows& d, const float (&xin)[NX], float wgt, float* pool, float* tab) {
   constexpr int QPH = 4, RS = 2 * 4 * QPH + 4;
   constexpr int NQ = (NX + 3) / 4, ROUNDS = (NQ + QPH - 1) / QPH;
@@ -762,7 +811,7 @@
       const int q = round * QPH + qq;
       if (q < NQ) mine[qq] = make_float4(X(4 * q), X(4 * q + 1), X(4 * q + 2), X(4 * q + 3));
     }
-    __syncthreads();
+    view_sync<LDS_ONLY>();
     const int total = d.PTW * 2 * nq;
     for (int task = tid; task < total; task += DYN_VIEW_THREADS) {
       const int pnt = task / (2 * nq), rem = task - pnt * (2 * nq), hh = rem / nq, qq = rem - hh * nq;
@@ -814,30 +863,37 @@
         }
       }
     }
-    __syncthreads();
-  }
-}
-
-template <int VSEG, int NX>
+    view_sync<LDS_ONLY>();
+  }
+}
+
+template <int NT, int NSLOTS, int AT, class Feed>
+__device__ __forceinline__ void view_layer(NetRing& ring, f32x16 (&acc)[NT], Feed&& feed) {
+  if constexpr (AT >= 0) net_layer<NT, NSLOTS, B6_AHEAD, AT, true>(ring, acc, feed);
+  else net_layer<NT, NSLOTS>(ring, acc, feed);
+}
+
+template <int VSEG, int NX, int L3V_AT = -1>
 __device__ __forceinline__ void base_fc0(NetRing& ring, const float* pooled_w, const float (&xin)[NX], float wgt, int V, int view, int p_local,
                                          float* pool, f32x16 (&a1)[8], const DenseRows* dr = nullptr, float wsum = 0.f) {
   constexpr int PHASE_KID = 0;
   (void)PHASE_KID;
   const int lane = threadIdx.x & 63, j = lane & 31, h = lane >> 5, wave = threadIdx.x >> 6;
   const float one_h0 = DYN_BIAS_ONE(h);
+  constexpr bool LDS_ONLY = L3V_AT >= 0;
   if constexpr (VSEG == 0) {
     float* res = pool + POOL_FLOATS(NX);
     B6TileW<2 * NX> pw;
     b6_tile_prefetch<8, 2 * NX>(pooled_w, wave, pw);
-    dense_pool_stats<NX>(*dr, xin, wgt, pool, res);
+    dense_pool_stats<NX, LDS_ONLY>(*dr, xin, wgt, pool, res);
     if (threadIdx.x < 2 * 2 * NX)
       for (int c = dr->PTW; c < 32; ++c) pool[threadIdx.x * 32 + c] = 0.f;
-    __syncthreads();
+    view_sync<LDS_ONLY>();
     f32x16 accp[1];
     acc_zero(accp);
     b6_tile_apply<2 * NX>(pw, accp[0], [&](int s) { return pool[(s * 2 + h) * 32 + j]; });
     res_put(res, wave, j, h, accp[0]);
-    __syncthreads();
+    view_sync<LDS_ONLY>();
     const int col = dr->p_local < dr->PTW ? dr->p_local : dr->PTW - 1;
     res_get(res, col, h, a1);
   } else if (VSEG >= 8) {
@@ -879,13 +935,13 @@
     if (8 * PT < 32 && threadIdx.x < 2 * 2 * NX)
       for (int c = 8 * PT; c < 32; ++c) pool[threadIdx.x * 32 + c] = 0.f;
     DYN_PHASE(6);
-    __syncthreads();
+    view_sync<LDS_ONLY>();
     f32x16 accp[1];
     acc_zero(accp);
     b6_tile_apply<2 * NX>(pw, accp[0], [&](int s) { return pool[(s * 2 + h) * 32 + j]; });
     DYN_PHASE(7);
     res_put(res, wave, j, h, accp[0]);
-    __syncthreads();
+    view_sync<LDS_ONLY>();
     res_get(res, col, h, a1);
     DYN_PHASE(8);
   } else {
@@ -898,11 +954,11 @@
       return seg_sum<VSEG>(wgt * (d * d), V, 0);
     });
   }
-  net_layer<8, NX + 1>(ring, a1, [&](int s) { return s < NX ? xin[s] : one_h0; });
+  view_layer<8, NX + 1, L3V_AT>(ring, a1, [&](int s) { return s < NX ? xin[s] : one_h0; });
   DYN_PHASE(9);
 }
 
-template <int VSEG, bool STORE_X>
+template <int VSEG, bool STORE_X, int L4_AT = -1>
 __device__ __forceinline__ void views_tail(NetRing& ring, f32x16 (&a1)[8], const StaticArgs& p, const float* ctab, float wgt, float msk,
                                            long tile, long point, bool valid, int view, int seg_base, const DenseRows* dr = nullptr,
                                            float* lds_base = nullptr, int v_const = 0) {
@@ -910,10 +966,12 @@
   (void)PHASE_KID;
   const int lane = threadIdx.x & 63, h = lane >> 5;
   const int V = v_const > 0 ? v_const : p.V;
+  constexpr int L5_PAIRS = b6_layer_pairs(4, SA_L5_STEPS);
+  constexpr int L5A_AT = L4_AT < 0 ? -1 : L4_AT + b6_layer_pairs(4, SA_L4_STEPS), L5B_AT = L4_AT < 0 ? -1 : L5A_AT + L5_PAIRS, L5C_AT = L4_AT < 0 ? -1 : L5B_AT + L5_PAIRS;
   f32x16 x[4];
   {
     acc_init_bias<4>(x, ctab + 272);
-    net_layer<4, SA_L4_STEPS>(ring, x, [&](int s) { return elu_s(a1[s / 16][s % 16]); });
+    view_layer<4, SA_L4_STEPS, L4_AT>(ring, x, [&](int s) { return elu_s(a1[s / 16][s % 16]); });
     DYN_PHASE(11);
   }
   float vis;
@@ -921,14 +979,14 @@
     f32x16 a5[4], a6[4];
     acc_init_bias<4>(a5, ctab + 400);
     DYN_PHASE(12);
-    net_layer<4, SA_L5_STEPS>(ring, a5, [&](int s) {
+    view_layer<4, SA_L5_STEPS, L5A_AT>(ring, a5, [&](int s) {
       const float r = elu1(x[s / 16][s % 16]);
       x[s / 16][s % 16] = r;
       return r * wgt;
     });
     DYN_PHASE(13);
     acc_init_bias<4>(a6, ctab + 528);
-    net_layer<4, SA_L5_STEPS>(ring, a6, [&](int s) {
+    view_layer<4, SA_L5_STEPS, L5B_AT>(ring, a6, [&](int s) {
       const float r = elu_s(a5[s / 16][s % 16]);
       a5[s / 16][s % 16] = r;
       return r;
@@ -945,7 +1003,7 @@
     f32x16 a7[4];
     acc_init_bias<4>(a7, ctab + 656);
     DYN_PHASE(15);
-    net_layer<4, SA_L5_STEPS>(ring, a7, [&](int s) { return x[s / 16][s % 16] * vis; });
+    view_layer<4, SA_L5_STEPS, L5C_AT>(ring, a7, [&](int s) { return x[s / 16][s % 16] * vis; });
     DYN_PHASE(16);
     acc_elu_s(a7);
     vis2 = sigmoid1(row_dot<4>(a7, ctab + 128) + ctab[257]) * msk;
@@ -1098,6 +1156,10 @@
   const bool valid = (VSEG == 0 ? p_local < PT : view < V) && (point < p.n_pts);
   const int seg_base = 0;
   const long pv = valid ? point * V + view : 0;
+  constexpr bool DSTREAM = POOLED && DYN_DENSE_STREAM;
+  if constexpr (DSTREAM)
+    net_ring_init(ring, p.blob + ST_OFF_AD, SA_D_CHUNKS, lds, 1 << 30, 0, DYN_VIEW_THREADS);
+  else
   net_ring_init(ring, p.blob + ST_OFF_A + (POOLED ? (size_t)SA_L1P_CHUNKS * NET_CHUNK : 0), SA_CHUNKS - (POOLED ? SA_L1P_CHUNKS : 0), lds,
                 SA_POOLED_AT - (POOLED ? SA_L1P_CHUNKS : 0), POOLED ? net_layer_chunks(8, SA_L3P_STEPS) : 0, DYN_VIEW_THREADS);
 
@@ -1166,13 +1228,13 @@
     in1[34] = h0 ? rd.z : rd.w;
     in1[35] = DYN_BIAS_ONE(h0 ? 0 : 1);
     DYN_PHASE(1);
-    net_layer<8, SA_L1V_STEPS>(ring, a1, [&](int s) { return in1[s]; });
+    view_layer<8, SA_L1V_STEPS, DSTREAM ? SA_D_L1V : -1>(ring, a1, [&](int s) { return in1[s]; });
     DYN_PHASE(2);
   }
   {
     f32x16 a2[2];
     acc_init_bias<2>(a2, ctab + 784);
-    net_layer<2, SA_L2_STEPS>(ring, a2, [&](int s) {
+    view_layer<2, SA_L2_STEPS, DSTREAM ? SA_D_L2 : -1>(ring, a2, [&](int s) {
       if (s == 64) {
 #pragma unroll
         for (int q = 0; q < 18; ++q) {
@@ -1200,18 +1262,18 @@
   float wgt;
   if (p.anti_alias) {
     const float e = ((VSEG == 0 ? p_local < PT : view < V)) ? aa_exp(ctab[258], rd.w) : 3.0e38f;
-    const float emin = RAG ? (valid ? p.rg_emin[point] : e) : views_min<VSEG>(dr, e);
+    const float emin = RAG ? (valid ? p.rg_emin[point] : e) : views_min<VSEG, DSTREAM>(dr, e);
     wgt = (e - emin) * msk;
   } else {
     wgt = msk;
   }
-  const float wraw = views_sum<VSEG>(dr, wgt);
+  const float wraw = views_sum<VSEG, DSTREAM>(dr, wgt);
   wgt = wgt / (wraw + 1e-8f);
 
   DYN_PHASE(5);
-  base_fc0<VSEG, SA_NX>(ring, p.blob + ST_OFF_A + (size_t)SA_POOLED_AT * NET_CHUNK, xin, wgt, V, view, p_local, ctab + SA_CT, a1, &dr, wraw / (wraw + 1e-8f));
+  base_fc0<VSEG, SA_NX, DSTREAM ? SA_D_L3V : -1>(ring, p.blob + ST_OFF_A + (size_t)SA_POOLED_AT * NET_CHUNK, xin, wgt, V, view, p_local, ctab + SA_CT, a1, &dr, wraw / (wraw + 1e-8f));
   DYN_PHASE(10);
-  views_tail<VSEG, true>(ring, a1, p, ctab, wgt, msk, tile, point, valid, view, seg_base, &dr, lds, VC);
+  views_tail<VSEG, true, DSTREAM ? SA_D_L4 : -1>(ring, a1, p, ctab, wgt, msk, tile, point, valid, view, seg_base, &dr, lds, VC);
   DYN_PHASE(20);
 }
 
@@ -2257,6 +2319,8 @@
   g_pack_range_error = false;
   g_pack_slot_error = false;
   o.reserve(DY_BLOB_FLOATS);
+  std::vector<PackedLayer> a_layers;
+  g_pack_record = &a_layers;
   {
     const float *W = T[DT_BASE0_W], *b = T[DT_BASE0_B];
     pack_net_layer(o, 8, DA_L3P_STEPS, scaled([=](int t, int i, int s, int h) -> float {
@@ -2274,6 +2338,7 @@
   pack_net_layer(o, 4, SA_L5_STEPS, scaled(chained(T[DT_VIS0_W], nullptr, 128, 128, 128), DYN_ELU_PRE));
   pack_net_layer(o, 4, SA_L5_STEPS, scaled(chained(T[DT_VIS2_W], nullptr, 128, 128, 128), DYN_ELU_POST));
   pack_net_layer(o, 4, SA_L5_STEPS, scaled(chained(T[DT_VISB0_W], nullptr, 128, 128, 128), DYN_ELU_PRE));
+  g_pack_record = nullptr;
   DYN_REQUIRE(o.size() == DY_OFF_B, "dynamic pack: A stream size mismatch");
   const auto pack_b = [&](bool by_head) {
 #if DYN_POINTS_DUO
@@ -2356,7 +2421,11 @@
 #if DYN_POINTS_DUO
   pack_b(true);
 #endif
-  DYN_REQUIRE(o.size() == DY_BLOB_FLOATS, "dynamic pack: B8 stream size mismatch");
+  DYN_REQUIRE(o.size() == DY_OFF_AD, "dynamic pack: B8 stream size mismatch");
+#if DYN_DENSE_STREAM
+  pack_dense_stream(o, a_layers, {1, 2, 3, 4, 5});
+#endif
+  DYN_REQUIRE(o.size() == DY_BLOB_FLOATS, "dynamic pack: dense stream size mismatch");
   DYN_REQUIRE(!g_pack_slot_error, "dyn_dynamic_net_pack: a layer's bias slot carries a weight in its second half (the one-product build stores the bias residual there)");
   DYN_REQUIRE(!g_pack_range_error, "dyn_dynamic_net_pack: a weight is outside the half-float range of the split engine (|w| >= 65504 or not finite)");
   for (size_t i = 0; i < DY_BLOB_FLOATS; ++i) blob[i] = o[i];
@@ -2406,6 +2475,10 @@
   for (int i = tid; i < SA_CT; i += DYN_VIEW_THREADS) ctab[i] = p.blob[DY_OFF_CTA + i];
   NetRing ring;
   constexpr int LDS_FLOATS = 2 * NET_CHUNK + SA_CT + POOL_FLOATS(SA_NX) + RES_FLOATS + (VSEG == 0 ? DENSE_EXTRA : 0);
+  constexpr bool DSTREAM = (VSEG >= 8 || VSEG == 0) && DYN_DENSE_STREAM;
+  if constexpr (DSTREAM)
+    net_ring_init(ring, p.blob + DY_OFF_AD, DA_D_CHUNKS, lds, 1 << 30, 0, DYN_VIEW_THREADS);
+  else
   net_ring_init(ring, p.blob + DY_OFF_A, DA_CHUNKS, lds, 0, (VSEG >= 8 || VSEG == 0) ? net_layer_chunks(8, DA_L3P_STEPS) : 0, DYN_VIEW_THREADS);
 
   const int V = p.V;
@@ -2430,8 +2503,8 @@
   const float wraw = views_sum<VSEG>(dr, msk);
   const float wgt = msk / (wraw + 1e-8f);
   f32x16 a1[8];
-  base_fc0<VSEG, DA_NX>(ring, p.blob + DY_OFF_A, xin, wgt, V, view, p_local, ctab + SA_CT, a1, &dr, wraw / (wraw + 1e-8f));
-  views_tail<VSEG, false>(ring, a1, p, ctab, wgt, msk, tile, point, valid, view, seg_base, &dr, lds);
+  base_fc0<VSEG, DA_NX, DSTREAM ? DA_D_L3V : -1>(ring, p.blob + DY_OFF_A, xin, wgt, V, view, p_local, ctab + SA_CT, a1, &dr, wraw / (wraw + 1e-8f));
+  views_tail<VSEG, false, DSTREAM ? DA_D_L4 : -1>(ring, a1, p, ctab, wgt, msk, tile, point, valid, view, seg_base, &dr, lds);
 }
 
 extern "C" int dyn_dynamic_net(const DynDynamicNetParams* q, void* stream_) {
@@ -2647,6 +2720,13 @@
   return 0;
 }
 
+extern "C" int dyn_view_ring_chunks(int dynamic) {
+#if DYN_DENSE_STREAM
+  return dynamic ? DA_D_CHUNKS : SA_D_CHUNKS;
+#else
+  return dynamic ? DA_CHUNKS - net_layer_chunks(8, DA_L3P_STEPS) : SA_CHUNKS - net_layer_chunks(8, SA_L1P_STEPS) - net_layer_chunks(8, SA_L3P_STEPS);
+#endif
+}
 extern "C" int dyn_mlp_split_terms(void) {
   return DYN_SPLIT_TERMS;
 }
@@ -2696,3 +2776,82 @@
              (hipStream_t)stream, stream_buf, x, y, rows);
   return 0;
 }
+
+#define TC_L1_STEPS 33
+#define TC_L2_STEPS 129
+#define TC_L3_STEPS 33
+#define TC_L4_STEPS 128
+#define TC_L5_STEPS 17
+constexpr int TC_D_L2 = b6_layer_pairs(8, TC_L1_STEPS);
+constexpr int TC_D_L3 = TC_D_L2 + b6_layer_pairs(2, TC_L2_STEPS);
+constexpr int TC_D_L4 = TC_D_L3 + b6_layer_pairs(8, TC_L3_STEPS);
+constexpr int TC_D_L5 = TC_D_L4 + b6_layer_pairs(4, TC_L4_STEPS);
+constexpr int TC_D_CHUNKS = b6_dense_chunks(TC_D_L5 + b6_layer_pairs(4, TC_L5_STEPS));
+constexpr int TC_A_CHUNKS = net_layer_chunks(8, TC_L1_STEPS) + net_layer_chunks(2, TC_L2_STEPS) + net_layer_chunks(8, TC_L3_STEPS) + net_layer_chunks(4, TC_L4_STEPS) +
+                            net_layer_chunks(4, TC_L5_STEPS);
+constexpr size_t TC_W1 = 0, TC_B1 = TC_W1 + 256 * 64, TC_W2 = TC_B1 + 256, TC_B2 = TC_W2 + 64 * 256, TC_W3 = TC_B2 + 64, TC_B3 = TC_W3 + 256 * 64,
+                 TC_W4 = TC_B3 + 256, TC_W5 = TC_W4 + 128 * 256, TC_B5 = TC_W5 + 128 * 32;
+
+template <bool DENSE>
+__global__ void __launch_bounds__(DYN_VIEW_THREADS, 2) k_selftest_chain(const float* __restrict__ stream, const float* __restrict__ x, float* __restrict__ y, int rows) {
+  float* lds = reinterpret_cast<float*>(dyn_smem);
+  const int lane = threadIdx.x & 63, j = lane & 31, h = lane >> 5, wave = threadIdx.x >> 6;
+  NetRing ring;
+  net_ring_init_t(ring, stream, DENSE ? TC_D_CHUNKS : TC_A_CHUNKS, lds, DYN_VIEW_THREADS);
+  const int row = (blockIdx.x * (DYN_VIEW_THREADS / 64) + wave) * 32 + j;
+  const float one_h0 = DYN_BIAS_ONE(h);
+  float in[32];
+#pragma unroll
+  for (int s = 0; s < 32; ++s) in[s] = row < rows ? x[row * 64 + 32 * (s / 16) + dyn_fi(s % 16, h)] : 0.f;
+  f32x16 a3[8];
+  {
+    f32x16 a2[2];
+    {
+      f32x16 a1[8];
+      acc_zero(a1);
+      view_layer<8, TC_L1_STEPS, DENSE ? 0 : -1>(ring, a1, [&](int s) { return s < 32 ? in[s] : one_h0; });
+      acc_zero(a2);
+      view_layer<2, TC_L2_STEPS, DENSE ? TC_D_L2 : -1>(ring, a2, [&](int s) { return s < 128 ? elu1(a1[s / 16][s % 16]) : one_h0; });
+    }
+    acc_zero(a3);
+    view_layer<8, TC_L3_STEPS, DENSE ? TC_D_L3 : -1>(ring, a3, [&](int s) { return s < 32 ? elu1(a2[s / 16][s % 16]) : one_h0; });
+  }
+  f32x16 a4[4], a5[4];
+  acc_zero(a4);
+  view_layer<4, TC_L4_STEPS, DENSE ? TC_D_L4 : -1>(ring, a4, [&](int s) { return elu1(a3[s / 16][s % 16]); });
+  acc_zero(a5);
+  view_layer<4, TC_L5_STEPS, DENSE ? TC_D_L5 : -1>(ring, a5, [&](int s) { return s < 16 ? elu1(a4[0][s]) : one_h0; });
+  if (row < rows)
+#pragma unroll
+    for (int s = 0; s < 64; ++s) y[row * 128 + 32 * (s / 16) + dyn_fi(s % 16, h)] = a5[s / 16][s % 16];
+}
+
+extern "C" size_t dyn_mlp_selftest_chain_floats(void) { return (size_t)(TC_A_CHUNKS + TC_D_CHUNKS) * NET_CHUNK; }
+
+extern "C" int dyn_mlp_selftest_chain(const float* weights, const float* x, float* y_aligned, float* y_dense, int rows, float* stream_buf, void* stream) {
+  DYN_REQUIRE(weights && x && y_aligned && y_dense && stream_buf && rows > 0, "dyn_mlp_selftest_chain: bad argument");
+  const float* W = weights;
+  std::vector<PackedLayer> L;
+  std::vector<float> o;
+  g_pack_slot_error = false;
+  g_pack_record = &L;
+  pack_net_layer(o, 8, TC_L1_STEPS, chained(W + TC_W1, W + TC_B1, 256, 64, 64), 32);
+  pack_net_layer(o, 2, TC_L2_STEPS, chained(W + TC_W2, W + TC_B2, 64, 256, 256), 128);
+  pack_net_layer(o, 8, TC_L3_STEPS, chained(W + TC_W3, W + TC_B3, 256, 64, 64), 32);
+  pack_net_layer(o, 4, TC_L4_STEPS, chained(W + TC_W4, nullptr, 128, 256, 256));
+  pack_net_layer(o, 4, TC_L5_STEPS, chained(W + TC_W5, W + TC_B5, 128, 32, 32), 16);
+  g_pack_record = nullptr;
+  DYN_REQUIRE(o.size() == (size_t)TC_A_CHUNKS * NET_CHUNK, "dyn_mlp_selftest_chain: aligned stream size mismatch");
+  pack_dense_stream(o, L, {0, 1, 2, 3, 4});
+  DYN_REQUIRE(o.size() == dyn_mlp_selftest_chain_floats(), "dyn_mlp_selftest_chain: dense stream size mismatch");
+  DYN_REQUIRE(!g_pack_slot_error, "dyn_mlp_selftest_chain: a bias slot carries a weight in its second half");
+  if (hipMemcpy(stream_buf, o.data(), o.size() * sizeof(float), hipMemcpyHostToDevice) != hipSuccess) {
+    dyn_set_error("dyn_mlp_selftest_chain: hipMemcpy failed");
+    return DYN_E_LAUNCH;
+  }
+  const dim3 grid(dyn_cdiv(rows, 256)), blk(DYN_VIEW_THREADS);
+  DYN_LAUNCH(DYN_K_SELFTEST, "k_selftest", k_selftest_chain<false>, grid, blk, 2 * NET_CHUNK * sizeof(float), (hipStream_t)stream, stream_buf, x, y_aligned, rows);
+  DYN_LAUNCH(DYN_K_SELFTEST, "k_selftest", k_selftest_chain<true>, grid, blk, 2 * NET_CHUNK * sizeof(float), (hipStream_t)stream,
+             stream_buf + (size_t)TC_A_CHUNKS * NET_CHUNK, x, y_dense, rows);
+  return 0;
+}
diff --git a/include/dynibar_hip.h b/include/dynibar_hip.h
--- a/include/dynibar_hip.h
+++ b/include/dynibar_hip.h
@@ -187,6 +187,11 @@
 int dyn_mlp_split_kind(void);
 
 int dyn_mlp_selftest(const float* W, const float* b, const float* x, float* y, int rows, float* stream_buf, void* stream);
+
+int dyn_view_ring_chunks(int dynamic);
+
+size_t dyn_mlp_selftest_chain_floats(void);
+int dyn_mlp_selftest_chain(const float* weights, const float* x, float* y_aligned, float* y_dense, int rows, float* stream_buf, void* stream);
 
 int dyn_profile_enable(int on);
 int dyn_profile_count(void);
```

After: 1.536 million, median of 6. No clear change (+0.1%).
